# rajgandhi1/threecrate

Hardware: AMD Instinct MI355X
Metric: ICP iterations/sec (whole job: k=16 normals + 50-iter point-to-plane ICP per 1M-pt pair; tc_cloud handles, inputs resident in HBM) (higher is better)
Workload: dtype f32; 1 GPU; 1000000-pt uniform-random cloud, k=16 normals + 50-iter point-to-plane ICP, independent sigma = 0.0001 noise on source and target, correspondences returned (BASELINE configs[1]; one independent pair per GPU); points=1000000, k=16, parallelism=pairs1, interface=tc_cloud handles (one index build per cloud)

## Files before the change

### threecrate_amd/csrc/api.hip

```cpp
#include "tc_internal.h"
#include <sched.h>
#include <time.h>

#include <algorithm>
#include <cmath>
#include <cstdlib>
#include <cstring>
#include <memory>

namespace tc {

[[maybe_unused]] constexpr int kDebugPrintOnlyBits = 8 | 64 | 256 | 1024;
int debug_flags() {
    static const int flags = [] {
        const char *e = getenv("TC_DEBUG");
        const int f = e ? atoi(e) : 0;
#ifdef TC_DEV
        return f;
#else
        return f & kDebugPrintOnlyBits;
#endif
    }();
    return flags;
}
// ... 178 lines not shown
    return TC_OK;
}

tc_status synced(tc_context *ctx) {
    TC_HIP_TRY(ctx, hipStreamSynchronize(ctx->stream));
    return TC_OK;
}
tc_status stage_out(tc_context *ctx, void *h_dst, const void *d_src, size_t bytes) {
    TC_HIP_TRY(ctx, hipMemcpyAsync(h_dst, d_src, bytes, hipMemcpyDeviceToHost, ctx->stream));
    return synced(ctx);
}
tc_status read_back(tc_context *ctx, void *host_dst, const void *dev_src, size_t bytes) {
    if (tc_status s = stage_out(ctx, host_dst, dev_src, bytes)) return s;
    TC_HIP_TRY(ctx, hipGetLastError());
    return TC_OK;
}

float normals_cell_factor(size_t k, bool large) {
    const double K1 = (double)k + 1.0;
    const double lam = K1 + 3.1 * std::sqrt(K1) + 2.0;
    const double c = std::cbrt(lam / 4.18879);
    return (float)((large ? 1.03 : 0.95) * c / 2.0);
}

float normals_target_ppo(size_t k) {
    const double K1 = (double)k + 1.0;
    return (float)((K1 + 3.1 * std::sqrt(K1) + 2.0) / 11.3);
}

IndexSpec knn_grid(size_t list_len) {
    IndexSpec spec; spec.cell_factor = normals_cell_factor(list_len > 1 ? list_len - 1 : 1, false) * 2.0f;
    return spec;
}
IndexSpec ball_grid(float radius, bool finite_only) {
    const float r2 = radius * radius;
    IndexSpec spec; spec.cell_factor = 0.5f;
    if (r2 <= r2 && (!finite_only || r2 <= 3.0e38f)) { spec.min_cell_edge = 0.5f * radius; spec.target_ppo = 2.0f; }
    return spec;
}

void recycle_index(tc_context *ctx, DeviceIndex &ix) {
    for_each_buf(ix, [ctx](DevBuf &b) { recycle(ctx, b); });
    ix.pts12_valid = false; ix.vor_valid = false;
}

void free_index(DeviceIndex &ix) { for_each_buf(ix, free_buf); }

tc_status normals_on_index(tc_context *ctx, DeviceIndex &ix, bool build, float cell_factor_override, const float *d_xyz, size_t n,
                           const tc_normal_config *cfg, float *d_out, size_t p_begin, size_t p_end, bool slice_out, float4 *d_sorted_nrm,
                           bool with_bounds) {
    if (build) {
        const float min_h = cfg->has_radius ? cfg->radius * 0.5005f : 0.0f;
        const float f = cell_factor_override > 0.0f ? cell_factor_override : normals_cell_factor(cfg->k_neighbors, n >= kAdaptMinPoints);
        IndexSpec spec; spec.cell_factor = f; spec.min_cell_edge = min_h; spec.target_ppo = normals_target_ppo(cfg->k_neighbors); spec.strict_order = slice_out;
        if (tc_status s = build_index(ctx, ix, d_xyz, n, spec)) return s;
    }
    float vp[3];
    if (cfg->has_viewpoint) {
        vp[0] = cfg->viewpoint[0]; vp[1] = cfg->viewpoint[1]; vp[2] = cfg->viewpoint[2];
    } else {
        const float *bmn = ix.exact_min, *bmx = ix.exact_max;
        const float cx = (bmn[0] + bmx[0]) / 2.0f, cy = (bmn[1] + bmx[1]) / 2.0f, cz = (bmn[2] + bmx[2]) / 2.0f;
        const float ex = bmx[0] - bmn[0], ey = bmx[1] - bmn[1], ez = bmx[2] - bmn[2];
        const float extent = std::sqrt(ex * ex + ey * ey + ez * ez);
        vp[0] = cx + 0.0f; vp[1] = cy + 0.0f; vp[2] = cz + extent;
    }
    float4 *d_vor = nullptr;
    const bool knn_mode = !(cfg->has_radius && cfg->radius > 0.0f);
    if (with_bounds && knn_mode && p_begin == 0 && p_end >= n) {
        if (tc_status s = ensure(ctx, ix.vor, n * sizeof(float4))) return s;
        d_vor = (float4 *)ix.vor.p;
    }
    if (tc_status s = launch_normals(ctx, ix, d_xyz, *cfg, vp, d_out, p_begin, p_end, slice_out, d_sorted_nrm, d_vor)) return s;
    ix.vor_valid = d_vor != nullptr;
    return TC_OK;
}

static tc_status normals_device(tc_context *ctx, const float *d_xyz, size_t n, const tc_normal_config *cfg, float *d_out,
                                size_t p_begin = 0, size_t p_end = (size_t)-1, bool slice_out = false) {
    return normals_on_index(ctx, ctx->tgt_index, true, 0.0f, d_xyz, n, cfg, d_out, p_begin, p_end, slice_out, nullptr);
}

}

using namespace tc;

extern "C" {

int tc_abi_version(void) { return TC_ABI_VERSION; }

int tc_device_count(void) try {
    int n = 0;
    if (hipGetDeviceCount(&n) != hipSuccess) return 0;
    return n;
} TC_CATCH_VALUE(0)

static tc_status context_create(int device, void *stream, bool own, tc_context **out) {
    if (!out) return TC_INVALID_DATA;
    *out = nullptr;
    fault_point("context");
    int n = 0;
    if (hipGetDeviceCount(&n) != hipSuccess || n <= 0 || device < 0 || device >= n) return TC_GPU;
    if (hipSetDevice(device) != hipSuccess) return TC_GPU;
    std::unique_ptr<tc_context> holder(new tc_context());
    tc_context *ctx = holder.get();
    ctx->last_error.reserve(256);
    ctx->device = device;
    ctx->own_stream = own;
    if (own) {
        if (hipStreamCreateWithFlags(&ctx->stream, hipStreamNonBlocking) != hipSuccess) return TC_GPU;
    } else {
        ctx->stream = (hipStream_t)stream;
    }
    if (hipHostMalloc(&ctx->pinned, kPinnedBytes, hipHostMallocDefault) != hipSuccess) {
        if (own) (void)hipStreamDestroy(ctx->stream);
        return TC_GPU;
    }
    *out = holder.release();
    return TC_OK;
}

tc_status tc_context_create(int device, tc_context **out) try { return context_create(device, nullptr, true, out); } TC_CATCH_STATUS(nullptr)
tc_status tc_context_create_on_stream(int device, void *hip_stream, tc_context **out) try {
    return context_create(device, hip_stream, false, out);
} TC_CATCH_STATUS(nullptr)

tc_status tc_context_wait_stream(tc_context *ctx, void *other_hip_stream) try {
    if (!ctx) return TC_INVALID_DATA;
    hipStream_t other = (hipStream_t)other_hip_stream;
    if (other == ctx->stream) return TC_OK;
    TC_HIP_TRY(ctx, hipSetDevice(ctx->device));
    if (!ctx->order_event) TC_HIP_TRY(ctx, hipEventCreateWithFlags(&ctx->order_event, hipEventDisableTiming));
    TC_HIP_TRY(ctx, hipEventRecord(ctx->order_event, other));
    TC_HIP_TRY(ctx, hipStreamWaitEvent(ctx->stream, ctx->order_event, 0));
    return TC_OK;
} TC_CATCH_STATUS(ctx)

tc_status tc_stream_wait_context(tc_context *ctx, void *other_hip_stream) try {
    if (!ctx) return TC_INVALID_DATA;
    hipStream_t other = (hipStream_t)other_hip_stream;
    if (other == ctx->stream) return TC_OK;
    TC_HIP_TRY(ctx, hipSetDevice(ctx->device));
    if (!ctx->release_event) TC_HIP_TRY(ctx, hipEventCreateWithFlags(&ctx->release_event, hipEventDisableTiming));
    TC_HIP_TRY(ctx, hipEventRecord(ctx->release_event, ctx->stream));
    TC_HIP_TRY(ctx, hipStreamWaitEvent(other, ctx->release_event, 0));
    return TC_OK;
} TC_CATCH_STATUS(ctx)

void tc_context_destroy(tc_context *ctx) try {
    if (!ctx) return;
    (void)hipSetDevice(ctx->device);
    (void)hipStreamSynchronize(ctx->stream);
    if (ctx->copy_stream) { (void)hipStreamSynchronize(ctx->copy_stream); (void)hipStreamDestroy(ctx->copy_stream); }
    if (ctx->upload_event) (void)hipEventDestroy(ctx->upload_event);
    for_each_buf(*ctx, free_buf);
    for (auto &pb : ctx->pool) (void)hipFree(pb.p);
    for (auto e : ctx->chunk_events) (void)hipEventDestroy(e);
    if (ctx->order_event) (void)hipEventDestroy(ctx->order_event);
    if (ctx->release_event) (void)hipEventDestroy(ctx->release_event);
    for (auto &t : ctx->timers) for (auto &p : t.pending) { (void)hipEventDestroy(p.first); (void)hipEventDestroy(p.second); }
    for (auto e : ctx->event_pool) (void)hipEventDestroy(e);
    if (ctx->pinned) (void)hipHostFree(ctx->pinned);
    if (ctx->own_stream && ctx->stream) (void)hipStreamDestroy(ctx->stream);
    delete ctx;
} TC_CATCH_VOID

tc_status tc_context_trim(tc_context *ctx) try {
    if (!ctx) return TC_INVALID_DATA;
    TC_HIP_TRY(ctx, hipSetDevice(ctx->device));
    TC_HIP_TRY(ctx, hipStreamSynchronize(ctx->stream));
    for (auto &pb : ctx->pool) (void)hipFree(pb.p);
    ctx->pool.clear();
    ctx->pool_bytes = 0;
    ctx->pool_largest = 0;
    return TC_OK;
} TC_CATCH_STATUS(ctx)

const char *tc_last_error_message(const tc_context *ctx) { return ctx ? ctx->last_error.c_str() : "null context"; }

tc_status tc_synchronize(tc_context *ctx) try {
    if (!ctx) return TC_INVALID_DATA;
    return synced(ctx);
} TC_CATCH_STATUS(ctx)

void tc_normal_config_default(tc_normal_config *cfg) try {
    if (!cfg) return;
    std::memset(cfg, 0, sizeof(*cfg));
    cfg->k_neighbors = 10;
    cfg->has_radius = 0;
    cfg->consistent_orientation = 1;
    cfg->has_viewpoint = 0;
} TC_CATCH_VOID

static tc_status normals_validate(tc_context *ctx, size_t n, const tc_normal_config *cfg, bool *empty) {
    *empty = false;
    if (!ctx || !cfg) return TC_INVALID_DATA;
    if (n == 0) { *empty = true; return TC_OK; }
    if (cfg->k_neighbors < 3) return fail(ctx, TC_INVALID_DATA, "k_neighbors must be at least 3");
    return TC_OK;
}

tc_status tc_estimate_normals_device(tc_context *ctx, const float *d_xyz, size_t n, const tc_normal_config *cfg,
                                     float *d_out) try {
    bool empty;
    if (tc_status s = normals_validate(ctx, n, cfg, &empty)) return s;
    if (empty) return TC_OK;
    TC_HIP_TRY(ctx, hipSetDevice(ctx->device));
    if (tc_status s = normals_device(ctx, d_xyz, n, cfg, d_out)) return s;
    return synced(ctx);
} TC_CATCH_STATUS(ctx)

tc_status tc_estimate_normals_slice_device(tc_context *ctx, const float *d_xyz, size_t n, const tc_normal_config *cfg, size_t begin,
                                           size_t end, float *d_slice_out) try {
    bool empty;
    if (tc_status s = normals_validate(ctx, n, cfg, &empty)) return s;
    if (empty) return TC_OK;
    if (begin > end || end > n) return fail(ctx, TC_INVALID_DATA, "normals slice: need begin <= end <= n");
    TC_HIP_TRY(ctx, hipSetDevice(ctx->device));
    if (tc_status s = normals_device(ctx, d_xyz, n, cfg, d_slice_out, begin, end, true)) return s;
    return synced(ctx);
} TC_CATCH_STATUS(ctx)

tc_status tc_normals_unsort_device(tc_context *ctx, const float *d_sorted_all, size_t n, float *d_out) try {
    if (!ctx) return TC_INVALID_DATA;
    if (n == 0) return TC_OK;
    if (ctx->tgt_index.geom.n != n || !ctx->tgt_index.pts.p)
        return fail(ctx, TC_INVALID_DATA, "normals unsort: call tc_estimate_normals_slice_device on this context with the same cloud first");
    TC_HIP_TRY(ctx, hipSetDevice(ctx->device));
    if (tc_status s = launch_normals_unsort(ctx, ctx->tgt_index, d_sorted_all, d_out)) return s;
    return synced(ctx);
} TC_CATCH_STATUS(ctx)

tc_status tc_estimate_normals(tc_context *ctx, const float *xyz, size_t n, const tc_normal_config *cfg, float *out) try {
    bool empty;
    if (tc_status s = normals_validate(ctx, n, cfg, &empty)) return s;
    if (empty) return TC_OK;
    TC_HIP_TRY(ctx, hipSetDevice(ctx->device));
    if (tc_status s = ensure(ctx, ctx->out_a, n * 6 * sizeof(float))) return s;
    if (tc_status s = stage_in(ctx, ctx->in_a, xyz, n * 3 * sizeof(float))) return s;
    if (tc_status s = normals_device(ctx, (const float *)ctx->in_a.p, n, cfg, (float *)ctx->out_a.p)) return s;
    return stage_out(ctx, out, ctx->out_a.p, n * 6 * sizeof(float));
} TC_CATCH_STATUS(ctx)

static tc_status sharded_normals_slot(tc_context *ctx, tc_comm *comm, const float *d_xyz, size_t n, const tc_normal_config *cfg,
                                      float *slot_out, size_t &lo, size_t &hi) {
    const size_t W = (size_t)comm->nranks, r = (size_t)comm->rank;
    const size_t rows = (n + W - 1) / W;
    lo = std::min(r * rows, n); hi = std::min((r + 1) * rows, n);
    return normals_device(ctx, d_xyz, n, cfg, slot_out, lo, hi, true);
}

tc_status tc_sharded_estimate_normals_device(tc_context *ctx, tc_comm *comm, const float *d_xyz, size_t n, const tc_normal_config *cfg,
                                             float *d_out) try {
    if (!comm) return TC_INVALID_DATA;
    bool empty;
    if (tc_status s = normals_validate(ctx, n, cfg, &empty)) return s;
    if (empty) return TC_OK;
    if (comm->ctx != ctx) return fail(ctx, TC_INVALID_DATA, "the communicator belongs to another context");
    TC_HIP_TRY(ctx, hipSetDevice(ctx->device));
    const size_t W = (size_t)comm->nranks, r = (size_t)comm->rank;
    const size_t rows = (n + W - 1) / W;
    tc_status local = ensure(ctx, ctx->out_a, W * rows * 6 * sizeof(float));
    float *sorted_all = (float *)ctx->out_a.p;
    size_t lo = 0, hi = 0;
    if (local == TC_OK) local = sharded_normals_slot(ctx, comm, d_xyz, n, cfg, sorted_all + r * rows * 6, lo, hi);
    if (tc_status s = comm_agree(comm, local)) return s;
    if (tc_status s = comm_allgather(comm, sorted_all, rows * 6 * sizeof(float))) return s;
    if (tc_status s = launch_normals_unsort(ctx, ctx->tgt_index, sorted_all, d_out)) return s;
    return synced(ctx);
} TC_CATCH_STATUS(ctx)

__global__ void __launch_bounds__(256) slice_orig_index_kernel(const float4 *__restrict__ pts, uint32_t lo, uint32_t count, uint32_t *__restrict__ out) {
    const uint32_t i = blockIdx.x * blockDim.x + threadIdx.x;
    if (i < count) out[i] = __float_as_uint(pts[lo + i].w);
}

tc_status tc_sharded_estimate_normals_local_device(tc_context *ctx, tc_comm *comm, const float *d_xyz, size_t n, const tc_normal_config *cfg,
                                                   float *d_out_slice, uint32_t *d_orig_index, size_t *first, size_t *count) try {
    if (!comm || !first || !count) return TC_INVALID_DATA;
    *first = 0; *count = 0;
    bool empty;
    if (tc_status s = normals_validate(ctx, n, cfg, &empty)) return s;
    if (empty) return TC_OK;
    if (comm->ctx != ctx) return fail(ctx, TC_INVALID_DATA, "the communicator belongs to another context");
    TC_HIP_TRY(ctx, hipSetDevice(ctx->device));
    size_t lo = 0, hi = 0;
    if (tc_status s = sharded_normals_slot(ctx, comm, d_xyz, n, cfg, d_out_slice, lo, hi)) return s;
    if (d_orig_index && hi > lo) {
        hipLaunchKernelGGL(slice_orig_index_kernel, dim3((unsigned)((hi - lo + 255) / 256)), dim3(256), 0, ctx->stream,
                           (const float4 *)ctx->tgt_index.pts.p, (uint32_t)lo, (uint32_t)(hi - lo), d_orig_index);
        TC_HIP_TRY(ctx, hipGetLastError());
    }
    TC_HIP_TRY(ctx, hipStreamSynchronize(ctx->stream));
    *first = lo; *count = hi - lo;
    return TC_OK;
} TC_CATCH_STATUS(ctx)

unsigned long long tc_debug_counter(const tc_context *ctx, int which) try {
    if (!ctx) return 0;
    if (which >= TC_COUNTER_ICP_ITERATIONS && which <= TC_COUNTER_ICP_STEPS_TAKEN) return ctx->stat_icp[which - TC_COUNTER_ICP_ITERATIONS];
    return which == TC_COUNTER_INDEXED_POINTS ? ctx->stat_indexed_points : which == TC_COUNTER_INDEX_BUILDS ? ctx->stat_index_builds : 0ull;
} TC_CATCH_VALUE(0)

void tc_profile_enable(tc_context *ctx, int on) {
    if (!ctx) return;
    ctx->profiling = on;
    ctx->prof_tick = 0;
    if (on == 3) for (auto &v : ctx->stat_icp) v = 0;
}

static void profile_collect(tc_context *ctx) {
    (void)hipStreamSynchronize(ctx->stream);
    for (auto &t : ctx->timers) {
        for (auto &p : t.pending) {
            float ms = 0.0f;
            if (hipEventElapsedTime(&ms, p.first, p.second) == hipSuccess) {
                t.total_ms += ms; t.launches += 1;
                t.min_ms = std::min(t.min_ms, (double)ms); t.max_ms = std::max(t.max_ms, (double)ms);
            }
            ctx->event_pool.push_back(p.first);
            ctx->event_pool.push_back(p.second);
        }
        t.pending.clear();
    }
}

void tc_profile_reset(tc_context *ctx) try {
    if (!ctx) return;
    profile_collect(ctx);
    for (auto &t : ctx->timers) { t.launches = 0; t.total_ms = 0.0; t.min_ms = 1e300; t.max_ms = 0.0; }
} TC_CATCH_VOID

size_t tc_profile_read(tc_context *ctx, tc_kernel_stat *out, size_t cap) try {
    if (!ctx) return 0;
    profile_collect(ctx);
    size_t n = 0;
    for (auto &t : ctx->timers) {
        if (n < cap && out) {
            std::memset(&out[n], 0, sizeof(out[n]));
            std::strncpy(out[n].name, t.name.c_str(), sizeof(out[n].name) - 1);
            out[n].launches = t.launches;
            out[n].total_ms = t.total_ms;
            out[n].min_ms = t.launches ? t.min_ms : 0.0;
            out[n].max_ms = t.max_ms;
        }
        ++n;
    }
    return n;
} TC_CATCH_VALUE(0)

}
```

### threecrate_amd/csrc/cloud.hip

```cpp
#include "tc_internal.h"

#include <algorithm>
#include <cmath>
#include <cstring>

struct tc_cloud {
    tc_context *ctx = nullptr;
    size_t n = 0;
    tc::DevBuf xyz;
    tc::DeviceIndex ix;
    bool indexed = false;
    float factor = 0.0f;
    bool has_normals = false;
    tc::DevBuf normals6;
    bool has_normals6 = false;
};

namespace {

using namespace tc;


float shared_factor(float want) {
    return (want > 0.8f * kIcpCellFactor && want < 1.25f * kIcpCellFactor) ? kIcpCellFactor : want;
}

__global__ void __launch_bounds__(256) cloud_unsort_normals_kernel(const float4 *__restrict__ pts, const float4 *__restrict__ sorted_nrm,
                                                                  const float *__restrict__ xyz, uint32_t n, float *__restrict__ out6) {
    const uint32_t p = blockIdx.x * blockDim.x + threadIdx.x;
    if (p >= n) return;
    const uint32_t orig = __float_as_uint(pts[p].w);
    const float4 nr = sorted_nrm[p];
    float *o = out6 + 6 * (size_t)orig;
    o[0] = xyz[3 * (size_t)orig]; o[1] = xyz[3 * (size_t)orig + 1]; o[2] = xyz[3 * (size_t)orig + 2];
    o[3] = nr.x; o[4] = nr.y; o[5] = nr.z;
}

tc_status ensure_index(tc_cloud *c, float want_factor, float target_ppo, float min_h) {
    tc_context *ctx = c->ctx;
    const float f = shared_factor(want_factor);
    if (c->indexed && c->factor > 0.8f * f && c->factor < 1.25f * f && min_h <= c->ix.geom.h) return TC_OK;
    if (c->has_normals && !c->has_normals6 && c->indexed && c->n) {
        if (tc_status s = ensure(ctx, c->normals6, c->n * 6 * sizeof(float))) return s;
        hipLaunchKernelGGL(cloud_unsort_normals_kernel, dim3((unsigned)((c->n + 255) / 256)), dim3(256), 0, ctx->stream,
                           (const float4 *)c->ix.pts.p, (const float4 *)c->ix.normals.p, (const float *)c->xyz.p, (uint32_t)c->n,
                           (float *)c->normals6.p);
        TC_HIP_TRY(ctx, hipGetLastError());
        c->has_normals6 = true;
    }
    c->has_normals = false;
    IndexSpec spec; spec.cell_factor = f; spec.min_cell_edge = min_h; spec.target_ppo = target_ppo;
    if (tc_status s = build_index(ctx, c->ix, (const float *)c->xyz.p, c->n, spec)) return s;
    c->indexed = true;
    c->factor = f;
    return TC_OK;
}

tc_status cloud_create(tc_context *ctx, const float *p, size_t n, bool from_host, tc_cloud **out) {
    if (!ctx || !out) return TC_INVALID_DATA;
    *out = nullptr;
    if (tc_status s = check_point_count(ctx, n)) return s;
    TC_HIP_TRY(ctx, hipSetDevice(ctx->device));
    tc_cloud *c = new tc_cloud();
    c->ctx = ctx;
    c->n = n;
    if (n) {
        tc_status s = ensure(ctx, c->xyz, n * 3 * sizeof(float));
        if (s == TC_OK && hipMemcpyAsync(c->xyz.p, p, n * 3 * sizeof(float), from_host ? hipMemcpyHostToDevice : hipMemcpyDeviceToDevice,
                                         ctx->stream) != hipSuccess) s = fail(ctx, TC_GPU, "cloud upload failed");
        if (s == TC_OK && from_host && hipStreamSynchronize(ctx->stream) != hipSuccess) s = fail(ctx, TC_GPU, "cloud upload failed");
        if (s != TC_OK) { recycle(ctx, c->xyz); delete c; return s; }
    }
    *out = c;
    return TC_OK;
}

tc_status adopt_normals(tc_cloud *c, const float *d_normals, size_t stride) {
    if (tc_status s = ensure_index(c, kIcpCellFactor, 2.5f, 0.0f)) return s;
    if (tc_status s = gather_normals(c->ctx, c->ix, d_normals, stride)) return s;
    c->has_normals = true;
    return TC_OK;
}

tc_status prepare_target(tc_cloud *tgt, bool p2plane);

tc_status cloud_icp(tc_cloud *src, tc_cloud *tgt, bool p2plane, const float init[7], size_t max_iters, float max_dist, float conv_thr,
                    tc_icp_result *res) {
    if (!src || !tgt || !res || !init) return TC_INVALID_DATA;
    tc_context *ctx = tgt->ctx;
    if (src->ctx != ctx) return fail(ctx, TC_INVALID_DATA, "source and target handles belong to different contexts");
    if (src->n == 0 || tgt->n == 0) return fail(ctx, TC_INVALID_DATA, "Source or target point cloud is empty");
    if (p2plane && !tgt->has_normals && !tgt->has_normals6)
        return fail(ctx, TC_INVALID_DATA, "target_normals length must equal the number of target points (the target handle has no normals: "
                                          "tc_cloud_estimate_normals or tc_cloud_set_normals_device first)");
    if (max_iters == 0) return fail(ctx, TC_INVALID_DATA, "Max iterations must be positive");
    TC_HIP_TRY(ctx, hipSetDevice(ctx->device));
    if (tc_status s = prepare_target(tgt, p2plane)) return s;
    IcpJob job;
    job.mode = p2plane ? 1 : 0;
    job.src = (const float *)src->xyz.p; job.ns = src->n; job.tgt = (const float *)tgt->xyz.p; job.nt = tgt->n;
    job.init = init; job.max_iters = max_iters; job.max_dist = max_dist; job.conv_thr = conv_thr;
    job.tgt_prebuilt = &tgt->ix;
    job.src_presorted = (src->indexed && src != tgt) ? &src->ix : nullptr;
    return icp_run(ctx, job, res);
}

tc_status prepare_target(tc_cloud *tgt, bool p2plane) {
    tc_context *ctx = tgt->ctx;
    if (tc_status s = ensure_index(tgt, kIcpCellFactor, 2.5f, 0.0f)) return s;
    if (p2plane && !tgt->has_normals) {
        if (!tgt->has_normals6) return fail(ctx, TC_INVALID_DATA, "the target handle has no normals in input order to re-sort after its index was rebuilt");
        if (tc_status s = gather_normals(ctx, tgt->ix, (const float *)tgt->normals6.p + 3, 6)) return s;
        tgt->has_normals = true;
    }
    return TC_OK;
}

}

extern "C" {

tc_status tc_cloud_sharded_icp(tc_comm *comm, int shard_mode, int point_to_plane, const float *d_source, size_t n_source, tc_cloud *target,
                               const float init[7], size_t max_iters, float max_dist, float conv_thr, tc_icp_result *result) try {
    if (!comm || !target || !result || !init) return TC_INVALID_DATA;
    tc_context *ctx = target->ctx;
    if (comm->ctx != ctx) return fail(ctx, TC_INVALID_DATA, "the communicator belongs to another context");
    if (shard_mode != TC_SHARD_SPATIAL && shard_mode != TC_SHARD_LOCAL && shard_mode != TC_SHARD_INDEX) return fail(ctx, TC_INVALID_DATA, "unknown shard mode");
    const bool may_be_empty = shard_mode == TC_SHARD_LOCAL && comm->nranks > 1;
    if ((n_source == 0 && !may_be_empty) || target->n == 0) return fail(ctx, TC_INVALID_DATA, "Source or target point cloud is empty");
    if (point_to_plane && !target->has_normals && !target->has_normals6)
        return fail(ctx, TC_INVALID_DATA, "target_normals length must equal the number of target points (the target handle has no normals)");
    if (max_iters == 0) return fail(ctx, TC_INVALID_DATA, "Max iterations must be positive");
    TC_HIP_TRY(ctx, hipSetDevice(ctx->device));
    if (tc_status s = prepare_target(target, point_to_plane != 0)) return s;
    IcpJob job;
    job.mode = point_to_plane ? 1 : 0;
    job.src = d_source; job.ns = n_source; job.tgt = (const float *)target->xyz.p; job.nt = target->n;
    job.init = init; job.max_iters = max_iters; job.max_dist = max_dist; job.conv_thr = conv_thr;
    job.tgt_prebuilt = &target->ix;
    return icp_run_sharded(ctx, comm, shard_mode, job, result);
} TC_CATCH_STATUS((comm ? comm->ctx : nullptr))

tc_status tc_cloud_upload(tc_context *ctx, const float *xyz, size_t n, tc_cloud **out) try { return cloud_create(ctx, xyz, n, true, out); } TC_CATCH_STATUS(ctx)
tc_status tc_cloud_upload_device(tc_context *ctx, const float *d_xyz, size_t n, tc_cloud **out) try { return cloud_create(ctx, d_xyz, n, false, out); } TC_CATCH_STATUS(ctx)
size_t tc_cloud_size(const tc_cloud *c) { return c ? c->n : 0; }
const float *tc_cloud_points_device(const tc_cloud *c) { return c ? (const float *)c->xyz.p : nullptr; }
const float *tc_cloud_normals_device(const tc_cloud *cc) try {
    tc_cloud *c = const_cast<tc_cloud *>(cc);
    if (!c || c->n == 0) return nullptr;
    if (c->has_normals6) return (const float *)c->normals6.p;
    if (!c->has_normals || !c->indexed) return nullptr;
    tc_context *ctx = c->ctx;
    if (hipSetDevice(ctx->device) != hipSuccess) { (void)fail(ctx, TC_GPU, "tc_cloud_normals_device: hipSetDevice failed"); return nullptr; }
    if (ensure(ctx, c->normals6, c->n * 6 * sizeof(float)) != TC_OK) return nullptr;
    hipLaunchKernelGGL(cloud_unsort_normals_kernel, dim3((unsigned)((c->n + 255) / 256)), dim3(256), 0, ctx->stream,
                       (const float4 *)c->ix.pts.p, (const float4 *)c->ix.normals.p, (const float *)c->xyz.p, (uint32_t)c->n,
                       (float *)c->normals6.p);
    hipError_t e = hipGetLastError();
    if (e == hipSuccess) e = hipStreamSynchronize(ctx->stream);
    if (e != hipSuccess) { (void)fail(ctx, TC_GPU, std::string("tc_cloud_normals_device: ") + hipGetErrorString(e)); return nullptr; }
    c->has_normals6 = true;
    return (const float *)c->normals6.p;
} TC_CATCH_VALUE(nullptr)

static tc_status cloud_normals(tc_cloud *c, const tc_normal_config *cfg, float *out, bool out_on_host, bool keep6) {
    if (!c || !cfg) return TC_INVALID_DATA;
    tc_context *ctx = c->ctx;
    if (c->n == 0) return TC_OK;
    if (cfg->k_neighbors < 3) return fail(ctx, TC_INVALID_DATA, "k_neighbors must be at least 3");
    TC_HIP_TRY(ctx, hipSetDevice(ctx->device));
    const float min_h = cfg->has_radius ? cfg->radius * 0.5005f : 0.0f;
    c->has_normals = false;
    c->has_normals6 = false;
    if (tc_status s = ensure_index(c, normals_cell_factor(cfg->k_neighbors, c->n >= kAdaptMinPoints), normals_target_ppo(cfg->k_neighbors), min_h)) return s;
    if (tc_status s = ensure(ctx, c->ix.normals, c->n * sizeof(float4))) return s;
    const bool direct = out != nullptr && !out_on_host && !keep6;
    const bool want6 = (out != nullptr || keep6) && !direct;
    float *d_out6 = direct ? out : nullptr;
    if (want6) {
        if (tc_status s = ensure(ctx, c->normals6, c->n * 6 * sizeof(float))) return s;
        d_out6 = (float *)c->normals6.p;
    }
    c->has_normals = false;
    c->has_normals6 = false;
    if (tc_status s = normals_on_index(ctx, c->ix, false, 0.0f, (const float *)c->xyz.p, c->n, cfg, d_out6, 0, (size_t)-1, false,
                                       (float4 *)c->ix.normals.p, true)) return s;
    c->has_normals = true;
    c->has_normals6 = want6;
    if (out && !direct) TC_HIP_TRY(ctx, hipMemcpyAsync(out, d_out6, c->n * 6 * sizeof(float), out_on_host ? hipMemcpyDeviceToHost : hipMemcpyDeviceToDevice, ctx->stream));
    TC_HIP_TRY(ctx, hipStreamSynchronize(ctx->stream));
    return TC_OK;
}

tc_status tc_cloud_estimate_normals(tc_cloud *c, const tc_normal_config *cfg, float *out) try { return cloud_normals(c, cfg, out, true, false); } TC_CATCH_STATUS(c ? c->ctx : nullptr)
tc_status tc_cloud_estimate_normals_device(tc_cloud *c, const tc_normal_config *cfg, float *d_out) try { return cloud_normals(c, cfg, d_out, false, false); } TC_CATCH_STATUS(c ? c->ctx : nullptr)

tc_status tc_cloud_set_normals_device(tc_cloud *c, const float *d_normals, size_t n_normals, size_t stride) try {
    if (!c) return TC_INVALID_DATA;
    tc_context *ctx = c->ctx;
    if (n_normals != c->n) return fail(ctx, TC_INVALID_DATA, "target_normals length must equal the number of target points");
    if (stride < 3) return fail(ctx, TC_INVALID_DATA, "normal_stride must be >= 3");
    if (c->n == 0) return TC_OK;
    TC_HIP_TRY(ctx, hipSetDevice(ctx->device));
    c->has_normals = false;
    c->has_normals6 = false;
    if (tc_status s = adopt_normals(c, d_normals, stride)) return s;
    TC_HIP_TRY(ctx, hipStreamSynchronize(ctx->stream));
    return TC_OK;
} TC_CATCH_STATUS((c ? c->ctx : nullptr))

tc_status tc_cloud_icp_point_to_plane(tc_cloud *source, tc_cloud *target, const float init[7], size_t max_iters, float max_dist,
                                      float conv_thr, tc_icp_result *result) try {
    return cloud_icp(source, target, true, init, max_iters, max_dist, conv_thr, result);
} TC_CATCH_STATUS((source ? source->ctx : nullptr))

tc_status tc_cloud_icp_detailed(tc_cloud *source, tc_cloud *target, const float init[7], size_t max_iters, float max_dist,
                                float conv_thr, tc_icp_result *result) try {
    return cloud_icp(source, target, false, init, max_iters, max_dist, conv_thr, result);
} TC_CATCH_STATUS((source ? source->ctx : nullptr))

void tc_cloud_destroy(tc_cloud *c) try {
    if (!c) return;
    (void)hipSetDevice(c->ctx->device);
    (void)hipStreamSynchronize(c->ctx->stream);
    tc::recycle(c->ctx, c->xyz); tc::recycle(c->ctx, c->normals6);
    tc::recycle_index(c->ctx, c->ix);
    delete c;
} TC_CATCH_VOID

}
```

### threecrate_amd/csrc/grid.hip

```cpp
#include "tc_internal.h"
#include <rocprim/device/device_radix_sort.hpp>

#include <algorithm>
#include <cmath>
#include <cstring>

namespace tc {

constexpr int kBboxBlocks = 256;
__device__ __forceinline__ uint32_t f2ord(float f) { const uint32_t b = __float_as_uint(f); return (b & 0x80000000u) ? ~b : (b | 0x80000000u); }
__device__ __forceinline__ float ord2f(uint32_t u) { return __uint_as_float((u & 0x80000000u) ? (u ^ 0x80000000u) : ~u); }
constexpr uint32_t kOrdPlusInf = 0xFF800000u, kOrdMinusInf = 0x007FFFFFu;
constexpr uint32_t kBboxAccStride = 32;
constexpr size_t kBboxStateBytes = 31 * kBboxAccStride * sizeof(uint32_t), kBboxBufBytes = kBboxStateBytes + 128 + 256;

template <bool VEC>
__global__ void __launch_bounds__(256) bbox_kernel(const float *__restrict__ xyz, uint32_t n, uint32_t *__restrict__ state, int robust,
                                                  float *__restrict__ out, uint32_t *__restrict__ done) {
    const bool sbox = robust != 0;
    __shared__ float sm[4][30];
    float v[30];
#pragma unroll
    for (int k = 0; k < 30; ++k) v[k] = (k % 6 < 3) ? INFINITY : -INFINITY;
    auto take = [&](float x, float y, float z, uint32_t i, int s) {
        if (!(fabsf(x) <= 3.0e38f && fabsf(y) <= 3.0e38f && fabsf(z) <= 3.0e38f)) return;
        v[0] = fminf(v[0], x); v[1] = fminf(v[1], y); v[2] = fminf(v[2], z);
        v[3] = fmaxf(v[3], x); v[4] = fmaxf(v[4], y); v[5] = fmaxf(v[5], z);
        if (sbox && ((i * 2654435761u) >> 28) == 0u) {
            float *b = v + 6 + 6 * s;
            b[0] = fminf(b[0], x); b[1] = fminf(b[1], y); b[2] = fminf(b[2], z);
            b[3] = fmaxf(b[3], x); b[4] = fmaxf(b[4], y); b[5] = fmaxf(b[5], z);
        }
    };
    const uint32_t gt = blockIdx.x * blockDim.x + threadIdx.x, stride = gridDim.x * blockDim.x;
    if constexpr (VEC) {
        const float4 *__restrict__ q = reinterpret_cast<const float4 *>(xyz);
        const uint32_t nq = n >> 2;
        constexpr int U = 4;
        for (uint32_t c0 = gt; c0 < nq; c0 += U * stride) {
            float4 a[U], b[U], c[U];
#pragma unroll
            for (int u = 0; u < U; ++u) {
                const uint32_t cc = min(c0 + (uint32_t)u * stride, nq - 1u);
                a[u] = q[3 * (size_t)cc]; b[u] = q[3 * (size_t)cc + 1]; c[u] = q[3 * (size_t)cc + 2];
            }
#pragma unroll
            for (int u = 0; u < U; ++u) {
                const uint32_t i = 4u * min(c0 + (uint32_t)u * stride, nq - 1u);
                take(a[u].x, a[u].y, a[u].z, i, 0);
                take(a[u].w, b[u].x, b[u].y, i + 1u, 1);
                take(b[u].z, b[u].w, c[u].x, i + 2u, 2);
                take(c[u].y, c[u].z, c[u].w, i + 3u, 3);
            }
        }
        if (gt < (n & 3u)) {
            const uint32_t i = (nq << 2) + gt;
            const float x = xyz[3 * (size_t)i], y = xyz[3 * (size_t)i + 1], z = xyz[3 * (size_t)i + 2];
            if ((i & 3u) == 0u) take(x, y, z, i, 0); else if ((i & 3u) == 1u) take(x, y, z, i, 1); else take(x, y, z, i, 2);
        }
    } else {
        for (uint32_t i = gt; i < n; i += stride) {
            const float x = xyz[3 * (size_t)i], y = xyz[3 * (size_t)i + 1], z = xyz[3 * (size_t)i + 2];
            const uint32_t sidx = threadIdx.x & 3u;
            if (sidx == 0u) take(x, y, z, i, 0); else if (sidx == 1u) take(x, y, z, i, 1); else if (sidx == 2u) take(x, y, z, i, 2); else take(x, y, z, i, 3);
        }
    }
#pragma unroll
    for (int k = 0; k < 30; ++k) {
        if (k < 6 || sbox) {
#pragma unroll
            for (int o = 32; o > 0; o >>= 1) {
                const float w = __shfl_xor(v[k], o);
                v[k] = (k % 6 < 3) ? fminf(v[k], w) : fmaxf(v[k], w);
            }
        }
    }
    if ((threadIdx.x & 63) == 0) {
#pragma unroll
        for (int k = 0; k < 30; ++k) sm[threadIdx.x >> 6][k] = v[k];
    }
    __syncthreads();
    uint32_t *acc = state + kBboxAccStride;
    if (threadIdx.x < (sbox ? 30 : 6)) {
        const bool is_min = threadIdx.x % 6 < 3;
        float r = sm[0][threadIdx.x];
        for (int w = 1; w < 4; ++w) r = is_min ? fminf(r, sm[w][threadIdx.x]) : fmaxf(r, sm[w][threadIdx.x]);
        if (is_min) atomicMin(&acc[threadIdx.x * kBboxAccStride], f2ord(r)); else atomicMax(&acc[threadIdx.x * kBboxAccStride], f2ord(r));
    }
    __shared__ uint32_t s_last;
    if (threadIdx.x < 64) {
        asm volatile("s_waitcnt vmcnt(0)" ::: "memory");
        if (threadIdx.x == 0) s_last = __hip_atomic_fetch_add(state, 1u, __ATOMIC_RELAXED, __HIP_MEMORY_SCOPE_AGENT) == gridDim.x - 1u ? 1u : 0u;
    }
    __syncthreads();
    if (!s_last) return;
    if (threadIdx.x < 30) {
        const uint32_t u = __hip_atomic_load(&acc[threadIdx.x * kBboxAccStride], __ATOMIC_RELAXED, __HIP_MEMORY_SCOPE_AGENT);
        __hip_atomic_store(&out[threadIdx.x], ord2f(u), __ATOMIC_RELAXED, __HIP_MEMORY_SCOPE_SYSTEM);
        __hip_atomic_store(&acc[threadIdx.x * kBboxAccStride], (threadIdx.x % 6 < 3) ? kOrdPlusInf : kOrdMinusInf, __ATOMIC_RELAXED, __HIP_MEMORY_SCOPE_AGENT);
    }
    if (threadIdx.x == 0) __hip_atomic_store(state, 0u, __ATOMIC_RELAXED, __HIP_MEMORY_SCOPE_AGENT);
    if (done) {
        if (threadIdx.x < 30) __threadfence_system();
        __syncthreads();
        if (threadIdx.x == 0) __hip_atomic_store(done, 1u, __ATOMIC_RELEASE, __HIP_MEMORY_SCOPE_SYSTEM);
    }
}

__global__ void bbox_state_init_kernel(uint32_t *__restrict__ state) {
    const uint32_t t = threadIdx.x;
    if (t == 0) state[0] = 0u;
    if (t < 30) state[(t + 1) * kBboxAccStride] = (t % 6 < 3) ? kOrdPlusInf : kOrdMinusInf;
}


__global__ void __launch_bounds__(256) cell_hist_kernel(const float *__restrict__ xyz, uint32_t n, GridGeom g,
                                                       const IcpState *__restrict__ st, TileGeom tg, int tile_major, uint32_t nkeys,
                                                       uint32_t *__restrict__ cell_of, uint32_t *__restrict__ hist,
                                                       uint32_t *__restrict__ arrival, uint32_t *__restrict__ pts_pad,
                                                       uint32_t *__restrict__ cs_front, uint32_t *__restrict__ cs_tail, uint32_t rank_max) {
    uint32_t i = blockIdx.x * blockDim.x + threadIdx.x;
    if (blockIdx.x == 0 && threadIdx.x < 4 * kPtsPad + kCellStartFront + kCellStartPad) {
        const uint32_t t = threadIdx.x;
        if (t < 4 * kPtsPad) pts_pad[t] = 0x7F7F7F7Fu;
        else if (t < 4 * kPtsPad + kCellStartFront) cs_front[t - 4 * kPtsPad] = 0u;
        else cs_tail[t - 4 * kPtsPad - kCellStartFront] = 0u;
    }
    if (i >= n) return;
    float x = xyz[3 * (size_t)i], y = xyz[3 * (size_t)i + 1], z = xyz[3 * (size_t)i + 2];
    if (st) {
        float q[4] = {st->q[0], st->q[1], st->q[2], st->q[3]}, t[3] = {st->t[0], st->t[1], st->t[2]};
        float ox, oy, oz;
        isometry_apply(q, t, x, y, z, ox, oy, oz);
        x = ox; y = oy; z = oz;
    }
    int ix = cell_coord(x, g.minx, g.inv_h, g.gx);
    int iy = cell_coord(y, g.miny, g.inv_h, g.gy);
    int iz = cell_coord(z, g.minz, g.inv_h, g.gz);
    uint32_t c = tile_major ? tile_major_id(tg, ix, iy, iz) : ((uint32_t)iz * g.gy + iy) * g.gx + ix;
    if (!(fabsf(x) <= 3.0e38f && fabsf(y) <= 3.0e38f && fabsf(z) <= 3.0e38f)) c = nkeys;
    cell_of[i] = c;
    const uint32_t a = atomicAdd(&hist[c], 1u);
    arrival[i] = a;
    if (a == rank_max) hist[nkeys + 1] = 1u;
}

__global__ void __launch_bounds__(256) iota_kernel(uint32_t *__restrict__ p, uint32_t n) {
    const uint32_t i = blockIdx.x * blockDim.x + threadIdx.x;
    if (i < n) p[i] = i;
}

constexpr int kScanItems = 8;
constexpr int kScanBlock = 256;
constexpr int kScanTile = kScanItems * kScanBlock;

__global__ void __launch_bounds__(kScanBlock) scan_reduce_kernel(const uint32_t *__restrict__ in, uint32_t n,
                                                                 uint32_t *__restrict__ blocksum) {
    __shared__ uint32_t wsum[kScanBlock / 64], wnz[kScanBlock / 64];
    uint32_t base = blockIdx.x * kScanTile;
    uint32_t s = 0, nz = 0;
#pragma unroll
    for (int k = 0; k < kScanItems; ++k) {
        uint32_t i = base + k * kScanBlock + threadIdx.x;
        if (i < n) { const uint32_t v = in[i]; s += v; nz += v != 0; }
    }
#pragma unroll
    for (int o = 32; o > 0; o >>= 1) { s += __shfl_xor(s, o); nz += __shfl_xor(nz, o); }
    if ((threadIdx.x & 63) == 0) { wsum[threadIdx.x >> 6] = s; wnz[threadIdx.x >> 6] = nz; }
    __syncthreads();
    if (threadIdx.x == 0) {
        blocksum[blockIdx.x] = wsum[0] + wsum[1] + wsum[2] + wsum[3];
        blocksum[gridDim.x + blockIdx.x] = wnz[0] + wnz[1] + wnz[2] + wnz[3];
    }
}

constexpr uint32_t kScanFusedMax = 2048;
__global__ void __launch_bounds__(1024) scan_top_kernel(uint32_t *__restrict__ blocksum, uint32_t nb) {
    __shared__ uint32_t wtot[16];
    uint32_t carry = 0;
    for (uint32_t base = 0; base < nb; base += 1024) {
        const uint32_t i = base + threadIdx.x;
        const uint32_t v = i < nb ? blocksum[i] : 0u;
        uint32_t inc = v;
#pragma unroll
        for (int o = 1; o < 64; o <<= 1) {
            const uint32_t t = __shfl_up(inc, o);
            if ((threadIdx.x & 63) >= (unsigned)o) inc += t;
        }
        if ((threadIdx.x & 63) == 63) wtot[threadIdx.x >> 6] = inc;
        __syncthreads();
        uint32_t woff = 0, tot = 0;
        for (int w = 0; w < 16; ++w) { if (w < (int)(threadIdx.x >> 6)) woff += wtot[w]; tot += wtot[w]; }
        if (i < nb) blocksum[i] = carry + woff + inc - v;
        carry += tot;
        __syncthreads();
    }
}

__global__ void __launch_bounds__(kScanBlock) scan_apply_kernel(const uint32_t *__restrict__ in, uint32_t n,
                                                                uint32_t *__restrict__ blocksum,
                                                                uint32_t *__restrict__ out , uint32_t *__restrict__ occ_out, int prefixed,
                                                                unsigned long long *__restrict__ occ_host) {
    __shared__ uint32_t wtot[kScanBlock / 64];
    __shared__ uint32_t wpre[kScanBlock / 64], wnz[kScanBlock / 64];
    uint32_t pre = 0, nzt = 0;
    if (prefixed) { if (threadIdx.x == 0) pre = blocksum[blockIdx.x]; }
    else for (uint32_t i = threadIdx.x; i < blockIdx.x; i += kScanBlock) pre += blocksum[i];
    if (blockIdx.x == 0) for (uint32_t i = threadIdx.x; i < gridDim.x; i += kScanBlock) nzt += blocksum[gridDim.x + i];
#pragma unroll
    for (int o = 32; o > 0; o >>= 1) { pre += __shfl_xor(pre, o); nzt += __shfl_xor(nzt, o); }
    if ((threadIdx.x & 63) == 0) { wpre[threadIdx.x >> 6] = pre; wnz[threadIdx.x >> 6] = nzt; }
    uint32_t base = blockIdx.x * kScanTile + threadIdx.x * kScanItems;
    uint32_t v[kScanItems];
    uint32_t s = 0;
#pragma unroll
    for (int k = 0; k < kScanItems; ++k) {
        uint32_t i = base + k;
        v[k] = (i < n) ? in[i] : 0;
        s += v[k];
    }
    uint32_t inc = s;
#pragma unroll
    for (int o = 1; o < 64; o <<= 1) {
        uint32_t t = __shfl_up(inc, o);
        if ((threadIdx.x & 63) >= (unsigned)o) inc += t;
    }
    if ((threadIdx.x & 63) == 63) wtot[threadIdx.x >> 6] = inc;
    __syncthreads();
    uint32_t woff = 0;
    for (int w = 0; w < (int)(threadIdx.x >> 6); ++w) woff += wtot[w];
    uint32_t block_pre = 0;
    for (int w = 0; w < kScanBlock / 64; ++w) block_pre += wpre[w];
    if (blockIdx.x == 0 && threadIdx.x == 0) {
        uint32_t t = 0;
        for (int w = 0; w < kScanBlock / 64; ++w) t += wnz[w];
        blocksum[2 * gridDim.x] = t;
        if (occ_out) *occ_out = t;
        if (occ_host) __hip_atomic_store(occ_host, (1ull << 32) | (unsigned long long)t, __ATOMIC_RELAXED, __HIP_MEMORY_SCOPE_SYSTEM);
    }
    uint32_t run = block_pre + woff + inc - s;
#pragma unroll
    for (int k = 0; k < kScanItems; ++k) {
        uint32_t i = base + k;
        if (i < n) out[i] = run;
        run += v[k];
        if (i == n - 1) out[n] = run;
    }
}

__global__ void __launch_bounds__(256) rank_gather_kernel(const float *__restrict__ xyz, uint32_t n, uint32_t nkeys,
                                                         const uint32_t *__restrict__ cell_of,
                                                         const uint32_t *__restrict__ cell_start,
                                                         const uint32_t *__restrict__ slot,
                                                         float4 *__restrict__ pts, int slot_is_ordered, uint32_t rank_max) {
    uint32_t p = blockIdx.x * blockDim.x + threadIdx.x;
    if (p >= n) return;
    uint32_t i = slot[p];
    uint32_t c = cell_of[i];
    uint32_t s = cell_start[c], e = cell_start[c + 1];
    uint32_t rank;
    if (slot_is_ordered) {
        rank = p - s;
    } else if (e - s <= rank_max) {
        rank = 0;
        for (uint32_t j = s; j < e; ++j) rank += (slot[j] < i) ? 1u : 0u;
    } else {
        rank = p - s;
    }
    float4 r;
    r.x = xyz[3 * (size_t)i]; r.y = xyz[3 * (size_t)i + 1]; r.z = xyz[3 * (size_t)i + 2];
    if (c == nkeys) r.x = r.y = r.z = __uint_as_float(0x7F7F7F7Fu);
    r.w = __uint_as_float(i);
    pts[s + rank] = r;
}

__global__ void __launch_bounds__(256) place_kernel(const float *__restrict__ xyz, uint32_t n, uint32_t nkeys,
                                                   const uint32_t *__restrict__ cell_of, const uint32_t *__restrict__ cell_start,
                                                   const uint32_t *__restrict__ arrival, float4 *__restrict__ tmp) {
    const uint32_t i = blockIdx.x * blockDim.x + threadIdx.x;
    if (i >= n) return;
    const uint32_t c = cell_of[i];
    const uint32_t pos = cell_start[c] + arrival[i];
    float4 r;
    r.x = xyz[3 * (size_t)i]; r.y = xyz[3 * (size_t)i + 1]; r.z = xyz[3 * (size_t)i + 2];
    if (c == nkeys) r.x = r.y = r.z = __uint_as_float(0x7F7F7F7Fu);
    r.w = __uint_as_float(i);
    tmp[pos] = r;
}

__global__ void __launch_bounds__(256) rerank_kernel(uint32_t n, GridGeom g, const IcpState *__restrict__ st, TileGeom tg, int tile_major,
                                                    uint32_t nkeys, const uint32_t *__restrict__ cell_start, const float4 *__restrict__ tmp,
                                                    float4 *__restrict__ pts, uint32_t rank_max) {
    const uint32_t p = blockIdx.x * blockDim.x + threadIdx.x;
    if (p >= n) return;
    const float4 r = tmp[p];
    uint32_t c;
    {
        float x = r.x, y = r.y, z = r.z;
        if (st) {
            float q[4] = {st->q[0], st->q[1], st->q[2], st->q[3]}, t[3] = {st->t[0], st->t[1], st->t[2]};
            float ox, oy, oz;
            isometry_apply(q, t, x, y, z, ox, oy, oz);
            x = ox; y = oy; z = oz;
        }
        const int ix = cell_coord(x, g.minx, g.inv_h, g.gx), iy = cell_coord(y, g.miny, g.inv_h, g.gy), iz = cell_coord(z, g.minz, g.inv_h, g.gz);
        c = tile_major ? tile_major_id(tg, ix, iy, iz) : ((uint32_t)iz * g.gy + iy) * g.gx + ix;
        if (!(fabsf(x) <= 3.0e38f && fabsf(y) <= 3.0e38f && fabsf(z) <= 3.0e38f)) c = nkeys;
    }
    const uint32_t s = cell_start[c], e = cell_start[c + 1];
    const uint32_t i = __float_as_uint(r.w);
    uint32_t rank;
    if (e - s <= rank_max) {
        rank = 0;
#pragma unroll 4
        for (uint32_t j = s; j < e; ++j) rank += (__float_as_uint(tmp[j].w) < i) ? 1u : 0u;
    } else {
        rank = p - s;
    }
    pts[s + rank] = r;
}

__global__ void __launch_bounds__(256) gather_normals_kernel(const float4 *__restrict__ pts, uint32_t n,
                                                            const float *__restrict__ nrm, size_t stride,
                                                            float4 *__restrict__ out) {
    uint32_t p = blockIdx.x * blockDim.x + threadIdx.x;
    if (p >= n) return;
    uint32_t i = __float_as_uint(pts[p].w);
    const float *s = nrm + (size_t)i * stride;
    out[p] = make_float4(s[0], s[1], s[2], 0.0f);
}

GridView view_of(const DeviceIndex &ix) {
    GridView v;
    v.g = ix.geom;
    v.pts = (const float4 *)ix.pts.p;
    v.cell_start = (const uint32_t *)ix.cell_start.p + kCellStartFront;
    v.pts12 = ix.pts12_valid ? (const float *)ix.pts12.p : nullptr;
    return v;
}

static void set_cell_edge(GridGeom &g, double h, size_t n, double cells_per_point) {
    const double e[3] = {(double)g.maxx - g.minx, (double)g.maxy - g.miny, (double)g.maxz - g.minz};
    const double max_cells = std::max<double>(cells_per_point * (double)n, 4096.0);
    for (int guard = 0; guard < 200; ++guard) {
        double gx = std::floor(e[0] / h) + 1.0, gy = std::floor(e[1] / h) + 1.0, gz = std::floor(e[2] / h) + 1.0;
        if (gx * gy * gz <= max_cells && gx * gy * gz < 2.0e9) {
            g.gx = (int)gx; g.gy = (int)gy; g.gz = (int)gz;
            break;
        }
        h *= 1.2;
    }
    g.h = (float)h;
    g.inv_h = 1.0f / g.h;
    g.ncell = (uint32_t)g.gx * (uint32_t)g.gy * (uint32_t)g.gz;
    g.n = (uint32_t)n;
}

static void derive_geom(GridGeom &g, const float mn[3], const float mx[3], size_t n, float f, float min_h) {
    g.minx = mn[0]; g.miny = mn[1]; g.minz = mn[2];
    g.maxx = mx[0]; g.maxy = mx[1]; g.maxz = mx[2];
    g.cx = 0.5f * (mn[0] + mx[0]); g.cy = 0.5f * (mn[1] + mx[1]); g.cz = 0.5f * (mn[2] + mx[2]);
    double e[3] = {(double)mx[0] - mn[0], (double)mx[1] - mn[1], (double)mx[2] - mn[2]};
    double emax = std::max(e[0], std::max(e[1], e[2]));
    double h = 1.0;
    if (!(emax > 0.0) || !std::isfinite(emax)) {
        h = 1.0;
    } else {
        double measure = 1.0;
        int dims = 0;
        for (int a = 0; a < 3; ++a)
            if (e[a] > 1e-6 * emax) { measure *= e[a]; ++dims; }
        h = f * std::pow(measure / (double)std::max<size_t>(n, 1), 1.0 / (double)dims);
        if (!(h > 0.0) || !std::isfinite(h)) h = emax;
        h = std::max(h, emax * 1e-4);
    }
    if (min_h > 0.0f && std::isfinite(min_h)) h = std::max(h, (double)min_h);
    set_cell_edge(g, h, n, 8.0);
}

TileGeom make_tiles(const GridGeom &g, int tx, int ty, int tz) {
    TileGeom t;
    t.tx = std::max(tx, 1); t.ty = std::max(ty, 1); t.tz = std::max(tz, 1);
    t.ntx = (g.gx + t.tx - 1) / t.tx; t.nty = (g.gy + t.ty - 1) / t.ty; t.ntz = (g.gz + t.tz - 1) / t.tz;
    t.cpt = (uint32_t)(t.tx * t.ty * t.tz);
    t.ntiles = (uint32_t)t.ntx * (uint32_t)t.nty * (uint32_t)t.ntz;
    return t;
}

tc_status exclusive_scan_u32(tc_context *ctx, const uint32_t *d_in, uint32_t n, uint32_t *d_out, DevBuf &blocksum, uint32_t *occ_out,
                             unsigned long long *occ_host) {
    hipStream_t st = ctx->stream;
    const uint32_t nscan = (n + kScanTile - 1) / kScanTile;
    if (tc_status s = ensure(ctx, blocksum, ((size_t)2 * nscan + 1) * sizeof(uint32_t))) return s;
    hipLaunchKernelGGL(scan_reduce_kernel, dim3(nscan), dim3(kScanBlock), 0, st, d_in, n, (uint32_t *)blocksum.p);
    const char *fm = getenv("TC_SCAN_FUSED_MAX");
    const bool prefixed = nscan > (fm ? (uint32_t)atoi(fm) : kScanFusedMax);
    if (prefixed) hipLaunchKernelGGL(scan_top_kernel, dim3(1), dim3(1024), 0, st, (uint32_t *)blocksum.p, nscan);
    hipLaunchKernelGGL(scan_apply_kernel, dim3(nscan), dim3(kScanBlock), 0, st, d_in, n, (uint32_t *)blocksum.p, d_out, occ_out, prefixed ? 1 : 0, occ_host);
    TC_HIP_TRY(ctx, hipGetLastError());
    return TC_OK;
}

__global__ void __launch_bounds__(256) compact_flagged_kernel(const float *__restrict__ xyz, uint32_t n, const uint32_t *__restrict__ flag,
                                                             const uint32_t *__restrict__ pos, float *__restrict__ out_xyz, uint32_t *__restrict__ out_index) {
    const uint32_t i = blockIdx.x * blockDim.x + threadIdx.x;
    if (i >= n || !flag[i]) return;
    store_compacted(xyz, i, pos[i], out_xyz, out_index);
}

tc_status compact_flagged(tc_context *ctx, const float *d_xyz, uint32_t n, const uint32_t *d_flag, uint32_t *d_pos, DevBuf &blocksum, float *d_out_xyz,
                          uint32_t *d_out_index) {
    if (tc_status s = exclusive_scan_u32(ctx, d_flag, n, d_pos, blocksum)) return s;
    hipLaunchKernelGGL(compact_flagged_kernel, dim3((n + 255u) / 256u), dim3(256), 0, ctx->stream, d_xyz, n, d_flag, (const uint32_t *)d_pos, d_out_xyz, d_out_index);
    return TC_OK;
}

unsigned bits_for_value(uint64_t v) {
    unsigned b = 1;
    while (b < 64 && (1ull << b) <= v) ++b;
    return b;
}

template <class K>
tc_status sort_pairs(tc_context *ctx, const K *keys, K *keys_out, const uint32_t *vals, uint32_t *vals_out, size_t n, unsigned end_bit, DevBuf &temp) {
    K *k_in = const_cast<K *>(keys);
    uint32_t *v_in = const_cast<uint32_t *>(vals);
    size_t temp_bytes = 0;
    TC_HIP_TRY(ctx, rocprim::radix_sort_pairs(nullptr, temp_bytes, k_in, keys_out, v_in, vals_out, n, 0u, end_bit, ctx->stream));
    if (tc_status s = ensure(ctx, temp, temp_bytes)) return s;
    TC_HIP_TRY(ctx, rocprim::radix_sort_pairs(temp.p, temp_bytes, k_in, keys_out, v_in, vals_out, n, 0u, end_bit, ctx->stream));
    return TC_OK;
}
template tc_status sort_pairs<uint64_t>(tc_context *, const uint64_t *, uint64_t *, const uint32_t *, uint32_t *, size_t, unsigned, DevBuf &);
template tc_status sort_pairs<uint32_t>(tc_context *, const uint32_t *, uint32_t *, const uint32_t *, uint32_t *, size_t, unsigned, DevBuf &);

__global__ void __launch_bounds__(256) key_head_kernel(const uint64_t *__restrict__ keys, uint32_t n, uint32_t *__restrict__ head) {
    const uint32_t p = blockIdx.x * blockDim.x + threadIdx.x;
    if (p >= n) return;
    head[p] = (p == 0 || keys[p] != keys[p - 1]) ? 1u : 0u;
}

__global__ void __launch_bounds__(256) key_starts_kernel(uint32_t n, const uint32_t *__restrict__ head, const uint32_t *__restrict__ runpos,
                                                         uint32_t *__restrict__ rstart) {
    const uint32_t p = blockIdx.x * blockDim.x + threadIdx.x;
    if (p >= n) return;
    if (head[p]) rstart[runpos[p]] = p;
    if (p == n - 1) rstart[runpos[n]] = n;
}

tc_status key_runs(tc_context *ctx, const uint64_t *keys_sorted, uint32_t n, uint32_t *head, uint32_t *runpos, uint32_t *rstart, DevBuf &blocksum) {
    const dim3 grid((n + 255u) / 256u), block(256);
    hipLaunchKernelGGL(key_head_kernel, grid, block, 0, ctx->stream, keys_sorted, n, head);
    if (tc_status s = exclusive_scan_u32(ctx, head, n, runpos, blocksum)) return s;
    hipLaunchKernelGGL(key_starts_kernel, grid, block, 0, ctx->stream, n, (const uint32_t *)head, (const uint32_t *)runpos, rstart);
    return TC_OK;
}

tc_status group_by_key(tc_context *ctx, const uint64_t *keys, const uint32_t *vals, size_t n, unsigned key_bits, const GroupBufs &b, KeyGroups &g, size_t room) {
    const size_t items = std::max(n, room);
    const std::pair<DevBuf *, size_t> need[] = {{&b.keys_sorted, items * sizeof(uint64_t)}, {&b.vals_sorted, items * sizeof(uint32_t)},
                                                {&b.head, items * sizeof(uint32_t)}, {&b.runpos, (items + 1) * sizeof(uint32_t)},
                                                {&b.rstart, (items + 1) * sizeof(uint32_t)}};
    for (const auto &[buf, bytes] : need) if (tc_status s = ensure(ctx, *buf, bytes)) return s;
    uint64_t *keys_sorted = (uint64_t *)b.keys_sorted.p;
    uint32_t *order = (uint32_t *)b.vals_sorted.p, *head = (uint32_t *)b.head.p, *runpos = (uint32_t *)b.runpos.p, *rstart = (uint32_t *)b.rstart.p;
    g = KeyGroups{keys_sorted, order, head, runpos, rstart, runpos + n};
    if (tc_status s = sort_pairs(ctx, keys, keys_sorted, vals, order, n, key_bits, b.sort_temp)) return s;
    return key_runs(ctx, keys_sorted, (uint32_t)n, head, runpos, rstart, b.blocksum);
}

static tc_status cloud_bbox_impl(tc_context *ctx, const float *d_xyz, size_t n, float mn[3], float mx[3], float *rmn, float *rmx,
                                 bool *clamped) {
    hipStream_t st = ctx->stream;
    const int nb = (int)((n + 255) / 256);
    const int bb = std::min(nb, kBboxBlocks);
    const bool robust = rmn != nullptr && n >= 4096;
    const bool poll = pinned_poll_enabled();
    const bool fresh = ctx->bbox.p == nullptr;
    if (tc_status s = ensure(ctx, ctx->bbox, kBboxBufBytes)) return s;
    uint32_t *d_state = (uint32_t *)ctx->bbox.p;
    if (fresh) hipLaunchKernelGGL(bbox_state_init_kernel, dim3(1), dim3(64), 0, st, d_state);
    float *hb = pinned_host(ctx)->bbox;
    volatile uint32_t *h_done = &pinned_host(ctx)->bbox_done;
    float *d_out = (float *)((char *)ctx->bbox.p + kBboxStateBytes + 128);
    uint32_t *d_done = nullptr;
    if (poll) {
        d_out = (float *)pinned_dev_ptr(ctx, hb);
        d_done = (uint32_t *)pinned_dev_ptr(ctx, (const void *)h_done);
        if (!d_out || !d_done) return fail(ctx, TC_GPU, "bbox: the pinned block has no device address");
        *h_done = 0u;
    }
    {
        ProfScope ps(ctx, "bbox");
        if (((uintptr_t)d_xyz & 15u) == 0u)
            hipLaunchKernelGGL(bbox_kernel<true>, dim3(std::min((int)((n / 4 + 255) / 256) + 1, kBboxBlocks)), dim3(256), 0, st, d_xyz, (uint32_t)n, d_state, robust ? 1 : 0, d_out, d_done);
        else
            hipLaunchKernelGGL(bbox_kernel<false>, dim3(bb), dim3(256), 0, st, d_xyz, (uint32_t)n, d_state, robust ? 1 : 0, d_out, d_done);
    }
    TC_HIP_TRY(ctx, hipGetLastError());
    if (poll) {
        if (tc_status s = wait_pinned_word(ctx, h_done, "bounding box")) { hipLaunchKernelGGL(bbox_state_init_kernel, dim3(1), dim3(64), 0, st, d_state); return s; }
    } else {
        TC_HIP_TRY(ctx, hipMemcpyAsync(hb, d_out, 30 * sizeof(float), hipMemcpyDeviceToHost, st));
        TC_HIP_TRY(ctx, hipStreamSynchronize(st));
    }
    const float *hs = hb + 6;
    for (int c = 0; c < 3; ++c) { mn[c] = INFINITY; mx[c] = -INFINITY; }
    for (int c = 0; c < 3; ++c) { mn[c] = std::fmin(mn[c], hb[c]); mx[c] = std::fmax(mx[c], hb[3 + c]); }
    if (rmn) {
        for (int c = 0; c < 3; ++c) { rmn[c] = mn[c]; rmx[c] = mx[c]; }
        *clamped = false;
    }
    if (!robust) return TC_OK;
    float acc[24];
    for (int i = 0; i < 24; ++i) acc[i] = (i % 6 < 3) ? INFINITY : -INFINITY;
    for (int i = 0; i < 24; ++i) acc[i] = (i % 6 < 3) ? (hs[i] < acc[i] ? hs[i] : acc[i]) : (hs[i] > acc[i] ? hs[i] : acc[i]);
    for (int c = 0; c < 3; ++c) {
        float lo[4], hi[4];
        for (int k = 0; k < 4; ++k) { lo[k] = acc[6 * k + c]; hi[k] = acc[6 * k + 3 + c]; }
        std::sort(lo, lo + 4);
        std::sort(hi, hi + 4, [](float a, float b) { return a > b; });
        const float slo = lo[2], shi = hi[2];
        if (!(slo <= shi) || !std::isfinite(slo) || !std::isfinite(shi)) continue;
        const float ext = shi - slo, full = mx[c] - mn[c];
        if (!(full > 1.3f * ext) || !(full > 0.0f)) continue;
        rmn[c] = std::fmax(mn[c], slo - 0.05f * ext);
        rmx[c] = std::fmin(mx[c], shi + 0.05f * ext);
        *clamped = true;
    }
    return TC_OK;
}

tc_status cloud_bbox(tc_context *ctx, const float *d_xyz, size_t n, float mn[3], float mx[3]) {
    return cloud_bbox_impl(ctx, d_xyz, n, mn, mx, nullptr, nullptr, nullptr);
}


constexpr int kBinBlocks = 256;
constexpr int kBinWalkThreads = 1024;
#ifndef TC_BIN_TARGET
#define TC_BIN_TARGET 2048
#endif
#ifndef TC_BIN_PLACE_THREADS
#define TC_BIN_PLACE_THREADS 512
#endif
constexpr uint32_t kBinTarget = TC_BIN_TARGET;
constexpr uint32_t kBinCap = 2 * kBinTarget;
constexpr uint32_t kBinKeysMax = 2 * kBinTarget;
static_assert((kBinKeysMax + 3 * kBinCap) * sizeof(uint32_t) + 256 <= 160 * 1024, "bin_place_kernel's static LDS exceeds a gfx950 CU's 160 KB");
#if defined(__HIP_DEVICE_COMPILE__) && !defined(__gfx950__)
#error "libthreecrate_hip is written for gfx950 (MI355X): bin_place_kernel alone needs more than 64 KB of LDS per workgroup"
#endif
constexpr uint32_t kBinMaxBins = 8192;
constexpr int kBinPlaceThreads = TC_BIN_PLACE_THREADS;

__device__ __forceinline__ uint32_t point_key(float x, float y, float z, const GridGeom &g, const IcpState *__restrict__ st, const TileGeom &tg,
                                              int tile_major, uint32_t nkeys) {
    if (st) {
        float q[4] = {st->q[0], st->q[1], st->q[2], st->q[3]}, t[3] = {st->t[0], st->t[1], st->t[2]};
        float ox, oy, oz;
        isometry_apply(q, t, x, y, z, ox, oy, oz);
        x = ox; y = oy; z = oz;
    }
    const int ix = cell_coord(x, g.minx, g.inv_h, g.gx), iy = cell_coord(y, g.miny, g.inv_h, g.gy), iz = cell_coord(z, g.minz, g.inv_h, g.gz);
    uint32_t c = tile_major ? tile_major_id(tg, ix, iy, iz) : ((uint32_t)iz * g.gy + iy) * g.gx + ix;
    if (!(fabsf(x) <= 3.0e38f && fabsf(y) <= 3.0e38f && fabsf(z) <= 3.0e38f)) c = nkeys;
    return c;
}

__global__ void __launch_bounds__(kBinWalkThreads) bin_count_kernel(const float *__restrict__ xyz, uint32_t n, GridGeom g, const IcpState *__restrict__ st,
                                                       TileGeom tg, int tile_major, uint32_t nkeys, uint32_t kpb, uint32_t nbins,
                                                       uint32_t *__restrict__ cnt , uint32_t *__restrict__ pts_pad,
                                                       uint32_t *__restrict__ cs_front, uint32_t *__restrict__ cs_tail) {
    __shared__ uint32_t c[kBinMaxBins];
    if (blockIdx.x == 0 && threadIdx.x < 4 * kPtsPad + kCellStartFront + kCellStartPad) {
        const uint32_t t = threadIdx.x;
        if (t < 4 * kPtsPad) pts_pad[t] = 0x7F7F7F7Fu;
        else if (t < 4 * kPtsPad + kCellStartFront) cs_front[t - 4 * kPtsPad] = 0u;
        else cs_tail[t - 4 * kPtsPad - kCellStartFront] = 0u;
    }
    for (uint32_t b = threadIdx.x; b < nbins; b += kBinWalkThreads) c[b] = 0u;
    __syncthreads();
    const uint32_t per = (n + kBinBlocks - 1) / kBinBlocks;
    const uint32_t i0 = blockIdx.x * per, i1 = min(i0 + per, n);
    for (uint32_t i = i0 + threadIdx.x; i < i1; i += kBinWalkThreads) {
        const uint32_t k = point_key(xyz[3 * (size_t)i], xyz[3 * (size_t)i + 1], xyz[3 * (size_t)i + 2], g, st, tg, tile_major, nkeys);
        atomicAdd(&c[min(k / kpb, nbins - 1u)], 1u);
    }
    __syncthreads();
    for (uint32_t b = threadIdx.x; b < nbins; b += kBinWalkThreads) cnt[(size_t)b * kBinBlocks + blockIdx.x] = c[b];
}

static_assert(kBinBlocks == 256, "one wave x four entries per lane");
__global__ void __launch_bounds__(256) bin_offsets_kernel(uint32_t *__restrict__ cnt, uint32_t nbins, uint32_t *__restrict__ tot) {
    const uint32_t b = blockIdx.x * 4u + (threadIdx.x >> 6), lane = threadIdx.x & 63u;
    if (b >= nbins) return;
    uint4 *row = reinterpret_cast<uint4 *>(cnt + (size_t)b * kBinBlocks);
    const uint4 v = row[lane];
    const uint32_t s = v.x + v.y + v.z + v.w;
    uint32_t inc = s;
#pragma unroll
    for (int o = 1; o < 64; o <<= 1) {
        const uint32_t t = __shfl_up(inc, o);
        if (lane >= (unsigned)o) inc += t;
    }
    const uint32_t ex = inc - s;
    row[lane] = make_uint4(ex, ex + v.x, ex + v.x + v.y, ex + v.x + v.y + v.z);
    if (lane == 63u) tot[b] = inc;
}

__global__ void __launch_bounds__(kBinWalkThreads) bin_scatter_kernel(const float *__restrict__ xyz, uint32_t n, GridGeom g, const IcpState *__restrict__ st,
                                                         TileGeom tg, int tile_major, uint32_t nkeys, uint32_t kpb, uint32_t nbins,
                                                         const uint32_t *__restrict__ off ,
                                                         const uint32_t *__restrict__ tot, uint32_t *__restrict__ binstart,
                                                         uint32_t *__restrict__ occ_ticket, unsigned long long *__restrict__ host_word,
                                                         float4 *__restrict__ tmp) {
    static_assert(kBinWalkThreads == 1024, "the scan below is written for 16 waves");
    __shared__ uint32_t cur[kBinMaxBins];
    __shared__ uint32_t wtot[16], wmax[16];
    uint32_t carry = 0, mx = 0;
    for (uint32_t base = 0; base < nbins; base += kBinWalkThreads) {
        const uint32_t i = base + threadIdx.x;
        const uint32_t v = i < nbins ? tot[i] : 0u;
        const uint32_t o_mine = i < nbins ? off[(size_t)i * kBinBlocks + blockIdx.x] : 0u;
        mx = max(mx, v);
        uint32_t inc = v;
#pragma unroll
        for (int o = 1; o < 64; o <<= 1) {
            const uint32_t t = __shfl_up(inc, o);
            if ((threadIdx.x & 63) >= (unsigned)o) inc += t;
        }
        if ((threadIdx.x & 63) == 63) wtot[threadIdx.x >> 6] = inc;
        __syncthreads();
        uint32_t woff = 0, total = 0;
        for (int w = 0; w < 16; ++w) { if (w < (int)(threadIdx.x >> 6)) woff += wtot[w]; total += wtot[w]; }
        const uint32_t start = carry + woff + inc - v;
        if (i < nbins) {
            cur[i] = start + o_mine;
            if (blockIdx.x == 0) binstart[i] = start;
        }
        carry += total;
        __syncthreads();
    }
    if (blockIdx.x == 0) {
#pragma unroll
        for (int o = 32; o > 0; o >>= 1) mx = max(mx, (uint32_t)__shfl_xor(mx, o));
        if ((threadIdx.x & 63) == 0) wmax[threadIdx.x >> 6] = mx;
        __syncthreads();
        if (threadIdx.x == 0) {
            binstart[nbins] = carry;
            uint32_t m = 0;
            for (int w = 0; w < 16; ++w) m = max(m, wmax[w]);
            occ_ticket[0] = 0u; occ_ticket[1] = 0u;
            occ_ticket[2] = m;
            __hip_atomic_store(host_word, (1ull << 32) | (unsigned long long)m, __ATOMIC_RELAXED, __HIP_MEMORY_SCOPE_SYSTEM);
        }
    }
    const uint32_t per = (n + kBinBlocks - 1) / kBinBlocks;
    const uint32_t i0 = blockIdx.x * per, i1 = min(i0 + per, n);
    for (uint32_t i = i0 + threadIdx.x; i < i1; i += kBinWalkThreads) {
        float4 r;
        r.x = xyz[3 * (size_t)i]; r.y = xyz[3 * (size_t)i + 1]; r.z = xyz[3 * (size_t)i + 2];
        const uint32_t k = point_key(r.x, r.y, r.z, g, st, tg, tile_major, nkeys);
        if (k == nkeys) r.x = r.y = r.z = __uint_as_float(0x7F7F7F7Fu);
        r.w = __uint_as_float(i);
        tmp[atomicAdd(&cur[min(k / kpb, nbins - 1u)], 1u)] = r;
    }
}

__global__ void __launch_bounds__(kBinPlaceThreads) bin_place_kernel(const float4 *__restrict__ tmp, const uint32_t *__restrict__ binstart,
                                                                     uint32_t nbins, uint32_t kpb, uint32_t nkeys, GridGeom g,
                                                                     const IcpState *__restrict__ st, TileGeom tg, int tile_major,
                                                                     uint32_t *__restrict__ cs, float4 *__restrict__ pts,
                                                                     uint32_t *__restrict__ occ_ticket, uint32_t *__restrict__ occ_out,
                                                                     unsigned long long *__restrict__ occ_host) {
    __shared__ uint32_t cnt[kBinKeysMax];
    __shared__ uint32_t rkey[kBinCap];
    __shared__ uint32_t ridx[kBinCap];
    __shared__ uint32_t slot[kBinCap];
    __shared__ uint32_t wsum[kBinPlaceThreads / 64];
    __shared__ uint32_t s_occ;
    const uint32_t bin = blockIdx.x, tid = threadIdx.x;
    if (occ_ticket[2] > kBinCap) return;
    const uint32_t bs = binstart[bin], P = binstart[bin + 1] - bs;
    const uint32_t k0 = bin * kpb, K = min(kpb, nkeys + 1u - k0);
    for (uint32_t k = tid; k < K; k += kBinPlaceThreads) cnt[k] = 0u;
    if (tid == 0) s_occ = 0u;
    __syncthreads();
    for (uint32_t i = tid; i < P; i += kBinPlaceThreads) {
        const float4 r = tmp[bs + i];
        const uint32_t k = min(point_key(r.x, r.y, r.z, g, st, tg, tile_major, nkeys) - k0, K - 1u);
        const uint32_t a = atomicAdd(&cnt[k], 1u);
        rkey[i] = k | (a << 16);
        ridx[i] = __float_as_uint(r.w);
    }
    __syncthreads();
    constexpr uint32_t kPer = kBinKeysMax / kBinPlaceThreads;
    uint32_t v[kPer], sum = 0, nz = 0;
#pragma unroll
    for (uint32_t t = 0; t < kPer; ++t) {
        const uint32_t k = tid * kPer + t;
        v[t] = k < K ? cnt[k] : 0u;
        sum += v[t];
        nz += v[t] != 0u;
    }
    uint32_t inc = sum;
#pragma unroll
    for (int o = 1; o < 64; o <<= 1) {
        const uint32_t t2 = __shfl_up(inc, o);
        if ((tid & 63) >= (unsigned)o) inc += t2;
    }
#pragma unroll
    for (int o = 32; o > 0; o >>= 1) nz += __shfl_xor(nz, o);
    if ((tid & 63) == 63) wsum[tid >> 6] = inc;
    if ((tid & 63) == 0 && nz) atomicAdd(&s_occ, nz);
    __syncthreads();
    uint32_t run = inc - sum;
    for (uint32_t w = 0; w < (tid >> 6); ++w) run += wsum[w];
#pragma unroll
    for (uint32_t t = 0; t < kPer; ++t) {
        const uint32_t k = tid * kPer + t;
        if (k < K) { cnt[k] = run; cs[k0 + k] = bs + run; }
        run += v[t];
    }
    if (bin == nbins - 1 && tid == 0) cs[nkeys + 1] = bs + P;
    __syncthreads();
    for (uint32_t i = tid; i < P; i += kBinPlaceThreads) slot[cnt[rkey[i] & 0xFFFFu] + (rkey[i] >> 16)] = ridx[i];
    __syncthreads();
    for (uint32_t i = tid; i < P; i += kBinPlaceThreads) {
        const uint32_t k = rkey[i] & 0xFFFFu, me = ridx[i];
        const uint32_t s0 = cnt[k], e0 = (k + 1 < K) ? cnt[k + 1] : P;
        uint32_t rank = 0;
        for (uint32_t j = s0; j < e0; ++j) rank += slot[j] < me ? 1u : 0u;
        rkey[i] = s0 + rank;
    }
    __syncthreads();
    for (uint32_t i = tid; i < P; i += kBinPlaceThreads) slot[rkey[i]] = i;
    __syncthreads();
    for (uint32_t t = tid; t < P; t += kBinPlaceThreads) pts[bs + t] = tmp[bs + slot[t]];
    if (tid == 0) {
        const unsigned long long mine = ((unsigned long long)s_occ << 32) | 1ull;
        const unsigned long long old = __hip_atomic_fetch_add(reinterpret_cast<unsigned long long *>(occ_ticket), mine, __ATOMIC_RELAXED, __HIP_MEMORY_SCOPE_AGENT);
        if ((uint32_t)old == nbins - 1u) {
            const uint32_t occ = (uint32_t)(old >> 32) + s_occ;
            if (occ_out) __hip_atomic_store(occ_out, occ, __ATOMIC_RELAXED, __HIP_MEMORY_SCOPE_AGENT);
            if (occ_host) __hip_atomic_store(occ_host, (1ull << 32) | (unsigned long long)occ, __ATOMIC_RELAXED, __HIP_MEMORY_SCOPE_SYSTEM);
        }
    }
}

static uint32_t rank_quadratic_max() {
    const char *e = getenv("TC_RANK_QUADRATIC_MAX");
    return e ? (uint32_t)std::max(1, atoi(e)) : kRankQuadraticMax;
}

static bool binned_build_enabled() {
    const char *e = getenv("TC_INDEX_BINNED");
    return !(e && atoi(e) == 0);
}

tc_status build_index(tc_context *ctx, DeviceIndex &ix, const float *d_xyz, size_t n, const IndexSpec &spec) {
    if (n == 0 || n >= kMaxPoints) return fail(ctx, TC_INVALID_DATA, "build_index: bad point count");
    ctx->stat_indexed_points += n;
    ctx->stat_index_builds += 1;
    ix.vor_valid = false;
    ix.pts12_valid = false;
    ix.occ_host_valid = false;
    hipStream_t st = ctx->stream;
    const uint32_t n32 = (uint32_t)n;
    const int nb = (int)((n + 255) / 256);
    const int dbg = debug_flags();
    const uint32_t rank_max = rank_quadratic_max();

    if (spec.reuse_geom) {
        ix.geom = *spec.reuse_geom;
        ix.geom.n = n32;
    } else {
        float mn[3], mx[3], rmn[3], rmx[3];
        bool clamped = false;
        if (tc_status s = cloud_bbox_impl(ctx, d_xyz, n, mn, mx, rmn, rmx, &clamped)) return s;
        if (dbg & 2048) clamped = false, std::memcpy(rmn, mn, sizeof(mn)), std::memcpy(rmx, mx, sizeof(mx));
        for (int c = 0; c < 3; ++c) {
            if (!(mn[c] <= mx[c]) || !std::isfinite(mn[c]) || !std::isfinite(mx[c])) { mn[c] = 0.0f; mx[c] = 0.0f; rmn[c] = 0.0f; rmx[c] = 0.0f; }
            ix.exact_min[c] = mn[c]; ix.exact_max[c] = mx[c];
        }
        derive_geom(ix.geom, rmn, rmx, n, spec.cell_factor, spec.min_cell_edge);
        ix.geom.clamped = clamped ? 1 : 0;
        if ((dbg & 256) && clamped)
            fprintf(stderr, "[tc] index: box clamped to %g..%g %g..%g %g..%g (exact %g..%g %g..%g %g..%g)\n", rmn[0], rmx[0], rmn[1], rmx[1],
                    rmn[2], rmx[2], mn[0], mx[0], mn[1], mx[1], mn[2], mx[2]);
    }
    const bool adapt = spec.target_ppo > 0.0f && !spec.reuse_geom && !spec.tile_major && n >= kAdaptMinPoints && !(dbg & 512);
    uint32_t nkeys_final = 0;
    const uint32_t *cs_final = nullptr;
    for (int attempt = 0;; ++attempt) {
        const GridGeom g = ix.geom;
        TileGeom tg{};
        uint32_t nkeys = g.ncell;
        if (spec.tile_major) {
            tg = *spec.tile_major;
            ix.tile = tg;
            const uint64_t nk = (uint64_t)tg.ntiles * tg.cpt;
            if (nk >= kMaxPoints) return fail(ctx, TC_UNSUPPORTED, "tile-major key space too large");
            nkeys = (uint32_t)nk;
        }

        if (tc_status s = ensure(ctx, ix.pts, (n + kPtsPad) * sizeof(float4))) return s;
        if (tc_status s = ensure(ctx, ix.cell_of, n * sizeof(uint32_t))) return s;
        if (tc_status s = ensure(ctx, ix.slot, n * sizeof(uint32_t))) return s;
        if (tc_status s = ensure(ctx, ix.arrival, n * sizeof(uint32_t))) return s;
        const size_t fill_bytes = (((size_t)nkeys + 2) * sizeof(uint32_t) + 255) & ~(size_t)255;
        if (tc_status s = ensure(ctx, ix.fill, fill_bytes)) return s;
        if (tc_status s = ensure(ctx, ix.cell_start, (kCellStartFront + (size_t)nkeys + 2 + kCellStartPad) * sizeof(uint32_t))) return s;
        uint32_t *const cs = (uint32_t *)ix.cell_start.p + kCellStartFront;
        nkeys_final = nkeys; cs_final = cs;
        const bool check = adapt && attempt < 3;
        volatile uint32_t *h_occ = pinned_host(ctx)->occ;

        bool binned_done = false;
        if (binned_build_enabled() && pinned_poll_enabled() && !spec.strict_order && n >= kAdaptMinPoints && n <= (1u << 24) && nkeys < 0x7FFFFFF0u) {
            const uint32_t keys = nkeys + 1u;
            uint32_t nbins = std::max<uint32_t>((n32 + kBinTarget - 1) / kBinTarget, (keys + kBinKeysMax - 1) / kBinKeysMax);
            const uint32_t kpb = (keys + nbins - 1) / nbins;
            nbins = (keys + kpb - 1) / kpb;
            if (nbins <= kBinMaxBins && kpb <= kBinKeysMax) {
                const size_t words = 4 + (size_t)kBinBlocks * nbins + nbins + (nbins + 1);
                if (tc_status s = ensure(ctx, ix.fill, std::max(fill_bytes, words * sizeof(uint32_t)))) return s;
                uint32_t *occ_ticket = (uint32_t *)ix.fill.p, *cnt = occ_ticket + 4, *tot = cnt + (size_t)kBinBlocks * nbins, *binstart = tot + nbins;
                volatile uint32_t *h_max = pinned_host(ctx)->bin_max;
                unsigned long long *d_max = (unsigned long long *)pinned_dev_ptr(ctx, (const void *)h_max);
                if (!d_max) return fail(ctx, TC_GPU, "index build: the pinned block has no device address");
                h_max[0] = 0u; h_max[1] = 0u;
                {
                    ProfScope ps(ctx, "cell_bin_count");
                    hipLaunchKernelGGL(bin_count_kernel, dim3(kBinBlocks), dim3(kBinWalkThreads), 0, st, d_xyz, n32, g, spec.state_transform, tg, spec.tile_major ? 1 : 0, nkeys, kpb,
                                       nbins, cnt, reinterpret_cast<uint32_t *>((float4 *)ix.pts.p + n), (uint32_t *)ix.cell_start.p, cs + nkeys + 2);
                }
                {
                    ProfScope ps(ctx, "cell_bin_offsets");
                    hipLaunchKernelGGL(bin_offsets_kernel, dim3((nbins + 3) / 4), dim3(256), 0, st, cnt, nbins, tot);
                }
                if (tc_status s = ensure(ctx, ctx->build_tmp, (n + kPtsPad) * sizeof(float4))) return s;
                {
                    ProfScope ps(ctx, "cell_bin_scatter");
                    hipLaunchKernelGGL(bin_scatter_kernel, dim3(kBinBlocks), dim3(kBinWalkThreads), 0, st, d_xyz, n32, g, spec.state_transform, tg, spec.tile_major ? 1 : 0, nkeys,
                                       kpb, nbins, (const uint32_t *)cnt, (const uint32_t *)tot, binstart, occ_ticket, d_max, (float4 *)ctx->build_tmp.p);
                }
                if (check) { h_occ[0] = 0u; h_occ[1] = 0u; }
                unsigned long long *d_occ_host = check ? (unsigned long long *)pinned_dev_ptr(ctx, (const void *)h_occ) : nullptr;
                {
                    ProfScope ps(ctx, "cell_bin_place");
                    hipLaunchKernelGGL(bin_place_kernel, dim3(nbins), dim3(kBinPlaceThreads), 0, st, (const float4 *)ctx->build_tmp.p, (const uint32_t *)binstart,
                                       nbins, kpb, nkeys, g, spec.state_transform, tg, spec.tile_major ? 1 : 0, cs, (float4 *)ix.pts.p, occ_ticket,
                                       (uint32_t *)ix.cell_start.p, d_occ_host);
                }
                TC_HIP_TRY(ctx, hipGetLastError());
                if (tc_status s = wait_pinned_word(ctx, h_max + 1, "index build (bin populations)")) return s;
                if (h_max[0] <= kBinCap) {
                    binned_done = true;
                } else if (dbg & 256) {
                    fprintf(stderr, "[tc] index: largest bin holds %u points (> %u): atomic counting sort\n", h_max[0], kBinCap);
                }
            }
        }
        if (!binned_done) {
        TC_HIP_TRY(ctx, hipMemsetAsync(ix.fill.p, 0, fill_bytes, st));
        {
            ProfScope ps(ctx, "cell_hist");
            hipLaunchKernelGGL(cell_hist_kernel, dim3(nb), dim3(256), 0, st, d_xyz, n32, g, spec.state_transform, tg, spec.tile_major ? 1 : 0, nkeys,
                               (uint32_t *)ix.cell_of.p, (uint32_t *)ix.fill.p, (uint32_t *)ix.arrival.p,
                               reinterpret_cast<uint32_t *>((float4 *)ix.pts.p + n), (uint32_t *)ix.cell_start.p, cs + nkeys + 2, rank_max);
        }
        {
            ProfScope ps(ctx, "cell_scan");
            if (check) { h_occ[0] = 0u; h_occ[1] = 0u; }
            unsigned long long *d_occ_host = (check && pinned_poll_enabled()) ? (unsigned long long *)pinned_dev_ptr(ctx, (const void *)h_occ) : nullptr;
            if (check && pinned_poll_enabled() && !d_occ_host) return fail(ctx, TC_GPU, "index build: the pinned block has no device address");
            if (tc_status s = exclusive_scan_u32(ctx, (const uint32_t *)ix.fill.p, nkeys + 1, cs, ix.blocksum, (uint32_t *)ix.cell_start.p, d_occ_host)) return s;
        }
        if (tc_status s = ensure(ctx, ctx->build_tmp, (n + kPtsPad) * sizeof(float4))) return s;
        {
            ProfScope ps(ctx, "cell_place");
            hipLaunchKernelGGL(place_kernel, dim3(nb), dim3(256), 0, st, d_xyz, n32, nkeys, (const uint32_t *)ix.cell_of.p, (const uint32_t *)cs,
                               (const uint32_t *)ix.arrival.p, (float4 *)ctx->build_tmp.p);
        }
        {
            ProfScope ps(ctx, "cell_rerank");
            hipLaunchKernelGGL(rerank_kernel, dim3(nb), dim3(256), 0, st, n32, g, spec.state_transform, tg, spec.tile_major ? 1 : 0, nkeys, (const uint32_t *)cs,
                               (const float4 *)ctx->build_tmp.p, (float4 *)ix.pts.p, rank_max);
        }
        }
        TC_HIP_TRY(ctx, hipGetLastError());
        if (!check) break;
        if (pinned_poll_enabled()) {
            if (tc_status s = wait_pinned_word(ctx, h_occ + 1, "index build (occupied cells)")) return s;
        } else {
            const uint32_t nscan = (nkeys + 1 + kScanTile - 1) / kScanTile;
            TC_HIP_TRY(ctx, hipMemcpyAsync((void *)h_occ, (const uint32_t *)ix.blocksum.p + 2 * nscan, sizeof(uint32_t), hipMemcpyDeviceToHost, st));
            TC_HIP_TRY(ctx, hipStreamSynchronize(st));
        }
        const uint32_t occ_now = h_occ[0];
        const double ppo = (double)n / (double)std::max<uint32_t>(occ_now, 1u);
        ix.occ_host = occ_now; ix.occ_host_valid = true;
        if (dbg & 256)
            fprintf(stderr, "[tc] index: n %zu h %.5f grid %d x %d x %d = %u cells (%.2f n), %u occupied, %.2f points each (want %.1f)\n", n,
                    g.h, g.gx, g.gy, g.gz, g.ncell, (double)g.ncell / (double)n, occ_now, ppo, spec.target_ppo);
        if (!(ppo > 2.0 * spec.target_ppo)) break;
        double h = (double)g.h * std::min(0.8, std::max(0.35, std::sqrt((double)spec.target_ppo / ppo)));
        if (spec.min_cell_edge > 0.0f) h = std::max(h, (double)spec.min_cell_edge);
        GridGeom ng = g;
        set_cell_edge(ng, h, n, 32.0);
        if (!(ng.h < 0.95f * g.h)) break;
        ix.geom = ng;
        ix.occ_host_valid = false;
    }
    if (spec.strict_order) {
        if (tc_status s = read_back(ctx, &pinned_host(ctx)->big_cell, (const uint32_t *)ix.fill.p + nkeys_final + 1, sizeof(uint32_t))) return s;
        if (pinned_host(ctx)->big_cell) {
            if (tc_status s = ensure(ctx, ctx->overflow, n * sizeof(uint32_t))) return s;
            uint32_t *iota = (uint32_t *)ix.arrival.p, *keys_out = (uint32_t *)ctx->overflow.p;
            hipLaunchKernelGGL(iota_kernel, dim3(nb), dim3(256), 0, st, iota, n32);
            if (tc_status s = sort_pairs(ctx, (const uint32_t *)ix.cell_of.p, keys_out, (const uint32_t *)iota, (uint32_t *)ix.slot.p, n,
                                         bits_for_value(nkeys_final), ix.blocksum)) return s;
            ProfScope ps(ctx, "cell_rank_gather_strict");
            hipLaunchKernelGGL(rank_gather_kernel, dim3(nb), dim3(256), 0, st, d_xyz, n32, nkeys_final, (const uint32_t *)ix.cell_of.p,
                               (const uint32_t *)cs_final, (const uint32_t *)ix.slot.p, (float4 *)ix.pts.p, 1, rank_max);
            TC_HIP_TRY(ctx, hipGetLastError());
        }
    }
    return TC_OK;
}

tc_status gather_normals(tc_context *ctx, DeviceIndex &ix, const float *d_normals, size_t stride) {
    const size_t n = ix.geom.n;
    if (tc_status s = ensure(ctx, ix.normals, n * sizeof(float4))) return s;
    ProfScope ps(ctx, "gather_normals");
    hipLaunchKernelGGL(gather_normals_kernel, dim3((unsigned)((n + 255) / 256)), dim3(256), 0, ctx->stream,
                       (const float4 *)ix.pts.p, (uint32_t)n, d_normals, stride, (float4 *)ix.normals.p);
    TC_HIP_TRY(ctx, hipGetLastError());
    return TC_OK;
}

}
```

### threecrate_amd/csrc/icp.hip

```cpp
#include "tc_internal.h"
#include <hip/hip_ext.h>

#include <algorithm>
#include <type_traits>
#include <cmath>
#include <cstring>
#include <cstdlib>
#include <cstdio>

namespace tc {

typedef uint32_t u32x16 __attribute__((ext_vector_type(16)));
struct IcpHeader {
    float q[4], t[3];
    float prev_mse, conv_thr, max_dist;
    uint32_t iterations;
    int32_t done;
    float d_ang, d_t;
    uint32_t d_run;
};
static_assert(offsetof(IcpState, done) == 48 && offsetof(IcpState, max_dist) == 60 && offsetof(IcpState, iterations) == 36 &&
              offsetof(IcpState, prev_mse) == 28 && offsetof(IcpState, conv_thr) == 56, "IcpState header layout");
__device__ __forceinline__ IcpHeader load_header(const IcpState *st) {
    const u32x16 h = *reinterpret_cast<const u32x16 *>(st);
// ... 1297 lines not shown
    st->iterations = hd.iterations + 1u;
    st->mse = mse;
    st->n_corr = n;
    const float change = fabsf(hd.prev_mse - mse);
    if (change < hd.conv_thr) { st->converged = 1; st->done = 1; return; }
    st->prev_mse = mse;
}

constexpr int kFinalizeThreads = 512;
template <int MODE>
__device__ void finalize_body(const double *__restrict__ partials, uint32_t nblocks, IcpState *__restrict__ st, const GridGeom &g,
                              int do_sum, int do_apply, double (*sm)[TC_ICP_SUMS_STRIDE], const IcpHeader &hd, int cert_active = 0) {
    const bool done = hd.done != 0;
    constexpr bool P2PLANE = MODE != 0;
    if (do_sum) {
        constexpr int G = kFinalizeThreads / 32;
        {
            const int col = threadIdx.x & 31, grp = threadIdx.x >> 5;
            double s0 = 0.0, s1 = 0.0, s2 = 0.0, s3 = 0.0;
            uint32_t b = grp;
            if (nblocks == 256) {
                double v[256 / G];
#pragma unroll
                for (int k = 0; k < 256 / G; ++k) v[k] = partials[(size_t)(grp + G * k) * TC_ICP_SUMS_STRIDE + col];
#pragma unroll
                for (int k = 0; k < 256 / G; k += 4) { s0 += v[k]; s1 += v[k + 1]; s2 += v[k + 2]; s3 += v[k + 3]; }
                b = 256 + grp;
            }
            for (; b + 3 * G < nblocks; b += 4 * G) {
                s0 += partials[(size_t)b * TC_ICP_SUMS_STRIDE + col];
                s1 += partials[(size_t)(b + G) * TC_ICP_SUMS_STRIDE + col];
                s2 += partials[(size_t)(b + 2 * G) * TC_ICP_SUMS_STRIDE + col];
                s3 += partials[(size_t)(b + 3 * G) * TC_ICP_SUMS_STRIDE + col];
            }
            for (; b < nblocks; b += G) s0 += partials[(size_t)b * TC_ICP_SUMS_STRIDE + col];
            sm[grp][col] = (s0 + s1) + (s2 + s3);
        }
        __syncthreads();
        double tot = 0.0;
        if (threadIdx.x < TC_ICP_SUMS_STRIDE) {
#pragma unroll
            for (int gi = 0; gi < G; ++gi) tot += sm[gi][threadIdx.x];
            if (!done) st->sums[threadIdx.x] = tot;
        }
        __syncthreads();
        if (threadIdx.x < TC_ICP_SUMS_STRIDE) sm[0][threadIdx.x] = tot;
        __syncthreads();
    }
    if (!do_apply || threadIdx.x != 0 || done) return;
    const double *S = do_sum ? &sm[0][0] : st->sums;
    if (P2PLANE) {
        const double cnt = S[28];
        if (cnt < 6.0) { st->status = TC_ALGORITHM; st->done = 1; return; }
        double x[6];
        if (!chol6_solve(S, S + 21, x)) {
            __shared__ double sA[6][6], sx[6];
            int o = 0;
#pragma unroll
            for (int r = 0; r < 6; ++r)
#pragma unroll
                for (int c = r; c < 6; ++c) { sA[r][c] = S[o]; sA[c][r] = S[o]; ++o; }
#pragma unroll
            for (int r = 0; r < 6; ++r) sx[r] = S[21 + r];
            if (!lu6_solve(sA, sx)) { st->status = TC_ALGORITHM; st->done = 1; return; }
#pragma unroll
            for (int r = 0; r < 6; ++r) x[r] = sx[r];
        }
        const float hx = (float)x[0] / 2.0f, hy = (float)x[1] / 2.0f, hz = (float)x[2] / 2.0f;
        float sx, cx, sy, cy, sz, cz;
        sincosf(hx, &sx, &cx); sincosf(hy, &sy, &cy); sincosf(hz, &sz, &cz);
        const float qx[4] = {sx, 0.0f, 0.0f, cx};
        const float qy[4] = {0.0f, sy, 0.0f, cy};
        const float qz[4] = {0.0f, 0.0f, sz, cz};
        float zy[4], rot[4];
        quat_mul_f(qz, qy, zy);
        quat_mul_f(zy, qx, rot);
        const float dt[3] = {(float)x[3], (float)x[4], (float)x[5]};
        compose(hd, st, rot, dt, g, S[kSearchersCol], cnt, cert_active);
        finish_iteration(hd, st, (float)(S[27] / cnt), (uint32_t)cnt);
    } else {
        const double cnt = S[16];
        if (cnt < 3.0) { st->status = TC_ALGORITHM; st->done = 1; return; }
        const double ms[3] = {S[0] / cnt, S[1] / cnt, S[2] / cnt}, mq[3] = {S[3] / cnt, S[4] / cnt, S[5] / cnt};
        double H[3][3], R[3][3];
        for (int r = 0; r < 3; ++r) for (int c = 0; c < 3; ++c) H[r][c] = S[6 + 3 * r + c] - cnt * ms[r] * mq[c];
        if (st->kiss) {
            double hn = 0.0;
            for (int r = 0; r < 3; ++r) for (int c = 0; c < 3; ++c) hn += H[r][c] * H[r][c];
            if (sqrt(hn) < 1e-10) { st->status = TC_ALGORITHM; st->done = 1; return; }
        }
        kabsch_rotation(H, R);
        const double cs[3] = {ms[0] + (double)g.cx, ms[1] + (double)g.cy, ms[2] + (double)g.cz};
        const double cq[3] = {mq[0] + (double)g.cx, mq[1] + (double)g.cy, mq[2] + (double)g.cz};
        float dq[4];
        rotmat_to_quat(R, dq);
        float dt[3];
        for (int r = 0; r < 3; ++r) dt[r] = (float)(cq[r] - (R[r][0] * cs[0] + R[r][1] * cs[1] + R[r][2] * cs[2]));
        compose(hd, st, dq, dt, g, S[kSearchersCol], cnt, cert_active);
        double nmse = S[15];
        if (st->kiss) {
            const double d0 = ms[0] - mq[0], d1 = ms[1] - mq[1], d2 = ms[2] - mq[2];
            double rh = 0.0;
            for (int i = 0; i < 3; ++i) for (int j = 0; j < 3; ++j) rh += R[i][j] * H[j][i];
            nmse = S[15] - cnt * (d0 * d0 + d1 * d1 + d2 * d2) + 2.0 * (H[0][0] + H[1][1] + H[2][2]) - 2.0 * rh;
            nmse = fmax(nmse, 0.0);
        }
        finish_iteration(hd, st, (float)(nmse / cnt), (uint32_t)cnt);
    }
}

template <int MODE>
__global__ void __launch_bounds__(kFinalizeThreads) icp_finalize_kernel(const double *__restrict__ partials, uint32_t nblocks,
                                                           IcpState *__restrict__ st, const GridGeom g, int do_sum, int do_apply,
                                                           int32_t *__restrict__ done_out, int cert_active) {
    const IcpHeader hd = load_header(st);
    __shared__ double sm[kFinalizeThreads / 32][TC_ICP_SUMS_STRIDE];
    if (hd.done && !do_sum) { if (done_out && threadIdx.x == 0) __hip_atomic_store(done_out, 1, __ATOMIC_RELAXED, __HIP_MEMORY_SCOPE_SYSTEM); return; }
#ifdef TC_PHASE_STAMPS
    const unsigned long long t0 = __builtin_amdgcn_s_memtime();
    finalize_body<MODE>(partials, nblocks, st, g, do_sum, 0, sm, hd);
    const unsigned long long t1 = __builtin_amdgcn_s_memtime();
    finalize_body<MODE>(partials, nblocks, st, g, 0, do_apply, sm, hd, cert_active | (done_out != nullptr ? 2 : 0));
    const unsigned long long t2 = __builtin_amdgcn_s_memtime();
    if (threadIdx.x == 0) { st->refine_ring_hist[0] += (uint32_t)(t1 - t0); st->refine_ring_hist[1] += (uint32_t)(t2 - t1); }
#else
    finalize_body<MODE>(partials, nblocks, st, g, do_sum, do_apply, sm, hd, cert_active | (done_out != nullptr ? 2 : 0));
#endif
    if (done_out && threadIdx.x == 0)
        __hip_atomic_store(done_out, (hd.done || st->done) ? 1 : (st->d_ang >= 0.0f ? 3 : 2), __ATOMIC_RELAXED, __HIP_MEMORY_SCOPE_SYSTEM);
}

constexpr int kStateWords = (int)(offsetof(IcpState, sums) / sizeof(uint32_t));
static_assert(kStateWords <= 64, "one lane per word");
__device__ __forceinline__ void publish_state(const IcpState *st, IcpState *host_out, uint32_t *lds) {
    if (threadIdx.x == 0) {
        const uint32_t *s = reinterpret_cast<const uint32_t *>(st);
        for (int i = 0; i < kStateWords; ++i) lds[i] = s[i];
    }
    __syncthreads();
    if ((int)threadIdx.x < kStateWords)
        __hip_atomic_store(reinterpret_cast<uint32_t *>(host_out) + threadIdx.x, lds[threadIdx.x], __ATOMIC_RELAXED, __HIP_MEMORY_SCOPE_SYSTEM);
}
__global__ void icp_finish_kernel(IcpState *__restrict__ st, const double *__restrict__ partials, uint32_t nblocks, int p2plane, int from_sums,
                                  IcpState *__restrict__ host_out) {
    __shared__ uint32_t lds[64];
    if (threadIdx.x == 0 && !st->done) {
    st->converged = 0;
    if (p2plane || st->kiss) {
        st->mse = st->prev_mse;
    } else {
        double s = 0.0, c = 0.0;
        if (from_sums) { s = st->sums[0]; c = st->sums[1]; }
        else for (uint32_t b = 0; b < nblocks; ++b) { s += partials[(size_t)b * TC_ICP_SUMS_STRIDE]; c += partials[(size_t)b * TC_ICP_SUMS_STRIDE + 1]; }
        st->mse = (c > 0.0) ? (float)(s / c) : st->prev_mse;
    }
    st->done = 1;
    }
    if (host_out) publish_state(st, host_out, lds);
}

__global__ void icp_final_mse_fold_kernel(IcpState *__restrict__ st, const double *__restrict__ partials, uint32_t nblocks) {
    if (threadIdx.x >= TC_ICP_SUMS_STRIDE) return;
    double s = 0.0;
    if (threadIdx.x < 2 && !st->done)
        for (uint32_t b = 0; b < nblocks; ++b) s += partials[(size_t)b * TC_ICP_SUMS_STRIDE + threadIdx.x];
    st->sums[threadIdx.x] = s;
}

struct IcpLaunch {
    uint32_t nblocks = 0, chunk = 0;
    uint32_t mse_blocks = 0, mse_chunk = 0;
};
static IcpLaunch plan_launch(size_t ns) {
    IcpLaunch l;
    constexpr size_t kResidentBlocks = 4 * 256;
    size_t chunk = (ns + kResidentBlocks - 1) / kResidentBlocks;
    chunk = std::max<size_t>((chunk + kIcpBlock - 1) / kIcpBlock * kIcpBlock, kIcpBlock);
    uint32_t nb = (uint32_t)((ns + chunk - 1) / chunk);
    nb = std::max<uint32_t>((nb + 7) / 8 * 8, 8);
    l.nblocks = nb; l.chunk = (uint32_t)chunk;
    l.mse_blocks = nb; l.mse_chunk = (uint32_t)chunk;
    return l;
}

static TileGeom plan_tiles(const GridGeom &g, size_t ns) {
    const double rho = (double)ns / std::max<double>(g.ncell, 1.0);
    const double want = 256.0 / std::max(rho, 1e-6);
    static const int cand[][3] = {{8, 2, 2}, {8, 3, 2}, {8, 3, 3}, {8, 4, 3}, {8, 4, 4}, {8, 5, 4}, {8, 5, 5}, {8, 6, 5},
                                  {8, 6, 6}, {10, 6, 6}, {12, 6, 6}, {16, 6, 6}, {16, 8, 8}, {4, 2, 2}, {4, 2, 1}, {2, 2, 1}};
    int best = 0; double bd = 1e300;
    for (int i = 0; i < (int)(sizeof(cand) / sizeof(cand[0])); ++i) {
        const double c = (double)cand[i][0] * cand[i][1] * cand[i][2];
        const double d = std::fabs(std::log(c / want));
        if (d < bd) { bd = d; best = i; }
    }
    return make_tiles(g, cand[best][0], cand[best][1], cand[best][2]);
}

struct IcpSetup {
    int mode = 0;
    IcpLaunch l;
    GridView tv;
    TileGeom tg;
    DeviceIndex *tix = nullptr;
    const float4 *nrm = nullptr;
    const float4 *src = nullptr;
    float4 *wsrc = nullptr;
    uint32_t ns = 0;
    const float4 *src_cov = nullptr;
    float4 *wl = nullptr;
    IcpState *st = nullptr;
    uint32_t *rlist = nullptr;
    double *partials = nullptr;
};
static inline uint32_t *match_words(float4 *wsrc) { return reinterpret_cast<uint32_t *>(wsrc) + 3; }

enum class IcpStep { FullIteration, ReduceSum, ApplyOnly };

enum class MainVariant { Plain, Stats, Cert, Count };
static MainVariant main_variant(const IcpSetup &su, int dbg, bool want_cert, const int32_t *done_out) {
    if (dbg & 8) return MainVariant::Stats;
    const bool bounds = su.wl != nullptr && su.mode != 2;
    if (want_cert && bounds) return MainVariant::Cert;
    if (done_out != nullptr && bounds) return MainVariant::Count;
    return MainVariant::Plain;
}
using MainKernel = decltype(&icp_correspond_reduce_kernel<0>);
static MainKernel main_kernel(int mode, MainVariant v) {
    switch (v) {
    case MainVariant::Plain: return mode == 1 ? icp_correspond_reduce_kernel<1> : mode == 2 ? icp_correspond_reduce_kernel<2> : icp_correspond_reduce_kernel<0>;
    case MainVariant::Stats: return mode == 1 ? icp_correspond_reduce_kernel<1, true> : mode == 2 ? icp_correspond_reduce_kernel<2, true> : icp_correspond_reduce_kernel<0, true>;
    case MainVariant::Cert: return mode == 1 ? icp_correspond_reduce_kernel<1, false, true> : icp_correspond_reduce_kernel<0, false, true>;
    case MainVariant::Count: return mode == 1 ? icp_correspond_reduce_kernel<1, false, false, true> : icp_correspond_reduce_kernel<0, false, false, true>;
    }
    return nullptr;
}

static void launch_iteration(tc_context *ctx, const IcpSetup &su, IcpStep step, const float4 *vor = nullptr, int32_t *done_out = nullptr,
                             bool want_cert = false) {
    hipStream_t s = ctx->stream;
    const int dbg = debug_flags() | (ctx->profiling == 3 ? 8 : 0), mode = su.mode;
    const bool reduce_sum = step != IcpStep::ApplyOnly, apply = step != IcpStep::ReduceSum;
    const IcpLaunch &l = su.l;
    uint32_t *corr_pos = match_words(su.wsrc);
    double *refine_rows = su.partials + (size_t)l.nblocks * TC_ICP_SUMS_STRIDE;
    const MainVariant variant = main_variant(su, dbg, want_cert, done_out);
    if (reduce_sum) {
        {
            ProfScope ps(ctx, mode == 1 ? "icp_correspond_reduce_p2plane" : mode == 2 ? "icp_correspond_reduce_gicp" : "icp_correspond_reduce_p2p", true);
            const MainKernel kern = main_kernel(mode, variant);
            const float4 *vor_arg = (dbg & 4) ? nullptr : vor;
            unsigned long long *times_arg = (dbg & 1024) ? (unsigned long long *)ctx->dbg_times.p : nullptr;
            if (ps.active())
                hipExtLaunchKernelGGL(kern, dim3(l.nblocks), dim3(kIcpBlock), 0, s, ps.e0, ps.e1, 0, su.tv, su.nrm, su.wsrc, su.ns, l.chunk,
                                      (const IcpState *)su.st, su.rlist, su.partials, dbg, su.src_cov, vor_arg, times_arg, su.tv.pts12);
            else
                hipLaunchKernelGGL(kern, dim3(l.nblocks), dim3(kIcpBlock), 0, s, su.tv, su.nrm, su.wsrc, su.ns, l.chunk, su.st, su.rlist, su.partials, dbg,
                                   su.src_cov, vor_arg, times_arg, su.tv.pts12);
        }
        ProfScope ps(ctx, "icp_refine");
        auto kern = mode == 1 ? icp_refine_kernel<1> : mode == 2 ? icp_refine_kernel<2> : icp_refine_kernel<0>;
        hipLaunchKernelGGL(kern, dim3(kRefineBlocks), dim3(kRefineThreads), 0, s, su.tv, su.nrm, (const float4 *)su.wsrc, su.st, corr_pos, su.rlist, su.partials,
                           l.nblocks, l.chunk / (kIcpBlock / 64), refine_rows, su.src_cov, dbg);
        if (mode == 0 && !(dbg & 16)) {
            ProfScope ps2(ctx, "icp_exact_p2p_sums");
            const uint32_t chunk = exact_sums_chunk(su.ns);
            const uint32_t blocks = std::min<uint32_t>(std::max<uint32_t>((uint32_t)(((uint64_t)su.ns + chunk - 1) / chunk), 1u), (uint32_t)kRefineBlocks);
            hipLaunchKernelGGL(icp_exact_p2p_sums_kernel, dim3(blocks), dim3(kIcpBlock), 0, s, su.tv, (const float4 *)su.wsrc, su.ns, chunk,
                               (const IcpState *)su.st, refine_rows);
        }
    }
    ProfScope ps(ctx, "icp_finalize");
    const uint32_t rows = kRefineBlocks;
    auto kern = mode == 0 ? icp_finalize_kernel<0> : icp_finalize_kernel<1>;
    hipLaunchKernelGGL(kern, dim3(1), dim3(kFinalizeThreads), 0, s, refine_rows, rows, su.st, su.tv.g, reduce_sum ? 1 : 0, (apply && !(dbg & 32)) ? 1 : 0,
                       apply ? done_out : nullptr, (variant == MainVariant::Cert && reduce_sum) ? 1 : 0);
}

static size_t vor_after() {
    static const size_t v = [] { const char *e = getenv("TC_VOR_AFTER"); return e ? (size_t)atoi(e) : (size_t)6; }();
    return v;
}
static tc_status launch_target_nn_bounds(tc_context *ctx, DeviceIndex &ix, const GridView &tv, const IcpState *st, const float4 **out) {
    *out = nullptr;
    if (ix.vor_valid) { *out = (const float4 *)ix.vor.p; return TC_OK; }
    if (tc_status s = ensure(ctx, ix.vor, (size_t)ix.geom.n * sizeof(float4))) return s;
    ProfScope ps(ctx, "icp_target_nn_bounds");
    const bool persistent = &ix != &ctx->tgt_index;
    hipLaunchKernelGGL(icp_target_nn_bound_kernel, dim3((ix.geom.n + 255) / 256), dim3(256), 0, ctx->stream, tv, (float4 *)ix.vor.p,
                       persistent ? nullptr : st);
    ix.vor_valid = persistent;
    *out = (const float4 *)ix.vor.p;
    return TC_OK;
}

__global__ void __launch_bounds__(256) icp_pack12_kernel(const float4 *__restrict__ pts, uint32_t n, uint32_t npad, float *__restrict__ out) {
    const uint32_t i = blockIdx.x * blockDim.x + threadIdx.x;
    if (i >= npad) return;
    float4 r = make_float4(__uint_as_float(0x7F7F7F7Fu), __uint_as_float(0x7F7F7F7Fu), __uint_as_float(0x7F7F7F7Fu), 0.f);
    if (i < n) r = pts[i];
    out[3 * (size_t)i] = r.x; out[3 * (size_t)i + 1] = r.y; out[3 * (size_t)i + 2] = r.z;
}

__global__ void __launch_bounds__(256) icp_working_source_kernel(const float4 *__restrict__ src, uint32_t n, float4 *__restrict__ out, float4 *__restrict__ wl) {
    const uint32_t i = blockIdx.x * blockDim.x + threadIdx.x;
    if (i >= n) return;
    if (wl) wl[i] = make_float4(0.f, 0.f, 0.f, 0.f);
    float4 r = src[i];
    r.w = __uint_as_float(0xFFFFFFFFu);
    out[i] = r;
}

static tc_status icp_setup(tc_context *ctx, const IcpJob &job, const DeviceIndex *src_presorted, bool strict_source_order, IcpSetup &out) {
    const float *d_src = job.src, *d_tgt = job.tgt, *init = job.init;
    const size_t ns = job.ns, nt = job.nt;
    DeviceIndex *tgt_prebuilt = job.tgt_prebuilt;
    out.mode = job.mode;
    if (nt >= (1ull << 28) || ns >= (1ull << 28)) return fail(ctx, TC_UNSUPPORTED, "ICP clouds are limited to 2^28 - 1 points");
    out.tix = tgt_prebuilt ? tgt_prebuilt : &ctx->tgt_index;
    if (!tgt_prebuilt) {
        IndexSpec target_grid; target_grid.cell_factor = kIcpCellFactor; target_grid.target_ppo = 2.5f;
        if (tc_status s = build_index(ctx, ctx->tgt_index, d_tgt, nt, target_grid)) return s;
        if (tc_status s = wait_uploads(ctx)) return s;
        if (job.mode == 1)
            if (tc_status s = gather_normals(ctx, ctx->tgt_index, job.nrm, job.nstride)) return s;
    }
    if (tc_status s = wait_uploads(ctx)) return s;
    if (tc_status s = ensure(ctx, ctx->state, sizeof(IcpState))) return s;
    IcpState *hs = &pinned_host(ctx)->icp_staged;
    std::memset(hs, 0, sizeof(IcpState));
    for (int i = 0; i < 4; ++i) hs->q[i] = init[i];
    for (int i = 0; i < 3; ++i) hs->t[i] = init[4 + i];
    hs->prev_mse = INFINITY;
    hs->d_ang = -1.0f; hs->d_t = 0.0f; hs->d_run = 0;
    hs->conv_thr = job.conv_thr;
    hs->max_dist = job.max_dist;
    hs->kiss = job.kiss;
    hs->status = TC_OK;
    TC_HIP_TRY(ctx, hipMemcpyAsync(ctx->state.p, hs, sizeof(IcpState), hipMemcpyHostToDevice, ctx->stream));
    out.tg = plan_tiles((*out.tix).geom, ns);
    if (src_presorted && src_presorted->geom.n == ns) {
        out.src = (const float4 *)src_presorted->pts.p;
    } else {
        IndexSpec source_order;
        source_order.reuse_geom = &(*out.tix).geom; source_order.state_transform = (const IcpState *)ctx->state.p;
        source_order.tile_major = &out.tg; source_order.strict_order = strict_source_order;
        if (ns > 0)
            if (tc_status s = build_index(ctx, ctx->src_index, d_src, ns, source_order)) return s;
        out.src = (const float4 *)ctx->src_index.pts.p;
    }
    out.l = plan_launch(ns);
    if (tc_status s = ensure(ctx, ctx->partials, ((size_t)(kMaxPartialBlocks + kRefineBlocks) * TC_ICP_SUMS_STRIDE + 2) * sizeof(double))) return s;
    if (tc_status s = ensure(ctx, ctx->corr, (2 * ns + (size_t)kMaxPartialBlocks * (kIcpBlock / 64) + 4 + kRefineEntryWords * (size_t)out.l.nblocks * out.l.chunk) * sizeof(uint32_t))) return s;
    if (!out.tix->pts12_valid) {
        const uint32_t npad = (uint32_t)nt + 16u;
        if (tc_status s = ensure(ctx, out.tix->pts12, (size_t)npad * 12 + 64)) return s;
        ProfScope ps(ctx, "icp_pack12");
        hipLaunchKernelGGL(icp_pack12_kernel, dim3((npad + 255) / 256), dim3(256), 0, ctx->stream, (const float4 *)(*out.tix).pts.p, (uint32_t)nt, npad,
                           (float *)out.tix->pts12.p);
        out.tix->pts12_valid = true;
    }
    out.tv = view_of((*out.tix));
    if (tc_status s = ensure(ctx, ctx->icp_wsrc, 2 * (ns + 4) * sizeof(float4))) return s;
    out.wsrc = (float4 *)ctx->icp_wsrc.p;
    if (ns > 0) {
        ProfScope ps(ctx, "icp_working_source");
        hipLaunchKernelGGL(icp_working_source_kernel, dim3((unsigned)((ns + 255) / 256)), dim3(256), 0, ctx->stream, out.src, (uint32_t)ns, out.wsrc, (float4 *)nullptr);
    }
    out.ns = (uint32_t)ns;
    out.nrm = (const float4 *)out.tix->normals.p;
    out.st = (IcpState *)ctx->state.p;
    out.rlist = (uint32_t *)ctx->corr.p + 2 * ns;
    out.partials = (double *)ctx->partials.p;
    return TC_OK;
}

__global__ void __launch_bounds__(256) gather_cov_kernel(const float4 *__restrict__ pts_sorted, uint32_t n, const float4 *__restrict__ cov_orig,
                                                        float4 *__restrict__ out) {
    const uint32_t i = blockIdx.x * blockDim.x + threadIdx.x;
    if (i >= n) return;
    const uint32_t o = __float_as_uint(pts_sorted[i].w);
    out[2 * (size_t)i] = cov_orig[2 * (size_t)o];
    out[2 * (size_t)i + 1] = cov_orig[2 * (size_t)o + 1];
}

static void fold_search_stats(tc_context *ctx, const IcpState *hs) {
    if (!((debug_flags() & 8) || ctx->profiling == 3)) return;
    const uint32_t *h = hs->refine_ring_hist;
    unsigned long long needed;
    std::memcpy(&needed, &h[3], sizeof(needed));
    ctx->stat_icp[0] += hs->iterations; ctx->stat_icp[1] += h[5]; ctx->stat_icp[2] += h[6]; ctx->stat_icp[3] += h[7];
    ctx->stat_icp[4] += needed; ctx->stat_icp[5] += h[2];
    if (debug_flags() & 8)
        fprintf(stderr, "[tc] icp main pass over %u iterations: wave trips %u, without a search %u (%.1f %%); searches %u, candidate steps needed %llu "
                        "(%.2f per search), steps taken by the trips' slowest lanes %u (%.2f per searching trip): lock-step ratio (lane slots spent / steps needed) %.2f\n",
                hs->iterations, h[5], h[6], 100.0 * h[6] / std::max(h[5], 1u), h[7], needed, (double)needed / std::max(h[7], 1u), h[2],
                (double)h[2] / std::max(h[5] - h[6], 1u), (double)h[2] * 64.0 / std::max<double>((double)needed, 1.0));
}

static tc_status launch_finish(tc_context *ctx, const IcpSetup &su, uint32_t mse_blocks, int from_sums, bool via_staged_copy, const IcpState **out) {
    PinnedBlock *pb = pinned_host(ctx);
    IcpState *hs = via_staged_copy ? &pb->icp_staged : &pb->icp_result, *hs_dev = nullptr;
    if (!via_staged_copy) {
        hs_dev = (IcpState *)pinned_dev_ptr(ctx, hs);
        if (!hs_dev) return fail(ctx, TC_GPU, "ICP: the pinned block has no device address");
        hs->status = TC_GPU; hs->iterations = 0;
    }
    const bool direct = !via_staged_copy && pinned_poll_enabled();
    hipLaunchKernelGGL(icp_finish_kernel, dim3(1), dim3(64), 0, ctx->stream, su.st, (const double *)su.partials, mse_blocks, su.mode != 0 ? 1 : 0, from_sums,
                       direct ? hs_dev : (IcpState *)nullptr);
    if (!direct) TC_HIP_TRY(ctx, hipMemcpyAsync(hs, su.st, sizeof(IcpState), hipMemcpyDeviceToHost, ctx->stream));
    *out = hs;
    return TC_OK;
}

static tc_status fill_result(tc_context *ctx, const IcpState *hs, size_t max_iters, const char *failed, bool check_count, tc_icp_result *res) {
    if (hs->status != TC_OK) return fail(ctx, (tc_status)hs->status, failed);
    if (check_count && !hs->converged && hs->iterations != max_iters)
        return fail(ctx, TC_GPU, "internal error: the ICP loop executed " + std::to_string(hs->iterations) + " of " + std::to_string(max_iters) + " iterations");
    for (int i = 0; i < 4; ++i) res->transformation[i] = hs->q[i];
    for (int i = 0; i < 3; ++i) res->transformation[4 + i] = hs->t[i];
    res->mse = hs->mse;
    res->iterations = hs->converged ? hs->iterations : max_iters;
    res->converged = hs->converged;
    res->n_correspondences = hs->n_corr;
    return TC_OK;
}

template <typename F>
static tc_status run_chunked(tc_context *ctx, size_t max_iters, F &&enqueue_iteration) {
    auto chunk_len = [](size_t c) -> size_t { return c == 0 ? 6 : c == 1 ? 2 : c <= 4 ? 4 : 8; };
    size_t nchunks = 0;
    for (size_t covered = 0; covered < max_iters; ++nchunks) covered += chunk_len(nchunks);
    volatile int32_t *flags = pinned_host(ctx)->icp_flags;
    int32_t *d_flags = nullptr;
    TC_HIP_TRY(ctx, hipHostGetDevicePointer((void **)&d_flags, (void *)flags, 0));
    const size_t max_flags = kIcpMaxFlags;
    size_t it = 0;
    const bool sticky = ctx->icp_cert_hint && nchunks >= 3;
    ctx->icp_cert = sticky;
    struct Hint { tc_context *c; bool wanted; ~Hint() { c->icp_cert_hint = wanted; } } hint{ctx, sticky};
    for (size_t c = 0; c < nchunks; ++c) {
        if (c >= 2 && c - 2 < max_flags) {
            if (tc_status s = wait_pinned_word(ctx, (volatile uint32_t *)&flags[c - 2], "ICP loop")) return s;
            if (flags[c - 2] == 1) break;
            hint.wanted = flags[c - 2] == 3;
            ctx->icp_cert = sticky || hint.wanted;
        }
        if (c < max_flags) flags[c] = 0;
        for (size_t k = 0; k < chunk_len(c) && it < max_iters; ++k, ++it) {
            const bool last = k + 1 == chunk_len(c) || it + 1 == max_iters;
            if (tc_status s = enqueue_iteration((last && c < max_flags) ? d_flags + c : nullptr)) return s;
        }
    }
    return TC_OK;
}

static void dump_block_schedule(tc_context *ctx, uint32_t nblocks) {
    std::vector<unsigned long long> h(2 * (size_t)nblocks);
    (void)hipMemcpy(h.data(), ctx->dbg_times.p, h.size() * sizeof(unsigned long long), hipMemcpyDeviceToHost);
    unsigned long long t0 = ~0ull, t1 = 0;
    for (size_t b = 0; b < nblocks; ++b) { t0 = std::min(t0, h[2 * b]); t1 = std::max(t1, h[2 * b + 1]); }
    std::vector<double> dur, endt, startt;
    for (size_t b = 0; b < nblocks; ++b) { dur.push_back((h[2 * b + 1] - h[2 * b]) * 0.01); endt.push_back((h[2 * b + 1] - t0) * 0.01); startt.push_back((h[2 * b] - t0) * 0.01); }
    std::sort(dur.begin(), dur.end()); std::sort(endt.begin(), endt.end()); std::sort(startt.begin(), startt.end());
    auto q = [](const std::vector<double> &v, double f) { return v[(size_t)(f * (v.size() - 1))]; };
    fprintf(stderr, "[tc] main pass blocks: %u; span %.1f us; block duration us min %.1f p10 %.1f p50 %.1f p90 %.1f p99 %.1f max %.1f; start p50 %.1f p99 %.1f max %.1f; end p10 %.1f p50 %.1f p90 %.1f\n",
            nblocks, (t1 - t0) * 0.01, dur.front(), q(dur, 0.1), q(dur, 0.5), q(dur, 0.9), q(dur, 0.99), dur.back(), q(startt, 0.5), q(startt, 0.99), startt.back(),
            q(endt, 0.1), q(endt, 0.5), q(endt, 0.9));
#ifdef TC_PHASE_STAMPS
    {
        std::vector<unsigned long long> hp(8 * (size_t)nblocks);
        (void)hipMemcpy(hp.data(), (unsigned long long *)ctx->dbg_times.p + 2 * kMaxPartialBlocks, hp.size() * sizeof(unsigned long long), hipMemcpyDeviceToHost);
        double m[8] = {0};
        for (size_t b = 0; b < nblocks; ++b) for (int i = 0; i < 8; ++i) m[i] += (double)hp[8 * b + i] / nblocks;
        fprintf(stderr, "[tc]   wave 0 phases, mean s_memtime ticks: stage1-2 %.0f  windows %.0f  loop %.0f  post %.0f  stage4 %.0f  fold %.0f  end %.0f\n", m[0], m[1], m[2], m[3], m[4], m[5], m[6]);
    }
#endif
    fprintf(stderr, "[tc]   per XCD (block & 7): mean duration / last end, us:");
    for (int x = 0; x < 8; ++x) {
        double sum = 0, last = 0; int cnt = 0;
        for (size_t b = x; b < nblocks; b += 8) { sum += (h[2 * b + 1] - h[2 * b]) * 0.01; last = std::max(last, (h[2 * b + 1] - t0) * 0.01); ++cnt; }
        fprintf(stderr, " %.1f/%.1f", sum / std::max(cnt, 1), last);
    }
    fprintf(stderr, "\n");
}

tc_status icp_run(tc_context *ctx, const IcpJob &job, tc_icp_result *res) {
    const int mode = job.mode;
    const size_t ns = job.ns, nt = job.nt;
    IcpSetup su;
    if (tc_status s = icp_setup(ctx, job, mode == 2 ? nullptr : job.src_presorted, false, su)) return s;
    su.wl = su.wsrc + ns + 4;
    hipStream_t st = ctx->stream;
    uint32_t *corr = (uint32_t *)ctx->corr.p, *corr_pos = match_words(su.wsrc);
    if (mode == 2) {
        if (tc_status s = ensure(ctx, (*su.tix).normals, nt * 2 * sizeof(float4))) return s;
        if (tc_status s = ensure(ctx, ctx->gicp_src_cov, ns * 2 * sizeof(float4))) return s;
        hipLaunchKernelGGL(gather_cov_kernel, dim3((unsigned)((nt + 255) / 256)), dim3(256), 0, st, (const float4 *)(*su.tix).pts.p,
                           (uint32_t)nt, (const float4 *)job.cov_tgt, (float4 *)(*su.tix).normals.p);
        hipLaunchKernelGGL(gather_cov_kernel, dim3((unsigned)((ns + 255) / 256)), dim3(256), 0, st, su.src, (uint32_t)ns,
                           (const float4 *)job.cov_src, (float4 *)ctx->gicp_src_cov.p);
        su.src_cov = (const float4 *)ctx->gicp_src_cov.p;
        su.nrm = (const float4 *)(*su.tix).normals.p;
    }

    size_t enq = 0;
    const float4 *vor = su.tix->vor_valid ? (const float4 *)su.tix->vor.p : nullptr;
    if (debug_flags() & 1024)
        if (tc_status s = ensure(ctx, ctx->dbg_times, 10 * (size_t)kMaxPartialBlocks * sizeof(unsigned long long))) return s;
    if (tc_status s = run_chunked(ctx, job.max_iters, [&](int32_t *done_out) -> tc_status {
            if (enq++ == vor_after() && !vor)
                if (tc_status s = launch_target_nn_bounds(ctx, (*su.tix), su.tv, su.st, &vor)) return s;
            launch_iteration(ctx, su, IcpStep::FullIteration, vor, done_out, ctx->icp_cert);
            return TC_OK;
        })) return s;
    if (mode == 0) {
        ProfScope ps(ctx, "icp_final_mse");
        hipLaunchKernelGGL(icp_final_mse_kernel, dim3(su.l.mse_blocks), dim3(kIcpBlock), 0, st, su.tv, (const float4 *)su.wsrc, (uint32_t)ns,
                           su.l.mse_chunk, su.st, corr_pos, su.partials);
    }
    const IcpState *hs = nullptr;
    if (tc_status s = launch_finish(ctx, su, su.l.mse_blocks, 0, false, &hs)) return s;
    if (res->corr_target) {
        hipLaunchKernelGGL(icp_write_corr_kernel, dim3((unsigned)((ns + 255) / 256)), dim3(256), 0, st, su.tv, su.src, (uint32_t)ns,
                           corr_pos, job.corr_on_device ? res->corr_target : corr);
        if (!job.corr_on_device) TC_HIP_TRY(ctx, hipMemcpyAsync(res->corr_target, corr, ns * sizeof(uint32_t), hipMemcpyDeviceToHost, st));
    }
    TC_HIP_TRY(ctx, hipStreamSynchronize(st));
    TC_HIP_TRY(ctx, hipGetLastError());
    if ((debug_flags() & 1024) && ctx->dbg_times.p) dump_block_schedule(ctx, su.l.nblocks);
    fold_search_stats(ctx, hs);
    if (debug_flags() & 64)
        fprintf(stderr, "[tc] icp: searching lanes at the last evaluation of the certificate's gate %u (d_run %u, wanted %d)\n", hs->searchers, hs->d_run, hs->d_ang >= 0.0f ? 1 : 0);
    if (debug_flags() & 64)
        fprintf(stderr, "[tc] icp: %u iterations, refine queries total %u max %u  exit ring hist %u %u %u %u %u %u %u %u\n", hs->iterations,
                hs->refine_total, hs->refine_max, hs->refine_ring_hist[0], hs->refine_ring_hist[1], hs->refine_ring_hist[2], hs->refine_ring_hist[3],
                hs->refine_ring_hist[4], hs->refine_ring_hist[5], hs->refine_ring_hist[6], hs->refine_ring_hist[7]);
    return fill_result(ctx, hs, job.max_iters,
                       mode == 2 ? "GICP: insufficient correspondences (need >= 6) or ill-conditioned Gauss-Newton system"
                       : mode == 1 ? "Insufficient correspondences for point-to-plane ICP (need >= 6) or ill-conditioned system"
                                   : "Insufficient correspondences found", true, res);
}


__global__ void __launch_bounds__(256) icp_zero_u32_kernel(uint32_t *__restrict__ p, uint32_t n) {
    const uint32_t i = blockIdx.x * blockDim.x + threadIdx.x;
    if (i < n) p[i] = 0u;
}

tc_status icp_run_sharded(tc_context *ctx, tc_comm *comm, int shard_mode, const IcpJob &job, tc_icp_result *res) {
    const int mode = job.mode;
    const size_t ns = job.ns, max_iters = job.max_iters;
    const int W = comm ? comm->nranks : 1, rank = comm ? comm->rank : 0;
    IcpSetup su;
    const size_t rows = (ns + (size_t)W - 1) / (size_t)W;
    size_t ilo = 0, ihi = ns;
    if (shard_mode == TC_SHARD_INDEX) { ilo = std::min((size_t)rank * rows, ns); ihi = std::min(ilo + rows, ns); }
    const size_t n_setup = ihi - ilo;
    IcpJob mine = job;
    mine.src = job.src + 3 * ilo; mine.ns = n_setup;
    tc_status setup_rc = icp_setup(ctx, mine, nullptr, shard_mode == TC_SHARD_SPATIAL && W > 1, su);
    if (setup_rc == TC_OK && !su.tix->vor_valid) setup_rc = ensure(ctx, su.tix->vor, (size_t)su.tix->geom.n * sizeof(float4));
    const bool gather_index = shard_mode == TC_SHARD_INDEX && res->corr_target && ns > 0 && (W > 1 || (comm && comm->nccl));
    if (setup_rc == TC_OK && gather_index) setup_rc = ensure(ctx, ctx->out_a, (size_t)W * rows * sizeof(uint32_t));
    if (tc_status s = comm_agree(comm, setup_rc)) return s;
    hipStream_t st = ctx->stream;
    size_t lo = 0, hi = n_setup;
    if (shard_mode == TC_SHARD_SPATIAL) { lo = ns * (size_t)rank / (size_t)W; hi = ns * ((size_t)rank + 1) / (size_t)W; }
    const size_t nl = hi - lo;
    su.src += lo; su.wsrc += lo; su.ns = (uint32_t)nl; su.l = plan_launch(nl);
    const IcpLaunch &l = su.l;
    uint32_t *corr = (uint32_t *)ctx->corr.p, *corr_pos = match_words(su.wsrc);
    size_t enq = 0;
    const float4 *vor = su.tix->vor_valid ? (const float4 *)su.tix->vor.p : nullptr;
    if (tc_status s = run_chunked(ctx, max_iters, [&](int32_t *done_out) -> tc_status {
            if (enq++ == vor_after() && !vor)
                if (tc_status s = launch_target_nn_bounds(ctx, (*su.tix), su.tv, su.st, &vor)) return s;
            launch_iteration(ctx, su, IcpStep::ReduceSum, vor);
            if (tc_status s = comm_allreduce_f64(comm, su.st->sums, TC_ICP_SUMS_STRIDE)) return s;
            launch_iteration(ctx, su, IcpStep::ApplyOnly, nullptr, done_out);
            return TC_OK;
        })) return s;
    if (mode == 0) {
        hipLaunchKernelGGL(icp_final_mse_kernel, dim3(l.mse_blocks), dim3(kIcpBlock), 0, st, su.tv, (const float4 *)su.wsrc, (uint32_t)nl, l.mse_chunk, su.st,
                           corr_pos, su.partials);
        hipLaunchKernelGGL(icp_final_mse_fold_kernel, dim3(1), dim3(64), 0, st, su.st, su.partials, l.mse_blocks);
        if (tc_status s = comm_allreduce_f64(comm, su.st->sums, TC_ICP_SUMS_STRIDE)) return s;
    }
    const IcpState *hs = nullptr;
    if (tc_status s = launch_finish(ctx, su, 0u, 1, false, &hs)) return s;
    if (res->corr_target && ns > 0) {
        if (gather_index) {
            uint32_t *all = (uint32_t *)ctx->out_a.p;
            if (nl > 0)
                hipLaunchKernelGGL(icp_write_corr_kernel, dim3((unsigned)((nl + 255) / 256)), dim3(256), 0, st, su.tv, su.src, (uint32_t)nl, corr_pos,
                                   all + (size_t)rank * rows);
            if (tc_status s = comm_allgather(comm, all, rows * sizeof(uint32_t))) return s;
            TC_HIP_TRY(ctx, hipMemcpyAsync(res->corr_target, all, ns * sizeof(uint32_t), hipMemcpyDeviceToDevice, st));
        } else {
            const bool gather = shard_mode == TC_SHARD_SPATIAL && (W > 1 || (comm && comm->nccl));
            if (gather) hipLaunchKernelGGL(icp_zero_u32_kernel, dim3((unsigned)((ns + 255) / 256)), dim3(256), 0, st, corr, (uint32_t)ns);
            if (nl > 0)
                hipLaunchKernelGGL(icp_write_corr_kernel, dim3((unsigned)((nl + 255) / 256)), dim3(256), 0, st, su.tv, su.src, (uint32_t)nl, corr_pos, corr);
            if (gather)
                if (tc_status s = comm_allreduce_u32(comm, corr, ns)) return s;
            TC_HIP_TRY(ctx, hipMemcpyAsync(res->corr_target, corr, n_setup * sizeof(uint32_t), hipMemcpyDeviceToDevice, st));
        }
    }
    TC_HIP_TRY(ctx, hipStreamSynchronize(st));
    TC_HIP_TRY(ctx, hipGetLastError());
    fold_search_stats(ctx, hs);
    return fill_result(ctx, hs, max_iters, mode == 1 ? "Insufficient correspondences for point-to-plane ICP (need >= 6) or ill-conditioned system"
                                                     : "Insufficient correspondences found", true, res);
}

}

struct tc_icp_shard {
    tc_context *ctx;
    tc::IcpSetup su;
};

extern "C" {

tc_status tc_icp_shard_create(tc_context *ctx, int point_to_plane, const float *d_source_slice, size_t n_source_slice,
                              const float *d_target, size_t n_target, const float *d_target_normals, size_t normal_stride,
                              const float init[7], float max_correspondence_distance, float convergence_threshold,
                              tc_icp_shard **out) try {
    if (!ctx || !out) return TC_INVALID_DATA;
    if (n_source_slice == 0 || n_target == 0) return tc::fail(ctx, TC_INVALID_DATA, "Source or target point cloud is empty");
    if (!point_to_plane) return tc::fail(ctx, TC_UNSUPPORTED, "tc_icp_shard_*: point-to-plane only; use tc_sharded_icp_detailed_device");
    tc::IcpJob job;
    job.mode = 1;
    job.src = d_source_slice; job.ns = n_source_slice;
    job.tgt = d_target; job.nt = n_target;
    job.nrm = d_target_normals; job.nstride = normal_stride;
    job.init = init; job.max_dist = max_correspondence_distance; job.conv_thr = convergence_threshold;
    tc_icp_shard *s = new tc_icp_shard{ctx, {}};
    tc_status rc = tc::icp_setup(ctx, job, nullptr, false, s->su);
    if (rc != TC_OK) { delete s; return rc; }
    *out = s;
    return TC_OK;
} TC_CATCH_STATUS(ctx)

double *tc_icp_shard_sums(tc_icp_shard *s) { return ((tc::IcpState *)s->ctx->state.p)->sums; }

tc_status tc_icp_shard_get_sums(tc_icp_shard *s, double *d_out) try {
    tc_context *ctx = s->ctx;
    TC_HIP_TRY(ctx, hipMemcpyAsync(d_out, ((tc::IcpState *)ctx->state.p)->sums, TC_ICP_SUMS_STRIDE * sizeof(double),
                                   hipMemcpyDeviceToDevice, ctx->stream));
    return TC_OK;
} TC_CATCH_STATUS((s ? s->ctx : nullptr))

tc_status tc_icp_shard_set_sums(tc_icp_shard *s, const double *d_in) try {
    tc_context *ctx = s->ctx;
    TC_HIP_TRY(ctx, hipMemcpyAsync(((tc::IcpState *)ctx->state.p)->sums, d_in, TC_ICP_SUMS_STRIDE * sizeof(double),
                                   hipMemcpyDeviceToDevice, ctx->stream));
    return TC_OK;
} TC_CATCH_STATUS((s ? s->ctx : nullptr))

tc_status tc_icp_shard_done(tc_icp_shard *s, int *done) try {
    tc_context *ctx = s->ctx;
    if (tc_status rc = tc::read_back(ctx, &tc::pinned_host(ctx)->count, &((tc::IcpState *)ctx->state.p)->done, sizeof(int32_t))) return rc;
    *done = (int32_t)tc::pinned_host(ctx)->count;
    return TC_OK;
} TC_CATCH_STATUS((s ? s->ctx : nullptr))

tc_status tc_icp_shard_reduce(tc_icp_shard *s) try {
    tc_context *ctx = s->ctx;
    tc::launch_iteration(ctx, s->su, tc::IcpStep::ReduceSum);
    TC_HIP_TRY(ctx, hipGetLastError());
    return TC_OK;
} TC_CATCH_STATUS((s ? s->ctx : nullptr))

tc_status tc_icp_shard_apply(tc_icp_shard *s) try {
    tc_context *ctx = s->ctx;
    tc::launch_iteration(ctx, s->su, tc::IcpStep::ApplyOnly);
    TC_HIP_TRY(ctx, hipGetLastError());
    return TC_OK;
} TC_CATCH_STATUS((s ? s->ctx : nullptr))

tc_status tc_icp_shard_finish(tc_icp_shard *s, size_t max_iters, tc_icp_result *res) try {
    tc_context *ctx = s->ctx;
    hipStream_t st = ctx->stream;
    const tc::IcpSetup &su = s->su;
    const tc::IcpState *hs = nullptr;
    if (tc_status rc = tc::launch_finish(ctx, su, 0u, 0, true, &hs)) return rc;
    if (res->corr_target) {
        uint32_t *corr = (uint32_t *)ctx->corr.p;
        hipLaunchKernelGGL(tc::icp_write_corr_kernel, dim3((unsigned)((su.ns + 255) / 256)), dim3(256), 0, st, su.tv, su.src, su.ns,
                           tc::match_words(su.wsrc), corr);
        TC_HIP_TRY(ctx, hipMemcpyAsync(res->corr_target, corr, su.ns * sizeof(uint32_t), hipMemcpyDeviceToDevice, st));
    }
    TC_HIP_TRY(ctx, hipStreamSynchronize(st));
    tc::fold_search_stats(ctx, hs);
    return tc::fill_result(ctx, hs, max_iters, "ICP failed (insufficient correspondences / singular system)", false, res);
} TC_CATCH_STATUS((s ? s->ctx : nullptr))

void tc_icp_shard_destroy(tc_icp_shard *s) { delete s; }

}
```

### threecrate_amd/csrc/tc_internal.h

```cpp
#pragma once
#include <hip/hip_runtime.h>
#include <stddef.h>
#include <stdint.h>
#include <new>
#include <exception>
#include <string>
#include <type_traits>
#include <vector>

#include "../../include/threecrate_hip.h"

namespace tc {

struct GridGeom {
    float minx, miny, minz;
    float maxx, maxy, maxz;
    float h, inv_h;
    int   gx, gy, gz;
    uint32_t ncell;
    uint32_t n;
    float cx, cy, cz;
    int   clamped;
};

struct TileGeom {
    int tx, ty, tz;
    int ntx, nty, ntz;
    uint32_t cpt;
    uint32_t ntiles;
};

struct GridView {
    GridGeom g;
    const float4   *pts;
    const uint32_t *cell_start;
    const float    *pts12;
};

struct IcpState {
    float    q[4];
    float    t[3];
    float    prev_mse;
    float    mse;
    uint32_t iterations;
    int32_t  converged;
    int32_t  status;
    int32_t  done;
    uint32_t n_corr;
    float    conv_thr;
    float    max_dist;
    int32_t  kiss;
    uint32_t refine_total;
    uint32_t refine_max;
    uint32_t refine_ring_hist[8];
    float    d_ang;
    float    d_t;
    uint32_t d_run;
    uint32_t searchers;
    double   sums[TC_ICP_SUMS_STRIDE];
};

static_assert(offsetof(IcpState, refine_ring_hist) % 8 == 4 && offsetof(IcpState, sums) % 8 == 0,
              "refine_ring_hist[3..4] is ONE 64-bit counter of the statistics instantiation (icp.hip): it must sit on an 8-byte boundary");

struct PlaneOut {
    float    coeff[4];
    uint32_t count, index;
    uint32_t found, pad;
};

struct NdtState {
    float    q[4], t[3];
    float    rot[9];
    float    score;
    uint32_t iterations;
    int32_t  converged;
    int32_t  done;
    uint32_t n_hits;
    float    step_size, epsilon;
    uint32_t pad;
};
static_assert(sizeof(NdtState) == 96, "");
struct NdtBuildOut {
    int32_t  kmin[3], kmax[3];
    uint32_t n_finite, n_runs, n_voxels, pad[7];
};
static_assert(sizeof(NdtBuildOut) == 64, "");

struct TsdfOut {
    uint32_t n_updated;
    uint32_t n_points;
    uint32_t pad[14];
};
static_assert(sizeof(TsdfOut) == 64, "");

struct RansacOut {
    float    transform[12];
    uint32_t count, index;
    uint32_t found;
    uint32_t exit;
};
static_assert(sizeof(RansacOut) == 64, "");

struct VoxelMapOut {
    uint32_t runs;
    uint32_t out_of_range;
    uint32_t n_long;
    uint32_t n_new;
    uint32_t pad[12];
};
static_assert(sizeof(VoxelMapOut) == 64, "");

constexpr int kColorSlices = 16;
struct ColorOut {
    uint32_t slice[kColorSlices];
};
static_assert(sizeof(ColorOut) == 64, "");

struct MeshOut {
    uint32_t bad_index;
    uint32_t n_long;
    uint32_t n_entries;
    uint32_t pad[13];
};
static_assert(sizeof(MeshOut) == 64, "");

struct SimplifyOut {
    uint32_t flags;
    uint32_t n_long;
    uint32_t n_out_vertices;
    uint32_t n_out_faces;
    uint32_t pad[12];
};
static_assert(sizeof(SimplifyOut) == 64, "");

struct McOut {
    uint32_t n_cubes;
    uint32_t n_vertices;
    uint32_t n_faces;
    uint32_t pad[13];
};
static_assert(sizeof(McOut) == 64, "");

constexpr size_t kIcpMaxFlags = 200;
struct PinnedBlock {
    char     reserved[256];
    IcpState icp_staged;
    IcpState icp_result;
    union {
        volatile int32_t icp_flags[kIcpMaxFlags];
        uint32_t count;
        uint32_t filter_out[2];
        PlaneOut plane_out;
    };
    char     pad_flags[1024 - kIcpMaxFlags * sizeof(int32_t)];
    float    bbox[30];
    char     pad_bbox[8192 - 30 * sizeof(float)];
    volatile uint32_t occ[2];
    char     pad_occ[56];
    uint32_t big_cell;
    char     pad_big[60];
    uint32_t agree;
    char     pad_agree[60];
    volatile uint32_t bbox_done;
    char     pad_done[60];
    volatile uint32_t bin_max[2];
    char     pad_bin[56];
    NdtBuildOut ndt_build;
    NdtState ndt_state;
    TsdfOut  tsdf_out;
    RansacOut ransac_out;
    VoxelMapOut voxelmap_out;
    ColorOut color_out;
    MeshOut  mesh_out;
    SimplifyOut simplify_out;
    McOut    mc_out;
};
constexpr size_t kPinnedBytes = 1 << 16;
static_assert(offsetof(PinnedBlock, icp_staged) == 256 && offsetof(PinnedBlock, icp_result) == 640 && offsetof(PinnedBlock, icp_flags) == 1024 &&
              offsetof(PinnedBlock, count) == 1024 && offsetof(PinnedBlock, filter_out) == 1024 && offsetof(PinnedBlock, plane_out) == 1024 &&
              sizeof(PlaneOut) <= sizeof(PinnedBlock::icp_flags) && offsetof(PinnedBlock, bbox) == 2048 && offsetof(PinnedBlock, occ) == 2048 + 8192 &&
              offsetof(PinnedBlock, big_cell) == 2048 + 8192 + 64 && offsetof(PinnedBlock, agree) == 2048 + 8192 + 128 &&
              offsetof(PinnedBlock, bbox_done) == 2048 + 8192 + 192 && offsetof(PinnedBlock, bin_max) == 2048 + 8192 + 256 &&
              offsetof(PinnedBlock, ndt_build) == 2048 + 8192 + 320 && offsetof(PinnedBlock, ndt_state) == 2048 + 8192 + 384 &&
              offsetof(PinnedBlock, tsdf_out) == 2048 + 8192 + 480 && offsetof(PinnedBlock, ransac_out) == 2048 + 8192 + 544 &&
              offsetof(PinnedBlock, voxelmap_out) == 2048 + 8192 + 608 && offsetof(PinnedBlock, color_out) == 2048 + 8192 + 672 &&
              offsetof(PinnedBlock, mesh_out) == 2048 + 8192 + 736 && offsetof(PinnedBlock, simplify_out) == 2048 + 8192 + 800 &&
              offsetof(PinnedBlock, mc_out) == 2048 + 8192 + 864,
              "a region of the pinned block has moved");
static_assert(offsetof(PinnedBlock, icp_result) - offsetof(PinnedBlock, icp_staged) >= sizeof(IcpState) &&
              offsetof(PinnedBlock, icp_flags) - offsetof(PinnedBlock, icp_result) >= sizeof(IcpState),
              "an IcpState slot of the pinned block is too small: the staged state would run into the result, the result into the chunk flags");
static_assert(sizeof(PinnedBlock::icp_flags) == kIcpMaxFlags * sizeof(int32_t) &&
              offsetof(PinnedBlock, icp_flags) + sizeof(PinnedBlock::icp_flags) <= offsetof(PinnedBlock, bbox), "the chunk flags run into the bounding box");
static_assert(sizeof(PinnedBlock) <= kPinnedBytes, "the pinned block outgrew its allocation");
constexpr int kIcpBlock = 256;
constexpr int kTsdfBlock = 256, kTsdfRun = 64;
constexpr size_t kTsdfMaxVoxels = (size_t)1 << 28;
constexpr size_t kPtsPad = 4, kCellStartPad = 4;
constexpr size_t kCellStartFront = 4;
constexpr uint32_t kRankQuadraticMax = 1u << 20;
constexpr int kMaxPartialBlocks = 1024;
constexpr uint32_t kAdaptMinPoints = 1u << 18;

#if defined(__HIPCC__)
__device__ __forceinline__ uint32_t tile_major_id(const TileGeom &t, int cx, int cy, int cz) {
    const int ax = cx / t.tx, ay = cy / t.ty, az = cz / t.tz;
    const int lx = cx - ax * t.tx, ly = cy - ay * t.ty, lz = cz - az * t.tz;
    const uint32_t tile = ((uint32_t)az * t.nty + ay) * t.ntx + ax;
    return tile * t.cpt + ((uint32_t)lz * t.ty + ly) * t.tx + lx;
}
__device__ __forceinline__ float d2_nc(float ax, float ay, float az, float bx, float by, float bz) {
    float dx = ax - bx, dy = ay - by, dz = az - bz;
    return dx * dx + dy * dy + dz * dz;
}
__device__ __forceinline__ int cell_coord(float v, float mn, float inv_h, int g) {
    float f = (v - mn) * inv_h;
    int c = (f >= 0.0f) ? (int)f : 0;
    return c < g ? c : g - 1;
}
__device__ __forceinline__ void isometry_apply(const float q[4], const float t[3], float x, float y, float z,
                                               float &ox, float &oy, float &oz) {
    float tx = (q[1] * z - q[2] * y) * 2.0f;
    float ty = (q[2] * x - q[0] * z) * 2.0f;
    float tz = (q[0] * y - q[1] * x) * 2.0f;
    float cx = q[1] * tz - q[2] * ty;
    float cy = q[2] * tx - q[0] * tz;
    float cz = q[0] * ty - q[1] * tx;
    ox = ((tx * q[3] + cx) + x) + t[0];
    oy = ((ty * q[3] + cy) + y) + t[1];
    oz = ((tz * q[3] + cz) + z) + t[2];
}
__device__ __forceinline__ void store_compacted(const float *__restrict__ xyz, uint32_t i, uint32_t o, float *__restrict__ out_xyz,
                                                uint32_t *__restrict__ out_index) {
    if (out_xyz) {
        out_xyz[3 * (size_t)o] = xyz[3 * (size_t)i]; out_xyz[3 * (size_t)o + 1] = xyz[3 * (size_t)i + 1]; out_xyz[3 * (size_t)o + 2] = xyz[3 * (size_t)i + 2];
    }
    if (out_index) out_index[o] = i;
}
typedef float f32x3 __attribute__((ext_vector_type(3)));
__device__ __forceinline__ __amdgpu_buffer_rsrc_t raw_rsrc(const void *p) {
    return __builtin_amdgcn_make_buffer_rsrc(const_cast<void *>(p), 0, 0xFFFFFFFF, 0x00020000);
}
#endif

struct DevBuf {
    void  *p = nullptr;
    size_t cap = 0;
};

struct ScopedBuf : DevBuf {
    ScopedBuf() = default;
    ScopedBuf(const ScopedBuf &) = delete; ScopedBuf &operator=(const ScopedBuf &) = delete;
    ~ScopedBuf() { if (p) (void)hipFree(p); }
};

struct KernelTimer {
    std::string name;
    std::vector<std::pair<hipEvent_t, hipEvent_t>> pending;
    uint64_t launches = 0;
    double   total_ms = 0.0;
    double   min_ms = 1e300, max_ms = 0.0;
};

struct DeviceIndex {
    GridGeom geom{};
    TileGeom tile{};
    float exact_min[3] = {0, 0, 0}, exact_max[3] = {0, 0, 0};
    DevBuf pts;
    DevBuf cell_start;
    DevBuf normals;
    DevBuf vor;
    bool vor_valid = false;
    DevBuf pts12;
    bool pts12_valid = false;
    uint32_t occ_host = 0;
    bool occ_host_valid = false;
    DevBuf cell_of;
    DevBuf slot;
    DevBuf arrival;
    DevBuf fill;
    DevBuf blocksum;
};
struct IndexSpec {
    float cell_factor = 0.0f;
    float min_cell_edge = 0.0f;
    float target_ppo = 0.0f;
    const GridGeom *reuse_geom = nullptr;
    const IcpState *state_transform = nullptr;
    const TileGeom *tile_major = nullptr;
    bool strict_order = false;
};
__host__ __device__ inline int ball_rings(const GridGeom &g, float radius) {
    const int gyz = g.gy > g.gz ? g.gy : g.gz;
    return (int)fminf(ceilf(radius * g.inv_h) + 1.0f, (float)(g.gx > gyz ? g.gx : gyz));
}
template <class F> void for_each_scratch_buf(DeviceIndex &ix, F f) { for (DevBuf *b : {&ix.cell_of, &ix.slot, &ix.arrival, &ix.fill, &ix.blocksum}) f(*b); }
template <class F> void for_each_buf(DeviceIndex &ix, F f) {
    for (DevBuf *b : {&ix.pts, &ix.cell_start, &ix.normals, &ix.vor, &ix.pts12}) f(*b);
    for_each_scratch_buf(ix, f);
}

enum CluSlot {
    CLU_PARENT, CLU_SIZE, CLU_MIN_INDEX,
    CLU_FLAG, CLU_POS,
    CLU_KEYS,
    CLU_ROOTS,
    CLU_RANK_OF, CLU_SIZES,
    CLU_LABELS, CLU_SORT_TEMP, CLU_COMP,
    CLU_SLOTS
};
enum FpfhSlot {
    FPFH_XYZ, FPFH_SPFH, FPFH_MODE,
    FPFH_FB_POS, FPFH_FB_XYZ, FPFH_FB_COUNT,
    FPFH_SORTED_OF,
    FPFH_KNN_IDX, FPFH_KNN_DIST, FPFH_KNN_COUNT,
    FPFH_SLOTS
};

enum VoxSlot {
    VOX_KEYS,
    VOX_KEYS_SORTED,
    VOX_INDEX,
    VOX_ORDER,
    VOX_FLAG,
    VOX_POS,
    VOX_START,
    VOX_SORT_TEMP,
    VOX_BLOCKSUM,
    VOX_SLOTS
};

}

struct tc_context {
    int device = 0;
    hipStream_t stream = nullptr;
    bool own_stream = true;
    std::string last_error;
    int profiling = 0;
    uint32_t prof_tick = 0;
    std::vector<tc::KernelTimer> timers;
    std::vector<hipEvent_t> event_pool;
    std::vector<tc::DevBuf> pool;
    size_t pool_bytes = 0;
    size_t pool_largest = 0;
    hipEvent_t order_event = nullptr;
    hipEvent_t release_event = nullptr;
    std::vector<hipEvent_t> chunk_events;
    hipStream_t copy_stream = nullptr;
    hipEvent_t upload_event = nullptr;
    bool upload_pending = false;
    bool upload_used_copy_stream = false;

    tc::DeviceIndex tgt_index;
    tc::DeviceIndex src_index;
    tc::DevBuf in_a, in_b, in_c;
    tc::DevBuf out_a;
    tc::DevBuf bbox;
    tc::DevBuf state;
    tc::DevBuf partials;
    tc::DevBuf corr;
    tc::DevBuf gicp_src_cov;
    tc::DevBuf icp_wsrc;
    tc::DevBuf dbg_times;
    tc::DevBuf overflow;
    tc::DevBuf build_tmp;
    tc::DevBuf normals_hard;
    unsigned long long stat_indexed_points = 0, stat_index_builds = 0;
    unsigned long long stat_icp[6] = {0, 0, 0, 0, 0, 0};
    bool icp_cert = false;
    bool icp_cert_hint = false;
    bool normals_hard_clean = false;
    tc::DevBuf vox[tc::VOX_SLOTS];
    tc::DevBuf clu[tc::CLU_SLOTS];
    tc::DevBuf fpfh[tc::FPFH_SLOTS];
    tc::DevBuf fpfh_np;
    void *pinned = nullptr;
    void *pinned_dev = nullptr;
};
template <class F> void for_each_buf(tc_context &c, F f) {
    for (tc::DeviceIndex *ix : {&c.tgt_index, &c.src_index}) tc::for_each_buf(*ix, f);
    for (auto &b : c.vox) f(b);
    for (auto &b : c.clu) f(b);
    for (auto &b : c.fpfh) f(b);
    for (tc::DevBuf *b : {&c.fpfh_np, &c.in_a, &c.in_b, &c.in_c, &c.out_a, &c.bbox, &c.state, &c.partials, &c.corr, &c.gicp_src_cov,
                          &c.overflow, &c.normals_hard, &c.build_tmp, &c.dbg_times, &c.icp_wsrc}) f(*b);
}

struct tc_comm {
    tc_context *ctx = nullptr;
    int rank = 0, nranks = 1;
    void *nccl = nullptr;
    bool own_nccl = false;
    tc_host_collective_fn host_fn = nullptr;
    void *host_user = nullptr;
    void *agree_word = nullptr;
};

namespace tc {

tc_status fail(tc_context *ctx, tc_status st, const std::string &msg);
tc_status fail_nothrow(tc_context *ctx, tc_status st, const char *msg) noexcept;
void fault_point(const char *site);
#define TC_CATCH_STATUS(CTX)                                                                                            \
    catch (const std::bad_alloc &) { return tc::fail_nothrow((CTX), TC_GPU, "out of host memory"); }                    \
    catch (const std::exception &e_) { return tc::fail_nothrow((CTX), TC_GPU, e_.what()); }                             \
    catch (...) { return tc::fail_nothrow((CTX), TC_GPU, "unknown C++ exception"); }
#define TC_CATCH_VOID catch (...) { }
#define TC_CATCH_VALUE(V) catch (...) { return V; }
#define TC_HIP_TRY(ctx, expr)                                                                  \
    do {                                                                                       \
        hipError_t _e = (expr);                                                                \
        if (_e != hipSuccess)                                                                  \
            return tc::fail((ctx), TC_GPU, std::string(#expr) + ": " + hipGetErrorString(_e)); \
    } while (0)

tc_status ensure(tc_context *ctx, DevBuf &b, size_t bytes);
constexpr size_t kMaxPoints = 0xFFFFFFF0ull, kMaxK = 2048;
inline tc_status check_point_count(tc_context *ctx, size_t a, size_t b = 0) {
    return (a >= kMaxPoints || b >= kMaxPoints) ? fail(ctx, TC_UNSUPPORTED, "more than 2^32 points") : TC_OK;
}
tc_status upload_async(tc_context *ctx, void *d_dst, const void *h_src, size_t bytes);
tc_status uploads_issued(tc_context *ctx);
tc_status wait_uploads(tc_context *ctx);
inline PinnedBlock *pinned_host(tc_context *ctx) { return static_cast<PinnedBlock *>(ctx->pinned); }
void *pinned_dev_ptr(tc_context *ctx, const void *host_addr);
bool pinned_poll_enabled();
tc_status wait_pinned_word(tc_context *ctx, volatile uint32_t *word, const char *what);
tc_status read_back(tc_context *ctx, void *host_dst, const void *dev_src, size_t bytes);
tc_status stage_in(tc_context *ctx, DevBuf &b, const void *h_src, size_t bytes);
tc_status synced(tc_context *ctx);
tc_status stage_out(tc_context *ctx, void *h_dst, const void *d_src, size_t bytes);
void recycle(tc_context *ctx, DevBuf &b);

struct ProfScope {
    tc_context *ctx; int idx = -1; hipEvent_t e0 = nullptr, e1 = nullptr; bool ext = false;
    ProfScope(tc_context *c, const char *name, bool dominant = false);
    ~ProfScope();
    bool active() const { return idx >= 0; }
};

tc_status build_index(tc_context *ctx, DeviceIndex &ix, const float *d_xyz, size_t n, const IndexSpec &spec);
TileGeom make_tiles(const GridGeom &g, int tx, int ty, int tz);
tc_status gather_normals(tc_context *ctx, DeviceIndex &ix, const float *d_normals, size_t stride);
GridView view_of(const DeviceIndex &ix);
template <class F> void with_clamped(const GridView &gv, F launch) {
    if (gv.g.clamped) launch(std::true_type{});
    else launch(std::false_type{});
}

tc_status exclusive_scan_u32(tc_context *ctx, const uint32_t *d_in, uint32_t n, uint32_t *d_out , DevBuf &blocksum, uint32_t *occ_out = nullptr,
                             unsigned long long *occ_host = nullptr);
tc_status cloud_bbox(tc_context *ctx, const float *d_xyz, size_t n, float mn[3], float mx[3]);
tc_status compact_flagged(tc_context *ctx, const float *d_xyz, uint32_t n, const uint32_t *d_flag, uint32_t *d_pos, DevBuf &blocksum, float *d_out_xyz,
                          uint32_t *d_out_index);

unsigned bits_for_value(uint64_t v);
template <class K>
tc_status sort_pairs(tc_context *ctx, const K *keys, K *keys_out, const uint32_t *vals, uint32_t *vals_out, size_t n, unsigned end_bit, DevBuf &temp);
tc_status key_runs(tc_context *ctx, const uint64_t *keys_sorted, uint32_t n, uint32_t *head, uint32_t *runpos, uint32_t *rstart, DevBuf &blocksum);
struct GroupBufs { DevBuf &keys_sorted, &vals_sorted, &head, &runpos, &rstart, &sort_temp, &blocksum; };
struct KeyGroups {
    const uint64_t *keys_sorted;
    const uint32_t *order;
    uint32_t *head, *runpos;
    const uint32_t *rstart;
    const uint32_t *n_runs;
};
tc_status group_by_key(tc_context *ctx, const uint64_t *keys, const uint32_t *vals, size_t n, unsigned key_bits, const GroupBufs &b, KeyGroups &g, size_t room = 0);
inline unsigned blocks_for(size_t n) { return (unsigned)((n + 255) / 256); }

tc_status voxel_filter_device(tc_context *ctx, const float *d_xyz, size_t n, float voxel, float *d_out, size_t *n_out);
tc_status range_filter_device(tc_context *ctx, const float *d_xyz, size_t n, float min_range, float max_range, float *d_out, size_t *n_out);

tc_status cluster_extract_device(tc_context *ctx, const float *d_xyz, size_t n, float tol, size_t min_size, size_t max_size,
                                 uint32_t *d_labels, uint32_t *d_members, uint64_t *d_offsets, size_t *n_clusters);

tc_status fpfh_device(tc_context *ctx, const float *d_np6, size_t n, float radius, size_t k, float *d_out);

tc_status sor_device(tc_context *ctx, const float *d_xyz, size_t n, size_t k, bool with_threshold, float param, float *d_out_xyz,
                     uint32_t *d_kept_index, float *d_mean, size_t *n_out, float *threshold_used);
tc_status radius_outlier_device(tc_context *ctx, const float *d_xyz, size_t n, float radius, size_t min_neighbors, float *d_out_xyz,
                                uint32_t *d_kept_index, size_t *n_out);

tc_status plane_segment_device(tc_context *ctx, const float *d_xyz, size_t n, float threshold, const uint32_t *d_samples, size_t n_samples,
                               uint64_t state0, float *coefficients, uint32_t *d_inlier_index, size_t *n_inliers, uint32_t *best_iteration);

tc_status launch_normals(tc_context *ctx, const DeviceIndex &ix, const float *d_xyz, const tc_normal_config &cfg,
                         const float vp[3], float *d_out6, size_t p_begin = 0, size_t p_end = (size_t)-1, bool slice_out = false,
                         float4 *d_sorted_nrm = nullptr, float4 *d_vor = nullptr);
tc_status normals_on_index(tc_context *ctx, DeviceIndex &ix, bool build, float cell_factor_override, const float *d_xyz, size_t n,
                           const tc_normal_config *cfg, float *d_out6, size_t p_begin, size_t p_end, bool slice_out, float4 *d_sorted_nrm,
                           bool with_bounds = false);
float normals_cell_factor(size_t k, bool large);
float normals_target_ppo(size_t k);
IndexSpec knn_grid(size_t list_len);
IndexSpec ball_grid(float radius, bool finite_only);
constexpr float kIcpCellFactor = 1.13f;
void free_buf(DevBuf &b);
void free_index(DeviceIndex &ix);
void recycle_index(tc_context *ctx, DeviceIndex &ix);
tc_status launch_normals_unsort(tc_context *ctx, const DeviceIndex &ix, const float *d_sorted6, float *d_out6);

tc_status launch_radius_all(tc_context *ctx, const DeviceIndex &ix, const float *d_queries, size_t nq, float radius, uint32_t *d_counts,
                            const unsigned long long *d_offsets, uint32_t *d_idx, float *d_dist);
tc_status launch_knn(tc_context *ctx, const DeviceIndex &ix, const float *d_queries, size_t nq, size_t k,
                     uint32_t *d_idx, float *d_dist, uint32_t *d_count, float radius_sq = INFINITY);

int debug_flags();

tc_status comm_allreduce_f64(tc_comm *comm, double *d_buf, size_t count);
tc_status comm_allreduce_u32(tc_comm *comm, uint32_t *d_buf, size_t count);
tc_status comm_allgather(tc_comm *comm, void *d_buf, size_t bytes_per_rank);
tc_status comm_agree(tc_comm *comm, tc_status local);

struct IcpJob {
    int mode = 0;
    const float *src = nullptr, *tgt = nullptr;
    size_t ns = 0, nt = 0;
    const float *nrm = nullptr;
    size_t nstride = 0;
    const float *cov_src = nullptr, *cov_tgt = nullptr;
    const float *init = nullptr;
    size_t max_iters = 0;
    float max_dist = -1.0f, conv_thr = 0.0f;
    int kiss = 0;
    bool corr_on_device = true;
    DeviceIndex *tgt_prebuilt = nullptr;
    const DeviceIndex *src_presorted = nullptr;
};
tc_status icp_run(tc_context *ctx, const IcpJob &job, tc_icp_result *res);
tc_status icp_run_sharded(tc_context *ctx, tc_comm *comm, int shard_mode, const IcpJob &job, tc_icp_result *res);

}
```

Before: 17820 it/s.

## Fuse pts12 packing and ICP working-source init into index placement kernels

The index-building placement kernels (bin_place, rerank) can now also write the packed 12-byte point copy and the ICP working-source copy, and initialise the ICP state words on the device. This replaces the separate pack12 and working_source kernel launches and the host staging copy of the initial state. The start transform is passed by value as a kernel argument instead of being read from a device state pointer. The intent is to remove extra full passes over the point array and some launch and transfer overhead during setup. In exchange the placement kernels become templated and do more stores, and strict-order builds still fall back to the separate kernels.

```diff
diff --git a/threecrate_amd/csrc/api.hip b/threecrate_amd/csrc/api.hip
--- a/threecrate_amd/csrc/api.hip
+++ b/threecrate_amd/csrc/api.hip
@@ -504,6 +504,34 @@
     return which == TC_COUNTER_INDEXED_POINTS ? ctx->stat_indexed_points : which == TC_COUNTER_INDEX_BUILDS ? ctx->stat_index_builds : 0ull;
 } TC_CATCH_VALUE(0)
 
+#ifdef TC_DEV
+tc_status tcdev_index_layouts(tc_context *ctx, const float *d_xyz, size_t n, int fused, int strict, const float start7[7], float *h_pts,
+                               float *h_pts12, float *h_working, uint32_t *h_state, int *written) try {
+    if (!ctx || !d_xyz || n == 0 || !start7 || !written) return TC_INVALID_DATA;
+    TC_HIP_TRY(ctx, hipSetDevice(ctx->device));
+    if (tc_status s = tc::ensure(ctx, ctx->state, sizeof(tc::IcpState))) return s;
+    if (tc_status s = tc::ensure(ctx, ctx->icp_wsrc, 2 * (n + 4) * sizeof(float4))) return s;
+    TC_HIP_TRY(ctx, hipMemsetAsync(ctx->state.p, 0xA5, sizeof(tc::IcpState), ctx->stream));
+    tc::IndexSpec spec; spec.cell_factor = tc::kIcpCellFactor; spec.target_ppo = 2.5f; spec.strict_order = strict != 0;
+    for (int i = 0; i < 4; ++i) spec.start.q[i] = start7[i];
+    for (int i = 0; i < 3; ++i) spec.start.t[i] = start7[4 + i];
+    spec.start.conv_thr = 1e-6f; spec.start.max_dist = 0.5f; spec.start.kiss = 1;
+    if (fused) { spec.pack12 = true; spec.working_copy = (float4 *)ctx->icp_wsrc.p; spec.fresh_state = (tc::IcpState *)ctx->state.p; }
+    tc::DeviceIndex &ix = ctx->src_index;
+    if (tc_status s = tc::build_index(ctx, ix, d_xyz, n, spec)) return s;
+    *written = (ix.pts12_valid ? 1 : 0) | (ix.working_copy_written ? 2 : 0);
+    if (!ix.pts12_valid) if (tc_status s = tc::pack12(ctx, ix)) return s;
+    if (!ix.working_copy_written)
+        if (tc_status s = tc::working_source(ctx, (const float4 *)ix.pts.p, n, (float4 *)ctx->icp_wsrc.p, (tc::IcpState *)ctx->state.p, spec.start)) return s;
+    TC_HIP_TRY(ctx, hipMemcpyAsync(h_pts, ix.pts.p, n * sizeof(float4), hipMemcpyDeviceToHost, ctx->stream));
+    TC_HIP_TRY(ctx, hipMemcpyAsync(h_pts12, ix.pts12.p, (n + tc::kPts12Pad) * 12, hipMemcpyDeviceToHost, ctx->stream));
+    TC_HIP_TRY(ctx, hipMemcpyAsync(h_working, ctx->icp_wsrc.p, n * sizeof(float4), hipMemcpyDeviceToHost, ctx->stream));
+    TC_HIP_TRY(ctx, hipMemcpyAsync(h_state, ctx->state.p, sizeof(tc::IcpState), hipMemcpyDeviceToHost, ctx->stream));
+    TC_HIP_TRY(ctx, hipStreamSynchronize(ctx->stream));
+    return TC_OK;
+} TC_CATCH_STATUS(ctx)
+#endif
+
 void tc_profile_enable(tc_context *ctx, int on) {
     if (!ctx) return;
     ctx->profiling = on;
diff --git a/threecrate_amd/csrc/cloud.hip b/threecrate_amd/csrc/cloud.hip
--- a/threecrate_amd/csrc/cloud.hip
+++ b/threecrate_amd/csrc/cloud.hip
@@ -49,7 +49,7 @@
         c->has_normals6 = true;
     }
     c->has_normals = false;
-    IndexSpec spec; spec.cell_factor = f; spec.min_cell_edge = min_h; spec.target_ppo = target_ppo;
+    IndexSpec spec; spec.cell_factor = f; spec.min_cell_edge = min_h; spec.target_ppo = target_ppo; spec.pack12 = true;
     if (tc_status s = build_index(ctx, c->ix, (const float *)c->xyz.p, c->n, spec)) return s;
     c->indexed = true;
     c->factor = f;
diff --git a/threecrate_amd/csrc/grid.hip b/threecrate_amd/csrc/grid.hip
--- a/threecrate_amd/csrc/grid.hip
+++ b/threecrate_amd/csrc/grid.hip
@@ -114,8 +114,39 @@
 }
 
 
+struct KeyMove {
+    int on;
+    float q[4], t[3];
+};
+__device__ __forceinline__ void key_move(const KeyMove &mv, float &x, float &y, float &z) {
+    if (mv.on) {
+        float ox, oy, oz;
+        isometry_apply(mv.q, mv.t, x, y, z, ox, oy, oz);
+        x = ox; y = oy; z = oz;
+    }
+}
+
+constexpr int kOutPack12 = 1, kOutWorking = 2;
+struct PlaceExtra {
+    float    *pts12;
+    float4   *working;
+    IcpState *state;
+    IcpStart  start;
+    uint32_t  n;
+};
+template <int OUT>
+__device__ __forceinline__ void store_extra(const PlaceExtra &ex, uint32_t p, const float4 &r) {
+    if constexpr ((OUT & kOutPack12) != 0) { ex.pts12[3 * (size_t)p] = r.x; ex.pts12[3 * (size_t)p + 1] = r.y; ex.pts12[3 * (size_t)p + 2] = r.z; }
+    if constexpr ((OUT & kOutWorking) != 0) ex.working[p] = make_float4(r.x, r.y, r.z, __uint_as_float(0xFFFFFFFFu));
+}
+template <int OUT>
+__device__ __forceinline__ void store_extra_once(const PlaceExtra &ex, uint32_t t) {
+    if constexpr ((OUT & kOutPack12) != 0) { if (t < 3 * kPts12Pad) reinterpret_cast<uint32_t *>(ex.pts12)[3 * (size_t)ex.n + t] = 0x7F7F7F7Fu; }
+    if constexpr ((OUT & kOutWorking) != 0) { if (ex.state && t < kIcpStateWords) reinterpret_cast<uint32_t *>(ex.state)[t] = icp_state_word(ex.start, t); }
+}
+
 __global__ void __launch_bounds__(256) cell_hist_kernel(const float *__restrict__ xyz, uint32_t n, GridGeom g,
-                                                       const IcpState *__restrict__ st, TileGeom tg, int tile_major, uint32_t nkeys,
+                                                       KeyMove mv, TileGeom tg, int tile_major, uint32_t nkeys,
                                                        uint32_t *__restrict__ cell_of, uint32_t *__restrict__ hist,
                                                        uint32_t *__restrict__ arrival, uint32_t *__restrict__ pts_pad,
                                                        uint32_t *__restrict__ cs_front, uint32_t *__restrict__ cs_tail, uint32_t rank_max) {
@@ -128,12 +159,7 @@
     }
     if (i >= n) return;
     float x = xyz[3 * (size_t)i], y = xyz[3 * (size_t)i + 1], z = xyz[3 * (size_t)i + 2];
-    if (st) {
-        float q[4] = {st->q[0], st->q[1], st->q[2], st->q[3]}, t[3] = {st->t[0], st->t[1], st->t[2]};
-        float ox, oy, oz;
-        isometry_apply(q, t, x, y, z, ox, oy, oz);
-        x = ox; y = oy; z = oz;
-    }
+    key_move(mv, x, y, z);
     int ix = cell_coord(x, g.minx, g.inv_h, g.gx);
     int iy = cell_coord(y, g.miny, g.inv_h, g.gy);
     int iz = cell_coord(z, g.minz, g.inv_h, g.gz);
@@ -288,21 +314,18 @@
     tmp[pos] = r;
 }
 
-__global__ void __launch_bounds__(256) rerank_kernel(uint32_t n, GridGeom g, const IcpState *__restrict__ st, TileGeom tg, int tile_major,
+template <int OUT>
+__global__ void __launch_bounds__(256) rerank_kernel(uint32_t n, GridGeom g, KeyMove mv, TileGeom tg, int tile_major,
                                                     uint32_t nkeys, const uint32_t *__restrict__ cell_start, const float4 *__restrict__ tmp,
-                                                    float4 *__restrict__ pts, uint32_t rank_max) {
+                                                    float4 *__restrict__ pts, uint32_t rank_max, PlaceExtra ex) {
     const uint32_t p = blockIdx.x * blockDim.x + threadIdx.x;
+    if constexpr (OUT != 0) { if (blockIdx.x == 0) store_extra_once<OUT>(ex, threadIdx.x); }
     if (p >= n) return;
     const float4 r = tmp[p];
     uint32_t c;
     {
         float x = r.x, y = r.y, z = r.z;
-        if (st) {
-            float q[4] = {st->q[0], st->q[1], st->q[2], st->q[3]}, t[3] = {st->t[0], st->t[1], st->t[2]};
-            float ox, oy, oz;
-            isometry_apply(q, t, x, y, z, ox, oy, oz);
-            x = ox; y = oy; z = oz;
-        }
+        key_move(mv, x, y, z);
         const int ix = cell_coord(x, g.minx, g.inv_h, g.gx), iy = cell_coord(y, g.miny, g.inv_h, g.gy), iz = cell_coord(z, g.minz, g.inv_h, g.gz);
         c = tile_major ? tile_major_id(tg, ix, iy, iz) : ((uint32_t)iz * g.gy + iy) * g.gx + ix;
         if (!(fabsf(x) <= 3.0e38f && fabsf(y) <= 3.0e38f && fabsf(z) <= 3.0e38f)) c = nkeys;
@@ -318,6 +341,7 @@
         rank = p - s;
     }
     pts[s + rank] = r;
+    store_extra<OUT>(ex, s + rank, r);
 }
 
 __global__ void __launch_bounds__(256) gather_normals_kernel(const float4 *__restrict__ pts, uint32_t n,
@@ -554,21 +578,16 @@
 constexpr uint32_t kBinMaxBins = 8192;
 constexpr int kBinPlaceThreads = TC_BIN_PLACE_THREADS;
 
-__device__ __forceinline__ uint32_t point_key(float x, float y, float z, const GridGeom &g, const IcpState *__restrict__ st, const TileGeom &tg,
+__device__ __forceinline__ uint32_t point_key(float x, float y, float z, const GridGeom &g, const KeyMove &mv, const TileGeom &tg,
                                               int tile_major, uint32_t nkeys) {
-    if (st) {
-        float q[4] = {st->q[0], st->q[1], st->q[2], st->q[3]}, t[3] = {st->t[0], st->t[1], st->t[2]};
-        float ox, oy, oz;
-        isometry_apply(q, t, x, y, z, ox, oy, oz);
-        x = ox; y = oy; z = oz;
-    }
+    key_move(mv, x, y, z);
     const int ix = cell_coord(x, g.minx, g.inv_h, g.gx), iy = cell_coord(y, g.miny, g.inv_h, g.gy), iz = cell_coord(z, g.minz, g.inv_h, g.gz);
     uint32_t c = tile_major ? tile_major_id(tg, ix, iy, iz) : ((uint32_t)iz * g.gy + iy) * g.gx + ix;
     if (!(fabsf(x) <= 3.0e38f && fabsf(y) <= 3.0e38f && fabsf(z) <= 3.0e38f)) c = nkeys;
     return c;
 }
 
-__global__ void __launch_bounds__(kBinWalkThreads) bin_count_kernel(const float *__restrict__ xyz, uint32_t n, GridGeom g, const IcpState *__restrict__ st,
+__global__ void __launch_bounds__(kBinWalkThreads) bin_count_kernel(const float *__restrict__ xyz, uint32_t n, GridGeom g, KeyMove mv,
                                                        TileGeom tg, int tile_major, uint32_t nkeys, uint32_t kpb, uint32_t nbins,
                                                        uint32_t *__restrict__ cnt , uint32_t *__restrict__ pts_pad,
                                                        uint32_t *__restrict__ cs_front, uint32_t *__restrict__ cs_tail) {
@@ -584,7 +603,7 @@
     const uint32_t per = (n + kBinBlocks - 1) / kBinBlocks;
     const uint32_t i0 = blockIdx.x * per, i1 = min(i0 + per, n);
     for (uint32_t i = i0 + threadIdx.x; i < i1; i += kBinWalkThreads) {
-        const uint32_t k = point_key(xyz[3 * (size_t)i], xyz[3 * (size_t)i + 1], xyz[3 * (size_t)i + 2], g, st, tg, tile_major, nkeys);
+        const uint32_t k = point_key(xyz[3 * (size_t)i], xyz[3 * (size_t)i + 1], xyz[3 * (size_t)i + 2], g, mv, tg, tile_major, nkeys);
         atomicAdd(&c[min(k / kpb, nbins - 1u)], 1u);
     }
     __syncthreads();
@@ -609,7 +628,7 @@
     if (lane == 63u) tot[b] = inc;
 }
 
-__global__ void __launch_bounds__(kBinWalkThreads) bin_scatter_kernel(const float *__restrict__ xyz, uint32_t n, GridGeom g, const IcpState *__restrict__ st,
+__global__ void __launch_bounds__(kBinWalkThreads) bin_scatter_kernel(const float *__restrict__ xyz, uint32_t n, GridGeom g, KeyMove mv,
                                                          TileGeom tg, int tile_major, uint32_t nkeys, uint32_t kpb, uint32_t nbins,
                                                          const uint32_t *__restrict__ off ,
                                                          const uint32_t *__restrict__ tot, uint32_t *__restrict__ binstart,
@@ -661,19 +680,20 @@
     for (uint32_t i = i0 + threadIdx.x; i < i1; i += kBinWalkThreads) {
         float4 r;
         r.x = xyz[3 * (size_t)i]; r.y = xyz[3 * (size_t)i + 1]; r.z = xyz[3 * (size_t)i + 2];
-        const uint32_t k = point_key(r.x, r.y, r.z, g, st, tg, tile_major, nkeys);
+        const uint32_t k = point_key(r.x, r.y, r.z, g, mv, tg, tile_major, nkeys);
         if (k == nkeys) r.x = r.y = r.z = __uint_as_float(0x7F7F7F7Fu);
         r.w = __uint_as_float(i);
         tmp[atomicAdd(&cur[min(k / kpb, nbins - 1u)], 1u)] = r;
     }
 }
 
+template <int OUT>
 __global__ void __launch_bounds__(kBinPlaceThreads) bin_place_kernel(const float4 *__restrict__ tmp, const uint32_t *__restrict__ binstart,
                                                                      uint32_t nbins, uint32_t kpb, uint32_t nkeys, GridGeom g,
-                                                                     const IcpState *__restrict__ st, TileGeom tg, int tile_major,
+                                                                     KeyMove mv, TileGeom tg, int tile_major,
                                                                      uint32_t *__restrict__ cs, float4 *__restrict__ pts,
                                                                      uint32_t *__restrict__ occ_ticket, uint32_t *__restrict__ occ_out,
-                                                                     unsigned long long *__restrict__ occ_host) {
+                                                                     unsigned long long *__restrict__ occ_host, PlaceExtra ex) {
     __shared__ uint32_t cnt[kBinKeysMax];
     __shared__ uint32_t rkey[kBinCap];
     __shared__ uint32_t ridx[kBinCap];
@@ -689,7 +709,7 @@
     __syncthreads();
     for (uint32_t i = tid; i < P; i += kBinPlaceThreads) {
         const float4 r = tmp[bs + i];
-        const uint32_t k = min(point_key(r.x, r.y, r.z, g, st, tg, tile_major, nkeys) - k0, K - 1u);
+        const uint32_t k = min(point_key(r.x, r.y, r.z, g, mv, tg, tile_major, nkeys) - k0, K - 1u);
         const uint32_t a = atomicAdd(&cnt[k], 1u);
         rkey[i] = k | (a << 16);
         ridx[i] = __float_as_uint(r.w);
@@ -737,7 +757,16 @@
     __syncthreads();
     for (uint32_t i = tid; i < P; i += kBinPlaceThreads) slot[rkey[i]] = i;
     __syncthreads();
-    for (uint32_t t = tid; t < P; t += kBinPlaceThreads) pts[bs + t] = tmp[bs + slot[t]];
+    if constexpr (OUT == 0) {
+        for (uint32_t t = tid; t < P; t += kBinPlaceThreads) pts[bs + t] = tmp[bs + slot[t]];
+    } else {
+        if (bin == 0) store_extra_once<OUT>(ex, tid);
+        for (uint32_t t = tid; t < P; t += kBinPlaceThreads) {
+            const float4 r = tmp[bs + slot[t]];
+            pts[bs + t] = r;
+            store_extra<OUT>(ex, bs + t, r);
+        }
+    }
     if (tid == 0) {
         const unsigned long long mine = ((unsigned long long)s_occ << 32) | 1ull;
         const unsigned long long old = __hip_atomic_fetch_add(reinterpret_cast<unsigned long long *>(occ_ticket), mine, __ATOMIC_RELAXED, __HIP_MEMORY_SCOPE_AGENT);
@@ -766,11 +795,26 @@
     ix.vor_valid = false;
     ix.pts12_valid = false;
     ix.occ_host_valid = false;
+    ix.working_copy_written = false;
     hipStream_t st = ctx->stream;
     const uint32_t n32 = (uint32_t)n;
     const int nb = (int)((n + 255) / 256);
     const int dbg = debug_flags();
     const uint32_t rank_max = rank_quadratic_max();
+    KeyMove mv{};
+    if (spec.moved) {
+        mv.on = 1;
+        for (int i = 0; i < 4; ++i) mv.q[i] = spec.start.q[i];
+        for (int i = 0; i < 3; ++i) mv.t[i] = spec.start.t[i];
+    }
+    const int out = spec.strict_order ? 0 : (spec.pack12 ? kOutPack12 : 0) | (spec.working_copy ? kOutWorking : 0);
+    PlaceExtra ex{};
+    if (out & kOutPack12) {
+        if (tc_status s = ensure(ctx, ix.pts12, pts12_bytes(n))) return s;
+        ex.pts12 = (float *)ix.pts12.p;
+    }
+    if (out & kOutWorking) { ex.working = spec.working_copy; ex.state = spec.fresh_state; ex.start = spec.start; }
+    ex.n = n32;
 
     if (spec.reuse_geom) {
         ix.geom = *spec.reuse_geom;
@@ -833,7 +877,7 @@
                 h_max[0] = 0u; h_max[1] = 0u;
                 {
                     ProfScope ps(ctx, "cell_bin_count");
-                    hipLaunchKernelGGL(bin_count_kernel, dim3(kBinBlocks), dim3(kBinWalkThreads), 0, st, d_xyz, n32, g, spec.state_transform, tg, spec.tile_major ? 1 : 0, nkeys, kpb,
+                    hipLaunchKernelGGL(bin_count_kernel, dim3(kBinBlocks), dim3(kBinWalkThreads), 0, st, d_xyz, n32, g, mv, tg, spec.tile_major ? 1 : 0, nkeys, kpb,
                                        nbins, cnt, reinterpret_cast<uint32_t *>((float4 *)ix.pts.p + n), (uint32_t *)ix.cell_start.p, cs + nkeys + 2);
                 }
                 {
@@ -843,16 +887,18 @@
                 if (tc_status s = ensure(ctx, ctx->build_tmp, (n + kPtsPad) * sizeof(float4))) return s;
                 {
                     ProfScope ps(ctx, "cell_bin_scatter");
-                    hipLaunchKernelGGL(bin_scatter_kernel, dim3(kBinBlocks), dim3(kBinWalkThreads), 0, st, d_xyz, n32, g, spec.state_transform, tg, spec.tile_major ? 1 : 0, nkeys,
+                    hipLaunchKernelGGL(bin_scatter_kernel, dim3(kBinBlocks), dim3(kBinWalkThreads), 0, st, d_xyz, n32, g, mv, tg, spec.tile_major ? 1 : 0, nkeys,
                                        kpb, nbins, (const uint32_t *)cnt, (const uint32_t *)tot, binstart, occ_ticket, d_max, (float4 *)ctx->build_tmp.p);
                 }
                 if (check) { h_occ[0] = 0u; h_occ[1] = 0u; }
                 unsigned long long *d_occ_host = check ? (unsigned long long *)pinned_dev_ptr(ctx, (const void *)h_occ) : nullptr;
                 {
                     ProfScope ps(ctx, "cell_bin_place");
-                    hipLaunchKernelGGL(bin_place_kernel, dim3(nbins), dim3(kBinPlaceThreads), 0, st, (const float4 *)ctx->build_tmp.p, (const uint32_t *)binstart,
-                                       nbins, kpb, nkeys, g, spec.state_transform, tg, spec.tile_major ? 1 : 0, cs, (float4 *)ix.pts.p, occ_ticket,
-                                       (uint32_t *)ix.cell_start.p, d_occ_host);
+                    auto place = out == 0 ? bin_place_kernel<0> : out == kOutPack12 ? bin_place_kernel<kOutPack12>
+                               : out == kOutWorking ? bin_place_kernel<kOutWorking> : bin_place_kernel<kOutPack12 | kOutWorking>;
+                    hipLaunchKernelGGL(place, dim3(nbins), dim3(kBinPlaceThreads), 0, st, (const float4 *)ctx->build_tmp.p, (const uint32_t *)binstart,
+                                       nbins, kpb, nkeys, g, mv, tg, spec.tile_major ? 1 : 0, cs, (float4 *)ix.pts.p, occ_ticket,
+                                       (uint32_t *)ix.cell_start.p, d_occ_host, ex);
                 }
                 TC_HIP_TRY(ctx, hipGetLastError());
                 if (tc_status s = wait_pinned_word(ctx, h_max + 1, "index build (bin populations)")) return s;
@@ -867,7 +913,7 @@
         TC_HIP_TRY(ctx, hipMemsetAsync(ix.fill.p, 0, fill_bytes, st));
         {
             ProfScope ps(ctx, "cell_hist");
-            hipLaunchKernelGGL(cell_hist_kernel, dim3(nb), dim3(256), 0, st, d_xyz, n32, g, spec.state_transform, tg, spec.tile_major ? 1 : 0, nkeys,
+            hipLaunchKernelGGL(cell_hist_kernel, dim3(nb), dim3(256), 0, st, d_xyz, n32, g, mv, tg, spec.tile_major ? 1 : 0, nkeys,
                                (uint32_t *)ix.cell_of.p, (uint32_t *)ix.fill.p, (uint32_t *)ix.arrival.p,
                                reinterpret_cast<uint32_t *>((float4 *)ix.pts.p + n), (uint32_t *)ix.cell_start.p, cs + nkeys + 2, rank_max);
         }
@@ -886,8 +932,10 @@
         }
         {
             ProfScope ps(ctx, "cell_rerank");
-            hipLaunchKernelGGL(rerank_kernel, dim3(nb), dim3(256), 0, st, n32, g, spec.state_transform, tg, spec.tile_major ? 1 : 0, nkeys, (const uint32_t *)cs,
-                               (const float4 *)ctx->build_tmp.p, (float4 *)ix.pts.p, rank_max);
+            auto rerank = out == 0 ? rerank_kernel<0> : out == kOutPack12 ? rerank_kernel<kOutPack12>
+                        : out == kOutWorking ? rerank_kernel<kOutWorking> : rerank_kernel<kOutPack12 | kOutWorking>;
+            hipLaunchKernelGGL(rerank, dim3(nb), dim3(256), 0, st, n32, g, mv, tg, spec.tile_major ? 1 : 0, nkeys, (const uint32_t *)cs,
+                               (const float4 *)ctx->build_tmp.p, (float4 *)ix.pts.p, rank_max, ex);
         }
         }
         TC_HIP_TRY(ctx, hipGetLastError());
@@ -914,6 +962,8 @@
         ix.geom = ng;
         ix.occ_host_valid = false;
     }
+    ix.pts12_valid = (out & kOutPack12) != 0;
+    ix.working_copy_written = (out & kOutWorking) != 0;
     if (spec.strict_order) {
         if (tc_status s = read_back(ctx, &pinned_host(ctx)->big_cell, (const uint32_t *)ix.fill.p + nkeys_final + 1, sizeof(uint32_t))) return s;
         if (pinned_host(ctx)->big_cell) {
diff --git a/threecrate_amd/csrc/icp.hip b/threecrate_amd/csrc/icp.hip
--- a/threecrate_amd/csrc/icp.hip
+++ b/threecrate_amd/csrc/icp.hip
@@ -1623,8 +1623,19 @@
     out[3 * (size_t)i] = r.x; out[3 * (size_t)i + 1] = r.y; out[3 * (size_t)i + 2] = r.z;
 }
 
-__global__ void __launch_bounds__(256) icp_working_source_kernel(const float4 *__restrict__ src, uint32_t n, float4 *__restrict__ out, float4 *__restrict__ wl) {
+tc_status pack12(tc_context *ctx, DeviceIndex &ix) {
+    const uint32_t n = ix.geom.n, npad = n + kPts12Pad;
+    if (tc_status s = ensure(ctx, ix.pts12, pts12_bytes(n))) return s;
+    ProfScope ps(ctx, "icp_pack12");
+    hipLaunchKernelGGL(icp_pack12_kernel, dim3((npad + 255) / 256), dim3(256), 0, ctx->stream, (const float4 *)ix.pts.p, n, npad, (float *)ix.pts12.p);
+    ix.pts12_valid = true;
+    return TC_OK;
+}
+
+__global__ void __launch_bounds__(256) icp_working_source_kernel(const float4 *__restrict__ src, uint32_t n, float4 *__restrict__ out, float4 *__restrict__ wl,
+                                                                IcpState *__restrict__ st, IcpStart start) {
     const uint32_t i = blockIdx.x * blockDim.x + threadIdx.x;
+    if (st && i < kIcpStateWords) reinterpret_cast<uint32_t *>(st)[i] = icp_state_word(start, i);
     if (i >= n) return;
     if (wl) wl[i] = make_float4(0.f, 0.f, 0.f, 0.f);
     float4 r = src[i];
@@ -1632,7 +1643,14 @@
     out[i] = r;
 }
 
-static tc_status icp_setup(tc_context *ctx, const IcpJob &job, const DeviceIndex *src_presorted, bool strict_source_order, IcpSetup &out) {
+tc_status working_source(tc_context *ctx, const float4 *src, size_t n, float4 *out, IcpState *st, const IcpStart &start) {
+    ProfScope ps(ctx, "icp_working_source");
+    hipLaunchKernelGGL(icp_working_source_kernel, dim3((unsigned)((n + 255) / 256)), dim3(256), 0, ctx->stream, src, (uint32_t)n, out, (float4 *)nullptr, st, start);
+    TC_HIP_TRY(ctx, hipGetLastError());
+    return TC_OK;
+}
+
+static tc_status icp_setup(tc_context *ctx, const IcpJob &job, const DeviceIndex *src_presorted, bool strict_source_order, bool fused_source, IcpSetup &out) {
     const float *d_src = job.src, *d_tgt = job.tgt, *init = job.init;
     const size_t ns = job.ns, nt = job.nt;
     DeviceIndex *tgt_prebuilt = job.tgt_prebuilt;
@@ -1640,7 +1658,7 @@
     if (nt >= (1ull << 28) || ns >= (1ull << 28)) return fail(ctx, TC_UNSUPPORTED, "ICP clouds are limited to 2^28 - 1 points");
     out.tix = tgt_prebuilt ? tgt_prebuilt : &ctx->tgt_index;
     if (!tgt_prebuilt) {
-        IndexSpec target_grid; target_grid.cell_factor = kIcpCellFactor; target_grid.target_ppo = 2.5f;
+        IndexSpec target_grid; target_grid.cell_factor = kIcpCellFactor; target_grid.target_ppo = 2.5f; target_grid.pack12 = true;
         if (tc_status s = build_index(ctx, ctx->tgt_index, d_tgt, nt, target_grid)) return s;
         if (tc_status s = wait_uploads(ctx)) return s;
         if (job.mode == 1)
@@ -1648,24 +1666,21 @@
     }
     if (tc_status s = wait_uploads(ctx)) return s;
     if (tc_status s = ensure(ctx, ctx->state, sizeof(IcpState))) return s;
-    IcpState *hs = &pinned_host(ctx)->icp_staged;
-    std::memset(hs, 0, sizeof(IcpState));
-    for (int i = 0; i < 4; ++i) hs->q[i] = init[i];
-    for (int i = 0; i < 3; ++i) hs->t[i] = init[4 + i];
-    hs->prev_mse = INFINITY;
-    hs->d_ang = -1.0f; hs->d_t = 0.0f; hs->d_run = 0;
-    hs->conv_thr = job.conv_thr;
-    hs->max_dist = job.max_dist;
-    hs->kiss = job.kiss;
-    hs->status = TC_OK;
-    TC_HIP_TRY(ctx, hipMemcpyAsync(ctx->state.p, hs, sizeof(IcpState), hipMemcpyHostToDevice, ctx->stream));
+    IcpStart start{};
+    for (int i = 0; i < 4; ++i) start.q[i] = init[i];
+    for (int i = 0; i < 3; ++i) start.t[i] = init[4 + i];
+    start.conv_thr = job.conv_thr; start.max_dist = job.max_dist; start.kiss = job.kiss;
+    if (tc_status s = ensure(ctx, ctx->icp_wsrc, 2 * (ns + 4) * sizeof(float4))) return s;
+    out.wsrc = (float4 *)ctx->icp_wsrc.p;
     out.tg = plan_tiles((*out.tix).geom, ns);
-    if (src_presorted && src_presorted->geom.n == ns) {
+    const bool src_presorted_used = src_presorted && src_presorted->geom.n == ns;
+    if (src_presorted_used) {
         out.src = (const float4 *)src_presorted->pts.p;
     } else {
         IndexSpec source_order;
-        source_order.reuse_geom = &(*out.tix).geom; source_order.state_transform = (const IcpState *)ctx->state.p;
+        source_order.reuse_geom = &(*out.tix).geom; source_order.moved = true; source_order.start = start;
         source_order.tile_major = &out.tg; source_order.strict_order = strict_source_order;
+        if (fused_source) { source_order.working_copy = out.wsrc; source_order.fresh_state = (IcpState *)ctx->state.p; }
         if (ns > 0)
             if (tc_status s = build_index(ctx, ctx->src_index, d_src, ns, source_order)) return s;
         out.src = (const float4 *)ctx->src_index.pts.p;
@@ -1673,20 +1688,17 @@
     out.l = plan_launch(ns);
     if (tc_status s = ensure(ctx, ctx->partials, ((size_t)(kMaxPartialBlocks + kRefineBlocks) * TC_ICP_SUMS_STRIDE + 2) * sizeof(double))) return s;
     if (tc_status s = ensure(ctx, ctx->corr, (2 * ns + (size_t)kMaxPartialBlocks * (kIcpBlock / 64) + 4 + kRefineEntryWords * (size_t)out.l.nblocks * out.l.chunk) * sizeof(uint32_t))) return s;
-    if (!out.tix->pts12_valid) {
-        const uint32_t npad = (uint32_t)nt + 16u;
-        if (tc_status s = ensure(ctx, out.tix->pts12, (size_t)npad * 12 + 64)) return s;
-        ProfScope ps(ctx, "icp_pack12");
-        hipLaunchKernelGGL(icp_pack12_kernel, dim3((npad + 255) / 256), dim3(256), 0, ctx->stream, (const float4 *)(*out.tix).pts.p, (uint32_t)nt, npad,
-                           (float *)out.tix->pts12.p);
-        out.tix->pts12_valid = true;
-    }
+    if (!out.tix->pts12_valid)
+        if (tc_status s = pack12(ctx, *out.tix)) return s;
     out.tv = view_of((*out.tix));
-    if (tc_status s = ensure(ctx, ctx->icp_wsrc, 2 * (ns + 4) * sizeof(float4))) return s;
-    out.wsrc = (float4 *)ctx->icp_wsrc.p;
-    if (ns > 0) {
-        ProfScope ps(ctx, "icp_working_source");
-        hipLaunchKernelGGL(icp_working_source_kernel, dim3((unsigned)((ns + 255) / 256)), dim3(256), 0, ctx->stream, out.src, (uint32_t)ns, out.wsrc, (float4 *)nullptr);
+    const bool fused = !src_presorted_used && ns > 0 && ctx->src_index.working_copy_written;
+    if (ns > 0 && !fused)
+        if (tc_status s = working_source(ctx, out.src, ns, out.wsrc, (IcpState *)ctx->state.p, start)) return s;
+    if (ns == 0) {
+        IcpState *hs = &pinned_host(ctx)->icp_staged;
+        uint32_t *hw = reinterpret_cast<uint32_t *>(hs);
+        for (uint32_t w = 0; w < kIcpStateWords; ++w) hw[w] = icp_state_word(start, w);
+        TC_HIP_TRY(ctx, hipMemcpyAsync(ctx->state.p, hs, sizeof(IcpState), hipMemcpyHostToDevice, ctx->stream));
     }
     out.ns = (uint32_t)ns;
     out.nrm = (const float4 *)out.tix->normals.p;
@@ -1811,7 +1823,7 @@
     const int mode = job.mode;
     const size_t ns = job.ns, nt = job.nt;
     IcpSetup su;
-    if (tc_status s = icp_setup(ctx, job, mode == 2 ? nullptr : job.src_presorted, false, su)) return s;
+    if (tc_status s = icp_setup(ctx, job, mode == 2 ? nullptr : job.src_presorted, false, true, su)) return s;
     su.wl = su.wsrc + ns + 4;
     hipStream_t st = ctx->stream;
     uint32_t *corr = (uint32_t *)ctx->corr.p, *corr_pos = match_words(su.wsrc);
@@ -1881,7 +1893,7 @@
     const size_t n_setup = ihi - ilo;
     IcpJob mine = job;
     mine.src = job.src + 3 * ilo; mine.ns = n_setup;
-    tc_status setup_rc = icp_setup(ctx, mine, nullptr, shard_mode == TC_SHARD_SPATIAL && W > 1, su);
+    tc_status setup_rc = icp_setup(ctx, mine, nullptr, shard_mode == TC_SHARD_SPATIAL && W > 1, false, su);
     if (setup_rc == TC_OK && !su.tix->vor_valid) setup_rc = ensure(ctx, su.tix->vor, (size_t)su.tix->geom.n * sizeof(float4));
     const bool gather_index = shard_mode == TC_SHARD_INDEX && res->corr_target && ns > 0 && (W > 1 || (comm && comm->nccl));
     if (setup_rc == TC_OK && gather_index) setup_rc = ensure(ctx, ctx->out_a, (size_t)W * rows * sizeof(uint32_t));
@@ -1959,7 +1971,7 @@
     job.nrm = d_target_normals; job.nstride = normal_stride;
     job.init = init; job.max_dist = max_correspondence_distance; job.conv_thr = convergence_threshold;
     tc_icp_shard *s = new tc_icp_shard{ctx, {}};
-    tc_status rc = tc::icp_setup(ctx, job, nullptr, false, s->su);
+    tc_status rc = tc::icp_setup(ctx, job, nullptr, false, false, s->su);
     if (rc != TC_OK) { delete s; return rc; }
     *out = s;
     return TC_OK;
diff --git a/threecrate_amd/csrc/tc_internal.h b/threecrate_amd/csrc/tc_internal.h
--- a/threecrate_amd/csrc/tc_internal.h
+++ b/threecrate_amd/csrc/tc_internal.h
@@ -62,6 +62,23 @@
 
 static_assert(offsetof(IcpState, refine_ring_hist) % 8 == 4 && offsetof(IcpState, sums) % 8 == 0,
               "refine_ring_hist[3..4] is ONE 64-bit counter of the statistics instantiation (icp.hip): it must sit on an 8-byte boundary");
+
+struct IcpStart {
+    float   q[4], t[3];
+    float   conv_thr, max_dist;
+    int32_t kiss;
+};
+constexpr uint32_t kIcpStateWords = sizeof(IcpState) / 4;
+static_assert(sizeof(IcpState) % 4 == 0 && kIcpStateWords <= 256, "a fresh state is stored by one block, a word per thread");
+static_assert(TC_OK == 0, "a fresh state's status word is zero");
+__host__ __device__ inline uint32_t icp_state_word(const IcpStart &s, uint32_t w) {
+    const float f = w == offsetof(IcpState, q) / 4 ? s.q[0] : w == offsetof(IcpState, q) / 4 + 1 ? s.q[1] : w == offsetof(IcpState, q) / 4 + 2 ? s.q[2]
+                  : w == offsetof(IcpState, q) / 4 + 3 ? s.q[3] : w == offsetof(IcpState, t) / 4 ? s.t[0] : w == offsetof(IcpState, t) / 4 + 1 ? s.t[1]
+                  : w == offsetof(IcpState, t) / 4 + 2 ? s.t[2] : w == offsetof(IcpState, prev_mse) / 4 ? INFINITY
+                  : w == offsetof(IcpState, conv_thr) / 4 ? s.conv_thr : w == offsetof(IcpState, max_dist) / 4 ? s.max_dist
+                  : w == offsetof(IcpState, d_ang) / 4 ? -1.0f : 0.0f;
+    return w == offsetof(IcpState, kiss) / 4 ? (uint32_t)s.kiss : __builtin_bit_cast(uint32_t, f);
+}
 
 struct PlaneOut {
     float    coeff[4];
@@ -199,6 +216,8 @@
 constexpr size_t kTsdfMaxVoxels = (size_t)1 << 28;
 constexpr size_t kPtsPad = 4, kCellStartPad = 4;
 constexpr size_t kCellStartFront = 4;
+constexpr uint32_t kPts12Pad = 16;
+constexpr size_t pts12_bytes(size_t n) { return (n + kPts12Pad) * 12 + 64; }
 constexpr uint32_t kRankQuadraticMax = 1u << 20;
 constexpr int kMaxPartialBlocks = 1024;
 constexpr uint32_t kAdaptMinPoints = 1u << 18;
@@ -274,6 +293,7 @@
     bool vor_valid = false;
     DevBuf pts12;
     bool pts12_valid = false;
+    bool working_copy_written = false;
     uint32_t occ_host = 0;
     bool occ_host_valid = false;
     DevBuf cell_of;
@@ -287,9 +307,13 @@
     float min_cell_edge = 0.0f;
     float target_ppo = 0.0f;
     const GridGeom *reuse_geom = nullptr;
-    const IcpState *state_transform = nullptr;
+    bool moved = false;
+    IcpStart start{};
     const TileGeom *tile_major = nullptr;
     bool strict_order = false;
+    bool pack12 = false;
+    float4 *working_copy = nullptr;
+    IcpState *fresh_state = nullptr;
 };
 __host__ __device__ inline int ball_rings(const GridGeom &g, float radius) {
     const int gyz = g.gy > g.gz ? g.gy : g.gz;
@@ -531,6 +555,8 @@
     const DeviceIndex *src_presorted = nullptr;
 };
 tc_status icp_run(tc_context *ctx, const IcpJob &job, tc_icp_result *res);
+tc_status pack12(tc_context *ctx, DeviceIndex &ix);
+tc_status working_source(tc_context *ctx, const float4 *src, size_t n, float4 *out, IcpState *st, const IcpStart &start);
 tc_status icp_run_sharded(tc_context *ctx, tc_comm *comm, int shard_mode, const IcpJob &job, tc_icp_result *res);
 
 }
```

New measurement: 18060 it/s, median of 4. Within noise of the previous version (+1.4%).
